# manhtuando97/two-stage-gnn

Hardware: AMD Instinct MI355X
Metric: graphs/sec fwd+bwd, DD batch=32 SAGE-3L h=128 (higher is better)
Workload: dtype f32

## Files before the change

include/tsgnn.h:

```cpp
#ifndef TSGNN_H
#define TSGNN_H
#include <stdint.h>

typedef struct ihipStream_t* tsgnn_stream_t;

#ifdef __cplusplus
extern "C" {
#endif

#define TSGNN_ABI_VERSION 2
int tsgnn_abi_version(void);
const char* tsgnn_strerror(int code);
const char* tsgnn_last_kernel(void);


int tsgnn_scan_workspace_ints(int64_t n, int64_t* ws_ints);
int tsgnn_exclusive_scan_i32(const int* in, int64_t n, int* out, int* ws, tsgnn_stream_t stream);

int tsgnn_row_maps(const int* graph_ptr, int B, int64_t n_rows, int* row_graph, int* row_slot,
                   tsgnn_stream_t stream);

int tsgnn_dense_adj_count(const float* adj, int B, int nmax, const int* graph_ptr, const int* row_graph,
                          int64_t n_rows, int* row_cnt, tsgnn_stream_t stream);
int tsgnn_dense_adj_fill(const float* adj, int B, int nmax, const int* graph_ptr, const int* row_graph,
// ... 44 lines not shown
                              void* after_event, int64_t* ticket);
int tsgnn_collate_pool_submit_ack(tsgnn_collate_pool* pool, const int64_t* ds_graph_ptr, const int64_t* ds_rowptr, const int64_t* ds_col,
                                  const int64_t* ds_node_label, const int64_t* ds_graph_label, const int64_t* ids, int B, int nmax,
                                  int64_t row_cap, int64_t edge_cap, int ell_w, int64_t tail_cap, int32_t* staging, int64_t* out,
                                  const int64_t* host_ack, int64_t ack_target, int seq, int64_t* ticket);
int tsgnn_collate_pool_wait(tsgnn_collate_pool* pool, int64_t ticket);
int tsgnn_collate_pool_destroy(tsgnn_collate_pool* pool);

int tsgnn_csr_transpose(const int* rowptr, const int* col, const float* val, int64_t n_rows, int64_t n_cols,
                        int64_t nnz, int* rowptr_t, int* col_t, float* val_t, int* src_e, int* cnt_ws,
                        int* scan_ws, tsgnn_stream_t stream);


int tsgnn_csr_spmm_f32(const int* rowptr, const int* col, const float* val, const float* self_w,
                       const float* x, int64_t ldx, float* y, int64_t ldy, int64_t n_rows, int feat,
                       float self_scalar, int relu_in, int accumulate, tsgnn_stream_t stream);

int tsgnn_csr_to_ell(const int* rowptr, const int* col, int64_t n_rows, int W, int* ell, int* tail_cnt, tsgnn_stream_t stream);
int tsgnn_csr_tail_fill(const int* rowptr, const int* col, const int* tail_ptr, int64_t n_rows, int W, int* tail_col,
                        tsgnn_stream_t stream);
int tsgnn_ell_spmm_f32(const int* ell, int W, const float* x, int64_t ldx, float* y, int64_t ldy, int64_t n_rows, int feat,
                       float self_scalar, tsgnn_stream_t stream);

int tsgnn_gcn_norm_f32(const int* rowptr, const int* col, const float* val, int64_t n_rows, float self_fill,
                       float* dinv, float* val_out, float* self_w, tsgnn_stream_t stream);

int tsgnn_sddmm_rows_f32(const int* rowptr, const int* col, const float* dy, int64_t lddy, const float* x, int64_t ldx,
                         int64_t n_rows, int feat, float* dval, float* dself, tsgnn_stream_t stream);


int tsgnn_gemm_f32(const float* A, int64_t sam, int64_t sak, const float* B, int64_t sbk, int64_t sbn, float* C,
                   int64_t scm, int64_t scn, int M, int N, int K, int batch, int64_t stride_a, int64_t stride_b,
                   int64_t stride_c, const int* seg_ptr, int ragged, int max_seg, float alpha, int accumulate,
                   tsgnn_stream_t stream);
int tsgnn_gemm_splitk_plan(int M, int N, int K, int* ksplit, int64_t* ws_floats);
int tsgnn_gemm_splitk_f32(const float* A, int64_t sam, int64_t sak, const float* B, int64_t sbk, int64_t sbn,
                          float* C, int M, int N, int K, int ksplit, float* ws, int accumulate,
                          tsgnn_stream_t stream);
int tsgnn_linear_wgrad_plan(int64_t rows, int K_in, int N, int64_t ldz, int64_t lddu, int* nslab, int64_t* rows_per_slab,
                            int64_t* ws_floats);
int tsgnn_linear_wgrad_f32(const float* z, int64_t ldz, const float* du, int64_t lddu, int64_t rows, int K_in, int N, int nslab,
                           int64_t rows_per_slab, int64_t bias_only_rows, float* ws, float* dw, float* db, tsgnn_stream_t stream);
int tsgnn_wgrad_reduce_sets_blocks(const int64_t* desc);
int tsgnn_wgrad_reduce_sets_f32(const int64_t* desc, float* normparts, float* step_state, tsgnn_stream_t stream);
int tsgnn_wgrad_reduce_multi_f32(const float* ws0, int nslab0, int K0, int N0, float* dw0, float* db0, const float* ws1, int nslab1,
                                 int K1, int N1, float* dw1, float* db1, const float* ws2, int nslab2, int K2, int N2, float* dw2,
                                 float* db2, const float* ws3, int nslab3, int K3, int N3, float* dw3, float* db3,
                                 float* normparts, float* step_state, tsgnn_stream_t stream);
int tsgnn_wgrad_blocks_plan(int64_t rows, int K_in, int N, int64_t ldz, int64_t lddu, int* nslab, int64_t* rows_per_slab,
                            int64_t* ws_floats);
int tsgnn_wgrad_blocks_f32(const float* z, int64_t ldz, const float* du, int64_t lddu, int64_t rows, int K_in, int N, int nslab,
                           int64_t rows_per_slab, float* ws, float* dw, int64_t lddw, tsgnn_stream_t stream);
int tsgnn_wgrad_blocks_oi_f32(const float* z, int64_t ldz, const float* du, int64_t lddu, int64_t rows, int K_in, int N, int nslab,
                              int64_t rows_per_slab, float* ws, float* dw_oi, int64_t lddw, float* db, tsgnn_stream_t stream);
int tsgnn_ragged_tn_f32(const float* s_mat, int64_t lds_, const float* x, int64_t ldx, int K, int N, const int* slab_row_ptr,
                        int nslab, const int* seg_slab_ptr, int nseg, float* ws, float* out, tsgnn_stream_t stream);
int tsgnn_ragged_tn_direct_supported(int K, int64_t max_rows);
int tsgnn_ragged_tn_direct_f32(const float* s_mat, int64_t lds_, int K, const int* graph_ptr, int B, const float* x0, int64_t ldx0,
                               int N0, float* out0, const float* x1, int64_t ldx1, int N1, float* out1, tsgnn_stream_t stream);
int tsgnn_ragged_tn_direct_ro_f32(const float* s_mat, int64_t lds_, int K, const int* graph_ptr, int B, const float* x0, int64_t ldx0,
                                  int N0, float* out0, const float* x1, int64_t ldx1, int N1, float* out1, float* ro_out,
                                  int64_t ro_ldo, int* ro_arg, int nmax, int64_t n_real, int ghost_zero, tsgnn_stream_t stream);
int tsgnn_wgrad_narrow_plan(int64_t rows, int K_in, int N, int64_t* ws_floats);
int tsgnn_wgrad_narrow_f32(const float* z, int64_t ldz, const float* du, int64_t lddu, int64_t rows, int K_in, int N, float* ws,
                           float* dwb, tsgnn_stream_t stream);
int tsgnn_colsum_f32(const float* x, int64_t ld, int64_t rows, int F, float* out, float* ws, int accumulate,
                     tsgnn_stream_t stream);

int tsgnn_linear_l2norm_f32(const float* z, int64_t ldz, const float* w, int64_t ldw, const float* bias, float* v,
                            int64_t ldv, float* rinv, int64_t rows, int K, int N, int normalize,
                            tsgnn_stream_t stream);
int tsgnn_rowgemm_supported(const float* a, int64_t lda, const float* b, int64_t ldb, const float* c, int64_t ldc, int K, int N,
                            int trans_b);
int tsgnn_rowgemm_f32(const float* a, int64_t lda, const float* b, int64_t ldb, int trans_b, const float* bias, float* c,
                      int64_t ldc, float* rinv, int64_t rows, int K, int N, int normalize, int64_t fill_rows,
                      tsgnn_stream_t stream);
int tsgnn_panel_blocks(int64_t rows, int panel_units);
int tsgnn_gather_rowgemm_f32(const int* ell, int ell_w, const int* tail_ptr, const int* tail_col, const float* x, int64_t ldx, const float* b, int64_t ldb, int trans_b,
                             const float* bias, float* c, int64_t ldc, float* rinv, float* zout, int64_t ldz, int64_t rows, int K,
                             int N, int normalize, int64_t fill_rows, tsgnn_stream_t stream);
int tsgnn_gather_rowgemm_st_f32(const int* ell, int ell_w, const int* tail_ptr, const int* tail_col, const float* x, int64_t ldx, const float* b, int64_t ldb, const float* bias,
                                float* c, int64_t ldc, float* rinv, float* zout, int64_t ldz, int64_t rows, int K, int N,
                                int64_t fill_rows, const int* row_slot, unsigned long long* sums, float* ghost, int panel_units,
                                tsgnn_stream_t stream);
int tsgnn_sage_layer_fwd_bn_f32(const int* ell, int ell_w, const int* tail_ptr, const int* tail_col, const float* x, int64_t ldx, const float* w, int64_t ldw, const float* bias,
                                float* v, int64_t ldv, float* rinv, float* zout, int64_t ldz, int64_t rows, int K, int64_t fill_rows,
                                const int* graph_ptr, const int* slot_count, int B, int nslots, int n_ghost, unsigned long long* packed,
                                unsigned long long* packed_out, const int* row_graph, const unsigned long long* sums_in,
                                const float* ghost_in, float* mean_out, float* rstd_out, const int* row_slot,
                                unsigned long long* sums_out, float* ghost_out, const int* ro_map, int ro_map_ch, int panel_units,
                                tsgnn_stream_t stream);
int tsgnn_sage_layer_fwd_bn_plan(int64_t rows, int64_t fill_rows, int B, int nslots, int panel_units, int* ro_ch, int* n_gemm,
                                 int* n_full);
int tsgnn_sage_layer_fwd_f32(const int* ell, int ell_w, const int* tail_ptr, const int* tail_col, const float* x, int64_t ldx, const float* w, int64_t ldw, const float* bias,
                             float* v, int64_t ldv, float* rinv, float* zout, int64_t ldz, int64_t rows, int K, int64_t fill_rows,
                             const int* graph_ptr, int B, int nslots, int n_ghost, unsigned long long* packed, tsgnn_stream_t stream);
int tsgnn_sage_layer_fwd_ro_f32(const int* ell, int ell_w, const int* tail_ptr, const int* tail_col, const float* x, int64_t ldx, const float* w, int64_t ldw, const float* bias,
                                float* v, int64_t ldv, float* rinv, float* zout, int64_t ldz, int64_t rows, int K, int64_t fill_rows,
                                const int* graph_ptr, int B, int nslots, int n_ghost, unsigned long long* packed,
                                unsigned long long* packed_out, const int* row_graph, tsgnn_stream_t stream);
int tsgnn_sage_layer_bwd_f32(const int* ell, int ell_w, const int* tail_ptr, const int* tail_col, const float* du, int64_t lddu, const float* w, int64_t ldw, float* dxs,
                             int64_t lddxs, const float* z, int64_t ldz, int64_t rows, int nslab, int64_t rows_per_slab,
                             int64_t bias_only_rows, float* ws, int panel_units, tsgnn_stream_t stream);
int tsgnn_l2norm_bwd_f32(const float* v, int64_t ldv, const float* dv, int64_t lddv, const float* rinv, float* du,
                         int64_t lddu, int64_t rows, int F, tsgnn_stream_t stream);


int tsgnn_bn_slots_fwd_f32(const int* graph_ptr, const int* slot_count, const int* row_slot, int B, int nmax,
                           int64_t n_real, int n_ghost, const float* v, int64_t ldv, int F, int relu, int bn,
                           float* mean, float* rstd, float* y, int64_t ldy, tsgnn_stream_t stream);
int tsgnn_bn_slots_bwd_f32(const int* graph_ptr, const int* slot_count, const int* row_slot, int B, int nmax,
                           int64_t n_real, int n_ghost, const float* v, int64_t ldv, const float* dy, int64_t lddy, int F,
                           int relu, int bn, const float* mean, const float* rstd, float* m1, float* m2, float* dv,
                           int64_t lddv, tsgnn_stream_t stream);

int tsgnn_row_ln_fwd_f32(const float* v, int64_t ldv, int64_t rows, int F, int relu, float* mean, float* rstd, float* y, int64_t ldy,
                         tsgnn_stream_t stream);
int tsgnn_row_ln_bwd_f32(const float* v, int64_t ldv, const float* dy, int64_t lddy, int64_t rows, int F, int relu, const float* mean,
                         const float* rstd, float* dv, int64_t lddv, tsgnn_stream_t stream);

int tsgnn_row_post_bwd_f32(const int* row_graph, int B, int64_t n_real, int64_t rows, const float* v, int64_t ldv, const float* dxs,
                           int64_t lddxs, const float* dout, int64_t ldo, const int* arg, int F, int relu, int ln, const float* mean,
                           const float* rstd, const float* rinv, float* du, int64_t lddu, tsgnn_stream_t stream);

int tsgnn_row_post_nodes_bwd_f32(int64_t n_real, int64_t rows, const float* v, int64_t ldv, const float* dxs, int64_t lddxs,
                                 const float* dnode, int64_t lddn, int ghost_zero, int F, int relu, int ln, const float* mean,
                                 const float* rstd, const float* rinv, float* du, int64_t lddu, tsgnn_stream_t stream);

int tsgnn_readout_max_ws_words(int B, int nmax, int F);
int tsgnn_readout_max_fwd_f32(const int* graph_ptr, const int* slot_count, int B, int nmax, int64_t n_real, int n_ghost,
                              const float* x, int64_t ldx, int F, int relu, unsigned long long* packed_ws, float* out,
                              int64_t ldo, int* arg, tsgnn_stream_t stream);
int tsgnn_readout_max_bwd_f32(const float* dout, int64_t ldo, const int* arg, int B, int F, const float* x, int64_t ldx_in,
                              int relu, int64_t n_real, float* dx, int64_t ldx, tsgnn_stream_t stream);
int tsgnn_readout_max_bwd_rows_f32(const float* dout, int64_t ldo, const int* arg, const int* row_graph, int F, int64_t rows,
                                   int64_t rows_total, const float* add, int64_t ldadd, float* dx, int64_t ldx, tsgnn_stream_t stream);

int tsgnn_pack_rows_f32(const float* src, int nmax, int F, const int* row_graph, const int* row_slot, int64_t n_real,
                        float* dst, int64_t ld, tsgnn_stream_t stream);
int tsgnn_unpack_rows_f32(const int* graph_ptr, int B, int nmax, int64_t n_real, int n_ghost, const float* src, int64_t ld,
                          int F, float fill, float* dst, tsgnn_stream_t stream);
int tsgnn_unpack_rows_bwd_ghost_f32(const int* graph_ptr, int B, int nmax, int64_t n_real, const float* ddst, int F,
                                    float* dsrc, int64_t ld, tsgnn_stream_t stream);


int tsgnn_softmax_ce_f32(const float* logits, int64_t ld, const int64_t* label, int B, int C, float* loss, float* dlogits,
                         tsgnn_stream_t stream);
int tsgnn_adam_from_partials_f32(float* param, const float* grad, float* m, float* v, int64_t n, float lr, float beta1, float beta2,
                                 float eps, float weight_decay, float max_norm, float* state, const float* parts, int nparts,
                                 const float* poison, tsgnn_stream_t stream);
int tsgnn_clip_adam_step_f32(float* param, const float* grad, float* m, float* v, int64_t n, float lr, float beta1,
                             float beta2, float eps, float weight_decay, float max_norm, float grad_scale, float* state,
                             float* ws, const float* poison, tsgnn_stream_t stream);


int tsgnn_dense_stack_supported(int B, int K, int nstack, int L, int fin0, int hidden, int last0, int last1);
int tsgnn_dense_stack_fwd_f32(const int64_t* desc, tsgnn_stream_t stream);
int tsgnn_dense_stack_bwd_f32(const int64_t* desc, tsgnn_stream_t stream);
int tsgnn_dense_stack_max_resident(void);
int tsgnn_dense_stack_barrier_selftest(unsigned* sync, float* err, int expect, tsgnn_stream_t stream);


int tsgnn_node_scores_f32(const float* x, int64_t ldx, int64_t rows, int H, int Fh, const float* a, int64_t lda, float* s,
                          tsgnn_stream_t stream);
int tsgnn_node_scores2_f32(const float* x, int64_t ldx, int64_t rows, int H, int Fh, const float* a1, int64_t lda1, float* s1,
                           const float* a2, int64_t lda2, float* s2, tsgnn_stream_t stream);
int tsgnn_edge_softmax_fwd_f32(const int* rowptr, const int* col, int64_t rows, int H, const float* s_grp, const float* s_oth,
                               int mod, float slope, float* alpha, tsgnn_stream_t stream);
int tsgnn_edge_softmax_bwd_f32(const int* rowptr, const int* col, int64_t rows, int H, const float* s_grp, const float* s_oth,
                               int mod, float slope, const float* alpha, const float* dalpha, float* dt, float* ds_grp,
                               tsgnn_stream_t stream);
int tsgnn_edge_permute_f32(const float* src, const int* perm, int64_t n, int H, int scatter, float* dst, tsgnn_stream_t stream);
int tsgnn_csr_row_sum_f32(const int* rowptr, const float* val, int64_t rows, int H, float* out, tsgnn_stream_t stream);
int tsgnn_csr_row_sum_perm_f32(const int* rowptr, const float* val, const int* eperm, int64_t rows, int H, float* out,
                               tsgnn_stream_t stream);
int tsgnn_csr_spmm_heads_f32(const int* rowptr, const int* col, const float* alpha, int H, int Fh, const float* x, int64_t ldx,
                             int mod, float* y, int64_t ldy, int64_t rows, tsgnn_stream_t stream);
int tsgnn_csr_spmm_heads_epi_f32(const int* rowptr, const int* col, const float* alpha, int H, int Fh, const float* x, int64_t ldx,
                                 int mod, float* y, int64_t ldy, int64_t rows, const float* w1, const float* a1, int64_t lda1,
                                 const float* w2, const float* a2, int64_t lda2, const float* u, int64_t ldu, const float* uw,
                                 int rows_per_seg, const int* row_seg, float uscale, const int* eperm, tsgnn_stream_t stream);
int tsgnn_csr_sddmm_heads_f32(const int* rowptr, const int* col, int H, int Fh, const float* dy, int64_t lddy, const float* x,
                              int64_t ldx, int mod, float* dalpha, int64_t rows, tsgnn_stream_t stream);
int tsgnn_segment_wsum_f32(const float* x, int64_t ldx, const float* w, int H, int Fh, const int* seg_ptr, int nseg, int64_t rows,
                           int64_t max_seg, float scale, int mean, float* ws, float* out, int64_t ldo, tsgnn_stream_t stream);
int tsgnn_segment_wsum2_f32(const float* x, int64_t ldx, const float* w1, const float* w2, int H, int Fh, const int* seg_ptr, int nseg,
// ... 350 lines not shown
```

two-stage-gnn_amd/csrc/head.hip:

```cpp
#include "common.h"
#include "../../include/tsgnn.h"
#include "readout_body.h"
#include "ingest_rider.h"

namespace {

__device__ __forceinline__ float4 ld4(const float* p) { return *reinterpret_cast<const float4*>(p); }

constexpr int HW = 16;

__device__ __forceinline__ void head2_fwd_tail(const float* xs, float* vs, int b, const float* __restrict__ w1,
                                               const float* __restrict__ b1, const float* __restrict__ w2, const float* __restrict__ b2,
                                               int P, int E, int C, float* __restrict__ vec, float* __restrict__ y) {
  const int tid = threadIdx.x, lane = tid & 63, wid = tid >> 6;
  const int P4 = P >> 2;
  for (int j0 = wid; j0 < E; j0 += 8 * HW) {
    float acc[8];
#pragma unroll
    for (int u = 0; u < 8; ++u) acc[u] = 0.f;
    for (int k4 = lane; k4 < P4; k4 += 64) {
      const float4 x = *reinterpret_cast<const float4*>(xs + 4 * k4);
      float4 w[8];
#pragma unroll
      for (int u = 0; u < 8; ++u) {
        const int j = j0 + HW * u;
        w[u] = ld4(w1 + (int64_t)(j < E ? j : 0) * P + 4 * k4);
      }
#pragma unroll
      for (int u = 0; u < 8; ++u) acc[u] += (w[u].x * x.x + w[u].y * x.y) + (w[u].z * x.z + w[u].w * x.w);
    }
#pragma unroll
    for (int u = 0; u < 8; ++u) {
      const int j = j0 + HW * u;
      const float r = wave_sum(acc[u]);
      if (lane == 0 && j < E) { const float v = r + (b1 ? b1[j] : 0.f); vs[j] = v; vec[(int64_t)b * E + j] = v; }
    }
  }
  __syncthreads();
  for (int c = wid; c < C; c += HW) {
    float acc = 0.f;
    for (int j = lane; j < E; j += 64) acc = fmaf(w2[(int64_t)c * E + j], vs[j], acc);
    acc = wave_sum(acc);
    if (lane == 0) y[(int64_t)b * C + c] = acc + (b2 ? b2[c] : 0.f);
  }
}

struct RoTail {
  const float* z; int64_t ldz; int N, c0, F;
  int* arg;
  float* dz; int64_t lddz;
};

__global__ __launch_bounds__(64 * HW) void head2_fwd_kernel(float* __restrict__ out, int64_t ldo, const float* __restrict__ w1,
                                                        const float* __restrict__ b1, const float* __restrict__ w2,
                                                        const float* __restrict__ b2, int P, int E, int C,
                                                        float* __restrict__ vec, float* __restrict__ y, RoTail rt) {
  extern __shared__ __attribute__((aligned(16))) float smem[];
  float* xs = smem;
  float* vs = smem + ((P + 3) & ~3);
  const int b = blockIdx.x, tid = threadIdx.x;
  const int c0 = rt.z ? rt.c0 : P;
  for (int k = tid; k < P; k += 64 * HW) {
    if (k < c0) { xs[k] = out[(int64_t)b * ldo + k]; continue; }
    const int f = k - c0;
    unsigned long long best = 0ull;
    for (int n0 = 0; n0 < rt.N; n0 += 16) {
      float val[16];
#pragma unroll
      for (int u = 0; u < 16; ++u) val[u] = rt.z[((int64_t)b * rt.N + min(n0 + u, rt.N - 1)) * rt.ldz + f];
#pragma unroll
      for (int u = 0; u < 16; ++u) {
        if (n0 + u < rt.N) {
          const unsigned long long q = ((unsigned long long)f32_ordered(val[u]) << 32) |
                                       (unsigned long long)(0xFFFFFFFFu - (unsigned)(b * rt.N + n0 + u));
          best = q > best ? q : best;
        }
      }
    }
    const float v = best ? ordered_f32((unsigned)(best >> 32)) : 0.f;
    xs[k] = v;
    out[(int64_t)b * ldo + k] = v;
    rt.arg[(int64_t)b * rt.F + f] = best ? (int)(0xFFFFFFFFu - (unsigned)(best & 0xFFFFFFFFull)) : -1;
  }
  __syncthreads();
  head2_fwd_tail(xs, vs, b, w1, b1, w2, b2, P, E, C, vec, y);
}

struct ReadoutHeadArgs {
  const unsigned long long* packed; int B, L, Fh, Fl;
  const float* v_last; int64_t ldv;
// ... 326 lines not shown
  for (int b = only >= 0 ? only + (int)threadIdx.x * B : (int)threadIdx.x; b < B; b += 64 * HW) {
    const float* row = ce.y + (int64_t)b * C;
    float m = -INFINITY;
    for (int c = 0; c < C; ++c) m = fmaxf(m, row[c]);
    float d = 0.f;
    for (int c = 0; c < C; ++c) d += expf(row[c] - m);
    const int yb = (int)ce.label[b];
    const float logz = m + logf(d);
    lb[b] = logz - row[yb];
    for (int c = 0; c < C; ++c) dyl[b * C + c] = (expf(row[c] - logz) - (c == yb ? 1.f : 0.f)) * invB;
  }
}

struct DuArgs {
  const int* graph_ptr; int64_t n_real; int n_ghost_rows; int chunks;
  const float* v; int64_t ldv; const float* rinv; const int* arg; int off; int F;
  float* du; int64_t lddu;
  const int* map;
  int compact;
};
template <int DU_CHUNK>
__device__ __forceinline__ void du_resolve(const DuArgs& a, int d, int B, int& b, int& c, int& pad_k, int& pad_n) {
  pad_k = -1; pad_n = a.chunks;
  if (a.map) { b = a.map[d] >> 8; c = a.map[d] & 255; }
  else if (a.compact) {
    const int lane = threadIdx.x & 63;
    const int g0 = a.graph_ptr[min(lane, B)], g1 = a.graph_ptr[min(lane + 1, B)];
    const int nch = lane < B ? max(1, (g1 - g0 + DU_CHUNK - 1) / DU_CHUNK) : 0;
    int pre = nch;
#pragma unroll
    for (int o = 1; o < 64; o <<= 1) { const int t = __shfl_up(pre, o, 64); if (lane >= o) pre += t; }
    const int total = __shfl(pre, 63, 64);
    if (d >= total) { b = B; c = 0; pad_k = d - total; pad_n = (int)gridDim.x - a.compact - total; return; }
    const unsigned long long m = __ballot(pre > d);
    b = __ffsll((long long)m) - 1;
    c = d - (__shfl(pre, b, 64) - __shfl(nch, b, 64));
  } else { b = d / a.chunks; c = d - b * a.chunks; }
  if (b >= B) { pad_k = c; b = B; }
}

template <int DU_CHUNK>
__device__ __forceinline__ void head2_du_role(const DuArgs& a, float* smem, const float* dy , int b, int c,
                                              int pad_k, int pad_n, const float* __restrict__ dvec, const float* __restrict__ w1,
                                              const float* __restrict__ w2, int B, int P, int E, int C, bool dy_ready_needs_sync) {
  const int tid = threadIdx.x, NTH = 64 * HW;
  const int F4 = a.F >> 2, lig = tid & 31, rg = tid >> 5;
  const float4 z4 = make_float4(0.f, 0.f, 0.f, 0.f);
  if (pad_k >= 0) {
    const int64_t lo = a.graph_ptr[B];
    for (int64_t r = lo + (int64_t)pad_k * 32 + rg; r < a.n_real; r += (int64_t)max(pad_n, 1) * 32)
      if (lig < F4) *reinterpret_cast<float4*>(a.du + r * a.lddu + 4 * lig) = z4;
    return;
  }
  const int g0 = a.graph_ptr[b], sz = a.graph_ptr[b + 1] - g0;
  const int lo = DU_CHUNK * c, hi = min(sz, lo + DU_CHUNK);
  const bool ghost_job = c == 0;
  if (lo >= hi && !ghost_job) return;
  const int P4 = P >> 2;
  const int G = min(16, NTH / P4);
  float* ds = smem;
  float* part = smem + ((E + 3) & ~3);
  float* dseg = part + G * a.F;
  constexpr int DU_ROWS = 8;
  static_assert(RB_ROWS % DU_ROWS == 0, "the row block's batches are walked in pieces");
  const int jg = tid >> 5;
  const bool wact = jg < G && lig < F4;
  const unsigned wcol = (unsigned)a.off + 4u * (unsigned)(wact ? lig : 0);
  float4 w[DU_ROWS];
#pragma unroll
  for (int u = 0; u < DU_ROWS; ++u) {
    const int j = jg + G * u;
    w[u] = ld4(w1 + (size_t)((unsigned)((wact && j < E) ? j : 0) * (unsigned)P + wcol));
  }
  float w2r[4];
  float dv0 = 0.f;
  if (tid < E) {
#pragma unroll
    for (int q = 0; q < 4; ++q) w2r[q] = q < C ? w2[(int64_t)q * E + tid] : 0.f;
    if (dvec) dv0 = dvec[(int64_t)b * E + tid];
  }
  if (dy_ready_needs_sync) __syncthreads();
  for (int j = tid; j < E; j += NTH) {
    float acc = j == tid ? dv0 : (dvec ? dvec[(int64_t)b * E + j] : 0.f);
    for (int q = 0; q < C; ++q) acc = fmaf(dy[(int64_t)b * C + q], (j == tid && q < 4) ? w2r[q] : w2[(int64_t)q * E + j], acc);
    ds[j] = acc;
  }
  __syncthreads();
  float4 acc = z4;
#pragma unroll
  for (int u0 = 0; u0 < RB_ROWS; u0 += DU_ROWS) {
    if (u0 > 0) {
#pragma unroll
      for (int u = 0; u < DU_ROWS; ++u) {
        const int j = jg + G * (u0 + u);
        w[u] = ld4(w1 + (size_t)((unsigned)((wact && j < E) ? j : 0) * (unsigned)P + wcol));
      }
    }
#pragma unroll
    for (int u = 0; u < DU_ROWS; ++u) {
      const int j = jg + G * (u0 + u);
      const float dd = (wact && j < E) ? ds[j] : 0.f;
      acc.x = fmaf(dd, w[u].x, acc.x); acc.y = fmaf(dd, w[u].y, acc.y); acc.z = fmaf(dd, w[u].z, acc.z); acc.w = fmaf(dd, w[u].w, acc.w);
    }
    __builtin_amdgcn_sched_barrier(0);
  }
  const unsigned ldv = (unsigned)a.ldv, lddu = (unsigned)a.lddu, col = 4u * (unsigned)(lig < F4 ? lig : 0);
  float4 vv[DU_CHUNK / 32];
  float ri[DU_CHUNK / 32];
  int rows[DU_CHUNK / 32];
#pragma unroll
  for (int u = 0; u < DU_CHUNK / 32; ++u) {
    const int n = lo + rg + 32 * u;
    rows[u] = n < hi ? g0 + n : -1;
    const unsigned rr = rows[u] >= 0 ? (unsigned)rows[u] : 0u;
    vv[u] = ld4(a.v + (size_t)(rr * ldv + col));
    ri[u] = a.rinv[rr];
  }
  const bool has_ghost = ghost_job && sz < a.n_ghost_rows;
  const int grow = (int)a.n_real + (has_ghost ? sz : 0);
  float4 gv = z4;
  float gri = 0.f;
  if (ghost_job && rg == 0 && a.n_ghost_rows > 0) { gv = ld4(a.v + (size_t)((unsigned)grow * ldv + col)); gri = a.rinv[grow]; }
  const int4 win = *reinterpret_cast<const int4*>(a.arg + (size_t)((unsigned)b * (unsigned)a.F + col));
  if (wact) *reinterpret_cast<float4*>(part + jg * a.F + 4 * lig) = acc;
  __syncthreads();
  for (int k = tid; k < a.F; k += NTH) {
    float t = 0.f;
    for (int q = 0; q < G; ++q) t += part[q * a.F + k];
    dseg[k] = t;
  }
  __syncthreads();
  const float4 gd = lig < F4 ? *reinterpret_cast<const float4*>(dseg + 4 * lig) : z4;
#pragma unroll
  for (int u = 0; u < DU_CHUNK / 32; ++u) {
    const int r32 = rows[u];
    float4 dyv = z4;
    if (rows[u] >= 0 && lig < F4) {
      if (win.x == r32) dyv.x = gd.x;
      if (win.y == r32) dyv.y = gd.y;
      if (win.z == r32) dyv.z = gd.z;
      if (win.w == r32) dyv.w = gd.w;
    } else {
      vv[u] = z4;
    }
    float dot = (vv[u].x * dyv.x + vv[u].y * dyv.y) + (vv[u].z * dyv.z + vv[u].w * dyv.w);
    dot = group_sum<32>(dot);
    if (rows[u] >= 0 && lig < F4) {
      if (ri[u] >= 0.999e12f) dot = 0.f;
      *reinterpret_cast<float4*>(a.du + (size_t)((unsigned)rows[u] * lddu + col)) =
          make_float4(ri[u] * (dyv.x - vv[u].x * dot), ri[u] * (dyv.y - vv[u].y * dot), ri[u] * (dyv.z - vv[u].z * dot),
                      ri[u] * (dyv.w - vv[u].w * dot));
    }
  }
  if (ghost_job && rg == 0) {
    const int r32 = grow;
    float4 dyv = z4;
    if (has_ghost && lig < F4) {
      if (win.x == r32) dyv.x = gd.x;
      if (win.y == r32) dyv.y = gd.y;
      if (win.z == r32) dyv.z = gd.z;
      if (win.w == r32) dyv.w = gd.w;
    } else {
      gv = z4;
    }
    float dot = (gv.x * dyv.x + gv.y * dyv.y) + (gv.z * dyv.z + gv.w * dyv.w);
    dot = group_sum<32>(dot);
    if (gri >= 0.999e12f) dot = 0.f;
    if (lig < F4)
      *reinterpret_cast<float4*>(a.du + (size_t)((unsigned)((int)a.n_real + b) * lddu + col)) =
          make_float4(gri * (dyv.x - gv.x * dot), gri * (dyv.y - gv.y * dot), gri * (dyv.z - gv.z * dot), gri * (dyv.w - gv.w * dot));
  }
}

template <int DU_CHUNK>
__global__ __launch_bounds__(64 * HW) void head2_bwd2_kernel(const float* __restrict__ out, int64_t ldo, const float* __restrict__ vec,
                                                         const float* __restrict__ dy_in, const float* __restrict__ dvec,
                                                         const float* __restrict__ w1, const float* __restrict__ w2, int B, int P, int E,
                                                         int C, float* __restrict__ dout, int64_t lddo, float* __restrict__ dw1,
                                                         float* __restrict__ db1, float* __restrict__ dw2, float* __restrict__ db2,
                                                         float* __restrict__ normparts, CeArgs ce, DuArgs dua, RoTail rt) {
  extern __shared__ __attribute__((aligned(16))) float smem_all[];
  const int tid = threadIdx.x, NTH = 64 * HW;
  const int P4 = P >> 2, PP = P;
  const bool has_ce = ce.label != nullptr;
  float* dyl = smem_all;
  float* lb = smem_all + (has_ce ? ((B * C + 3) & ~3) : 0);
  float* smem = lb + (has_ce ? ((B + 3) & ~3) : 0);
  const float* dy = has_ce ? dyl : dy_in;
  const int nj = (E + 3) / 4;
  if ((int)blockIdx.x >= B + nj + 1) {
    const int d = (int)blockIdx.x - (B + nj + 1);
    int gb, gc, pad_k, pad_n;
    du_resolve<DU_CHUNK>(dua, d, B, gb, gc, pad_k, pad_n);
    if (has_ce && pad_k < 0) ce_rows(ce, B, C, dyl, lb, gb);
    head2_du_role<DU_CHUNK>(dua, smem, dy, gb, gc, pad_k, pad_n, dvec, w1, w2, B, P, E, C, has_ce);
    return;
  }

  if ((int)blockIdx.x < B) {
    const int b = blockIdx.x;
    const int G = min(16, NTH / P4);
    const int jg = tid / P4, k4 = tid - jg * P4;
    const bool active = jg < G;
    float* ds = smem;
    float* part = smem + ((E + 3) & ~3);
    float w2r[4];
    float dv0 = 0.f;
    if (tid < E) {
#pragma unroll
      for (int c = 0; c < 4; ++c) w2r[c] = c < C ? w2[(int64_t)c * E + tid] : 0.f;
      if (dvec) dv0 = dvec[(int64_t)b * E + tid];
    }
    float4 w[RB_ROWS];
#pragma unroll
    for (int u = 0; u < RB_ROWS; ++u) {
      const int j = jg + G * u;
      w[u] = ld4(w1 + (int64_t)((active && j < E) ? j : 0) * P + 4 * (active ? k4 : 0));
    }
    if (has_ce) {
      ce_rows(ce, B, C, dyl, lb, b == 0 ? -1 : b);
      __syncthreads();
      if (b == 0) {
        float* red = lb + ((B + 3) & ~3);
        if (tid < 256) {
          float part = 0.f;
          for (int q = tid; q < B; q += 256) part += lb[q];
          part = wave_sum(part);
          if ((tid & 63) == 0) red[tid >> 6] = part;
        }
        __syncthreads();
        if (tid == 0) ce.loss[0] = ((red[0] + red[1]) + (red[2] + red[3])) / (float)B;
        __syncthreads();
      }
    }
    for (int j = tid; j < E; j += NTH) {
      float acc = j == tid ? dv0 : (dvec ? dvec[(int64_t)b * E + j] : 0.f);
      for (int c = 0; c < C; ++c) acc = fmaf(dy[(int64_t)b * C + c], (j == tid && c < 4) ? w2r[c] : w2[(int64_t)c * E + j], acc);
      ds[j] = acc;
    }
    __syncthreads();
    float4 acc = make_float4(0.f, 0.f, 0.f, 0.f);
    for (int j0 = 0; j0 < E; j0 += G * RB_ROWS) {
      if (j0 > 0) {
#pragma unroll
        for (int u = 0; u < RB_ROWS; ++u) {
          const int j = j0 + jg + G * u;
          w[u] = ld4(w1 + (int64_t)((active && j < E) ? j : 0) * P + 4 * (active ? k4 : 0));
        }
      }
#pragma unroll
      for (int u = 0; u < RB_ROWS; ++u) {
        const int j = j0 + jg + G * u;
        const float d = (active && j < E) ? ds[j] : 0.f;
        acc.x = fmaf(d, w[u].x, acc.x); acc.y = fmaf(d, w[u].y, acc.y); acc.z = fmaf(d, w[u].z, acc.z); acc.w = fmaf(d, w[u].w, acc.w);
      }
    }
    if (active) *reinterpret_cast<float4*>(part + jg * PP + 4 * k4) = acc;
    __syncthreads();
    for (int k = tid; k < P; k += NTH) {
      float a = 0.f;
      for (int q = 0; q < G; ++q) a += part[q * PP + k];
      dout[(int64_t)b * lddo + k] = a;
      if (rt.dz && k >= rt.c0 && k < rt.c0 + rt.F) {
        const int f = k - rt.c0;
        const int win = rt.arg[(int64_t)b * rt.F + f];
        for (int n = 0; n < rt.N; ++n) rt.dz[((int64_t)b * rt.N + n) * rt.lddz + f] = (b * rt.N + n) == win ? a : 0.f;
      }
    }
    return;
  }
  const int jb = (int)blockIdx.x - B;
  float sq = 0.f;
  if (jb < nj) {
    const int j0 = 4 * jb;
    const int G = max(1, min(8, 768 / P4));
    const int bg = tid / P4, k4 = tid - bg * P4;
    const bool active = bg < G;
    float* dvs = smem;
    float* part = smem + 4 * ((B + 3) & ~3);
    float w2r[4];
    float dv0 = 0.f;
    const int sb = tid >> 2, sj = j0 + (tid & 3);
    if (tid < 4 * B && sj < E) {
#pragma unroll
      for (int c = 0; c < 4; ++c) w2r[c] = c < C ? w2[(int64_t)c * E + sj] : 0.f;
      if (dvec) dv0 = dvec[(int64_t)sb * E + sj];
    }
    float4 x[WB_ROWS];
#pragma unroll
    for (int u = 0; u < WB_ROWS; ++u) {
      const int bb = bg + G * u;
      x[u] = ld4(out + (int64_t)((active && bb < B) ? bb : 0) * ldo + 4 * (active ? k4 : 0));
    }
    if (has_ce) { ce_rows(ce, B, C, dyl, lb, -1); __syncthreads(); }
    for (int i = tid; i < 4 * B; i += NTH) {
      const int bb = i >> 2, jj = j0 + (i & 3);
      float a = 0.f;
      if (jj < E) {
        a = i == tid ? dv0 : (dvec ? dvec[(int64_t)bb * E + jj] : 0.f);
        for (int c = 0; c < C; ++c) a = fmaf(dy[(int64_t)bb * C + c], (i == tid && c < 4) ? w2r[c] : w2[(int64_t)c * E + jj], a);
      }
      dvs[i] = a;
    }
    __syncthreads();
    float4 a0 = make_float4(0.f, 0.f, 0.f, 0.f), a1 = a0, a2 = a0, a3 = a0;
    for (int b0 = 0; b0 < B; b0 += G * WB_ROWS) {
      if (b0 > 0) {
#pragma unroll
        for (int u = 0; u < WB_ROWS; ++u) {
          const int bb = b0 + bg + G * u;
          x[u] = ld4(out + (int64_t)((active && bb < B) ? bb : 0) * ldo + 4 * (active ? k4 : 0));
        }
      }
#pragma unroll
      for (int u = 0; u < WB_ROWS; ++u) {
        const int bb = b0 + bg + G * u;
        if (active && bb < B) {
          const float4 d = *reinterpret_cast<const float4*>(dvs + 4 * bb);
          a0.x = fmaf(d.x, x[u].x, a0.x); a0.y = fmaf(d.x, x[u].y, a0.y); a0.z = fmaf(d.x, x[u].z, a0.z); a0.w = fmaf(d.x, x[u].w, a0.w);
          a1.x = fmaf(d.y, x[u].x, a1.x); a1.y = fmaf(d.y, x[u].y, a1.y); a1.z = fmaf(d.y, x[u].z, a1.z); a1.w = fmaf(d.y, x[u].w, a1.w);
          a2.x = fmaf(d.z, x[u].x, a2.x); a2.y = fmaf(d.z, x[u].y, a2.y); a2.z = fmaf(d.z, x[u].z, a2.z); a2.w = fmaf(d.z, x[u].w, a2.w);
          a3.x = fmaf(d.w, x[u].x, a3.x); a3.y = fmaf(d.w, x[u].y, a3.y); a3.z = fmaf(d.w, x[u].z, a3.z); a3.w = fmaf(d.w, x[u].w, a3.w);
        }
      }
    }
    if (active) {
      float* pp = part + (int64_t)bg * 4 * PP + 4 * k4;
      *reinterpret_cast<float4*>(pp) = a0; *reinterpret_cast<float4*>(pp + PP) = a1;
      *reinterpret_cast<float4*>(pp + 2 * PP) = a2; *reinterpret_cast<float4*>(pp + 3 * PP) = a3;
    }
    __syncthreads();
    for (int i = tid; i < 4 * P; i += NTH) {
      const int jj = i / P, k = i - jj * P;
      if (j0 + jj < E) {
        float a = 0.f;
        for (int q = 0; q < G; ++q) a += part[(q * 4 + jj) * PP + k];
        dw1[(int64_t)(j0 + jj) * P + k] = a;
        sq = fmaf(a, a, sq);
      }
    }
    if (db1 && tid < 4 && j0 + tid < E) {
      float a = 0.f;
      for (int bb = 0; bb < B; ++bb) a += dvs[4 * bb + tid];
      db1[j0 + tid] = a;
      sq = fmaf(a, a, sq);
    }
  } else {
    if (has_ce) { ce_rows(ce, B, C, dyl, lb, -1); __syncthreads(); }
    for (int i = tid; i < C * E; i += NTH) {
      const int c = i / E, j = i - c * E;
      float a = 0.f;
      int bb = 0;
      for (; bb + 8 <= B; bb += 8) {
        float v[8];
#pragma unroll
        for (int u = 0; u < 8; ++u) v[u] = vec[(int64_t)(bb + u) * E + j];
#pragma unroll
        for (int u = 0; u < 8; ++u) a = fmaf(dy[(int64_t)(bb + u) * C + c], v[u], a);
      }
      for (; bb < B; ++bb) a = fmaf(dy[(int64_t)bb * C + c], vec[(int64_t)bb * E + j], a);
      dw2[i] = a;
      sq = fmaf(a, a, sq);
    }
    if (db2) for (int c = tid; c < C; c += NTH) {
      float a = 0.f;
      for (int bb = 0; bb < B; ++bb) a += dy[(int64_t)bb * C + c];
      db2[c] = a;
      sq = fmaf(a, a, sq);
    }
  }
  if (normparts) {
    sq = wave_sum(sq);
    __syncthreads();
    if ((tid & 63) == 0) smem[tid >> 6] = sq;
    __syncthreads();
    if (tid == 0) {
      float t = 0.f;
      for (int w = 0; w < HW; ++w) t += smem[w];
      normparts[jb] = t;
    }
  }
}

// ... 217 lines not shown
```

two-stage-gnn_amd/csrc/ingest_rider.h:

```cpp
#pragma once
#include "common.h"

struct PullRider { const int4* host; int4* mirror; long long n4; unsigned blocks; long long lo; int parts_left; int skip; };
extern thread_local PullRider tsgnn_pull_rider_;

static inline PullRider take_pull_rider(int threads = 256) {
  PullRider& a = tsgnn_pull_rider_;
  PullRider r = a;
  if (a.blocks == 0) return r;
  if (a.skip > 0) { --a.skip; r.blocks = 0; return r; }
  const int parts = a.parts_left > 1 ? a.parts_left : 1;
  const long long left = a.n4 - a.lo;
  const long long take = parts > 1 ? ((left / parts + 3) & ~3ll) : left;
  r.n4 = a.lo + (take < left ? take : left);
  long long blocks = (r.n4 - r.lo + 2ll * threads - 1) / (2ll * threads);
  if (blocks > 512) blocks = 512;
  if (blocks < 1) blocks = 1;
  r.blocks = (unsigned)blocks;
  a.lo = r.n4;
  a.parts_left = parts - 1;
  if (a.parts_left <= 0 || a.lo >= a.n4) a.blocks = 0;
  return r;
}
static inline void disarm_pull_rider() { tsgnn_pull_rider_.blocks = 0; }

__device__ __forceinline__ void pull_rider_body(const PullRider& p, unsigned b) {
  const long long gtid = (long long)b * blockDim.x + threadIdx.x, gsize = (long long)p.blocks * blockDim.x;
  int4 v[4];
  long long i = p.lo + gtid;
  for (; i + 3 * gsize < p.n4; i += 4 * gsize) {
#pragma unroll
    for (int u = 0; u < 4; ++u) v[u] = p.host[i + u * gsize];
#pragma unroll
    for (int u = 0; u < 4; ++u) p.mirror[i + u * gsize] = v[u];
  }
  for (; i < p.n4; i += gsize) p.mirror[i] = p.host[i];
}

struct CLayout {
  int64_t header, graph_ptr, slot_count, label, rowptr, node_label, tail_ptr, col, tail_col, total;
};

struct ExpandArgs {
  const int32_t* mirror; CLayout L;
  int B, nmax, ell_w, F, ld4; int64_t row_cap;
  int32_t* row_graph; int32_t* row_slot; int32_t* ell; int32_t* tail_ptr; float* x; int64_t ldx;
  int64_t* host_ack;
  int32_t* ell_slots; int32_t* tail_slots;
};
__device__ __forceinline__ int expand_graph_of(const ExpandArgs& a, int64_t r, const int32_t* gp) {
  int lo = 0, hi = a.B;
  while (hi - lo > 1) { const int mid = (lo + hi) >> 1; if (gp[mid] <= r) lo = mid; else hi = mid; }
  return lo;
}

__device__ __forceinline__ void expand_row_lane(const ExpandArgs& a, int64_t r, int q, const int32_t* gp) {
  const int64_t total_rows = a.row_cap + a.nmax;
  if (a.host_ack && r == 0 && q == 0) {
    __hip_atomic_store(a.host_ack, (int64_t)a.mirror[a.L.header + 4], __ATOMIC_RELEASE, __HIP_MEMORY_SCOPE_SYSTEM);
  }
  if (r >= total_rows) return;
  const int64_t n = a.mirror[a.L.header];
  const int32_t ntail = a.mirror[a.L.header + 2];
  const int EQ = a.ell_w / 4;
  const int l = (r < n) ? a.mirror[a.L.node_label + r] : -1;
  if (q < EQ) {
    int4 v = make_int4(-1, -1, -1, -1);
    if (r < n) {
      const int32_t* rowptr = a.mirror + a.L.rowptr;
      const int e0 = rowptr[r], d = rowptr[r + 1] - e0;
      const int32_t* col = a.mirror + a.L.col + e0;
      const int k = 4 * q;
      if (k < d) v.x = col[k];
      if (k + 1 < d) v.y = col[k + 1];
      if (k + 2 < d) v.z = col[k + 2];
      if (k + 3 < d) v.w = col[k + 3];
    }
    *reinterpret_cast<int4*>(a.ell + r * a.ell_w + 4 * q) = v;
    if (a.ell_slots) {
      int4 w = make_int4(-1, -1, -1, -1);
      if (r < n) {
        const int g0 = gp[expand_graph_of(a, r, gp)];
        if (v.x >= 0) w.x = ((v.x - g0) << 20) | v.x;
        if (v.y >= 0) w.y = ((v.y - g0) << 20) | v.y;
        if (v.z >= 0) w.z = ((v.z - g0) << 20) | v.z;
        if (v.w >= 0) w.w = ((v.w - g0) << 20) | v.w;
      }
      *reinterpret_cast<int4*>(a.ell_slots + r * a.ell_w + 4 * q) = w;
    }
  } else if (q == EQ) {
    int g0 = 0;
    if (r < a.row_cap) {
      int g = a.B, slot = -1;
      if (r < n) {
        g = expand_graph_of(a, r, gp);
        g0 = gp[g];
        slot = (int)(r - g0);
      }
      a.row_graph[r] = g;
      a.row_slot[r] = slot;
    }
    a.tail_ptr[r] = r < n ? a.mirror[a.L.tail_ptr + r] : ntail;
    if (r == total_rows - 1) a.tail_ptr[total_rows] = ntail;
    if (a.tail_slots && r < n) {
      const int e1 = (r + 1 < n) ? a.mirror[a.L.tail_ptr + r + 1] : ntail;
      for (int e = a.mirror[a.L.tail_ptr + r]; e < e1; ++e) {
        const int j = a.mirror[a.L.tail_col + e];
        a.tail_slots[e] = ((j - g0) << 20) | j;
      }
    }
  } else {
    const bool ok = l >= 0 && l < a.F;
    for (int c4 = q - EQ - 1; c4 < a.ld4; c4 += 32 - EQ - 1) {
      const int c = 4 * c4;
      const float4 v = make_float4((ok && l == c) ? 1.f : 0.f, (ok && l == c + 1) ? 1.f : 0.f, (ok && l == c + 2) ? 1.f : 0.f,
                                   (ok && l == c + 3) ? 1.f : 0.f);
      *reinterpret_cast<float4*>(a.x + r * a.ldx + c) = v;
// ... 31 lines not shown
```

two-stage-gnn_amd/csrc/layer_bwd.hip:

```cpp
#include "common.h"
#include "../../include/tsgnn.h"
#include "rowgemm_body.h"
#include "tn_rows_body.h"
#include <cstdlib>

namespace {

template <bool PANELS_FIRST, bool UNITS = false>
__global__ __launch_bounds__(256) void sage_layer_bwd_kernel(RowGemmArgs ga, TnArgs gt, unsigned n_tn, unsigned nslab, unsigned n_pan, int slab_delay) {
  extern __shared__ __attribute__((aligned(16))) float smem[];
  if (PANELS_FIRST) {
    if (blockIdx.x < n_pan) rowgemm_body<4, true, true, 1, false, false, false, UNITS>(ga, smem, blockIdx.x);
    else {
      for (int i = 0; i < slab_delay; ++i) __builtin_amdgcn_s_sleep(16);
      const unsigned b = blockIdx.x - n_pan, by = b / nslab, sp = b % nslab;
      unsigned sl = sp;
      if ((nslab & 7u) == 0) sl = ((blockIdx.x & 7u) * (nslab >> 3)) + (sp >> 3);
      tn_rows_body<4, 4, 2>(gt, smem, sl, by, nslab);
    }
  } else {
    if (blockIdx.x < n_tn) tn_rows_body<4, 4, 2>(gt, smem, blockIdx.x % nslab, blockIdx.x / nslab, nslab);
    else rowgemm_body<4, true, true, 1, false, false, false, UNITS>(ga, smem, blockIdx.x - n_tn);
  }
}

}

extern "C" {

int tsgnn_sage_layer_bwd_f32(const int* ell, int ell_w, const int* tail_ptr, const int* tail_col, const float* du, int64_t lddu, const float* w, int64_t ldw, float* dxs,
                             int64_t lddxs, const float* z, int64_t ldz, int64_t rows, int nslab, int64_t rows_per_slab,
                             int64_t bias_only_rows, float* ws, int panel_units, tsgnn_stream_t stream) {
  if (!ell || !du || !w || !dxs || !z || !ws || rows <= 0 || nslab <= 0 || rows_per_slab <= 0 || bias_only_rows < 0) return TSGNN_EINVAL;
  if (ell_w != 4 && ell_w != 8 && ell_w != 16) return TSGNN_EUNSUPPORTED;
  const uintptr_t al = reinterpret_cast<uintptr_t>(ell) | reinterpret_cast<uintptr_t>(du) | reinterpret_cast<uintptr_t>(w) |
                       reinterpret_cast<uintptr_t>(dxs) | reinterpret_cast<uintptr_t>(z);
  if ((al & 15) || (lddu % 4) || (ldw % 4) || (lddxs % 4) || (ldz % 4) || lddu < 128 || ldw < 128 || lddxs < 128 || ldz < 128)
    return TSGNN_EUNSUPPORTED;
  if ((tail_ptr == nullptr) != (tail_col == nullptr)) return TSGNN_EINVAL;
  RowGemmArgs ga{du, lddu, w, ldw, nullptr, dxs, lddxs, nullptr, rows, 128, 128, 0, 0, ell, ell_w, nullptr, 0, tail_ptr, tail_col};
  TnArgs gt{z, ldz, du, lddu, rows, rows_per_slab, 128, 128, ws, nullptr, bias_only_rows};
  const int ncu = device_cu_count();
  const unsigned n_tn = 2u * (unsigned)nslab, n_pan = panel_split(rows, ncu, panel_units, &ga.n_full, &ga.unit);
  constexpr size_t la = rowgemm_lds_bytes<4, true, true>(), lt = tn_rows_lds_bytes<4, 4>();
  static const int panels_first = [] { const char* e = getenv("TSGNN_BWD_PANELS_FIRST"); return e ? atoi(e) : 1; }();
  static const int slab_delay_env = [] { const char* e = getenv("TSGNN_SLAB_DELAY"); return e ? atoi(e) : -1; }();
  const int slab_delay = slab_delay_env >= 0 ? slab_delay_env : ((int64_t)n_pan <= (int64_t)ncu ? 2 : 0);
  const bool units = ga.unit == 8 || ga.unit == 16;
  TSGNN_KNAME("sage_layer_bwd_kernel<%s,%s>", panels_first ? "true" : "false", units ? "true" : "false");
  if (panels_first && units) sage_layer_bwd_kernel<true, true><<<n_tn + n_pan, 256, la > lt ? la : lt, stream>>>(ga, gt, n_tn, (unsigned)nslab, n_pan, slab_delay);
  else if (panels_first) sage_layer_bwd_kernel<true><<<n_tn + n_pan, 256, la > lt ? la : lt, stream>>>(ga, gt, n_tn, (unsigned)nslab, n_pan, slab_delay);
  else if (units) sage_layer_bwd_kernel<false, true><<<n_tn + n_pan, 256, la > lt ? la : lt, stream>>>(ga, gt, n_tn, (unsigned)nslab, n_pan, slab_delay);
  else sage_layer_bwd_kernel<false><<<n_tn + n_pan, 256, la > lt ? la : lt, stream>>>(ga, gt, n_tn, (unsigned)nslab, n_pan, slab_delay);
  TSGNN_CHECK_LAUNCH();
  return TSGNN_OK;
}

}
```

two-stage-gnn_amd/csrc/layer_fwd.hip:

```cpp
#include "common.h"
#include "../../include/tsgnn.h"
#include "rowgemm_body.h"
#include "readout_body.h"
#include "ingest_rider.h"

namespace {

template <bool RO>
__global__ __launch_bounds__(256) void sage_layer_fwd_kernel(RowGemmArgs ga, SlotArgs sa, unsigned n_gemm, unsigned ro_gx, int F4,
                                                             unsigned long long* __restrict__ packed, unsigned n_main, PullRider pr) {
  extern __shared__ __attribute__((aligned(16))) float smem[];
  if (blockIdx.x < n_gemm) {
    rowgemm_body<4, false, true, 1, RO>(ga, smem, blockIdx.x);
  } else if (blockIdx.x < n_main) {
    const unsigned r = blockIdx.x - n_gemm;
    readout_partial_body<32>(sa, ga.a, ga.lda, F4, packed, r % ro_gx, r / ro_gx, reinterpret_cast<unsigned long long*>(smem));
  } else {
    pull_rider_body(pr, blockIdx.x - n_main);
  }
}

template <bool RO, bool ST, bool UNITS = false>
__global__ __launch_bounds__(256, 2) void sage_layer_fwd_bn_kernel(RowGemmArgs ga, SlotArgs sa, BnReadArgs bn, unsigned n_gemm, unsigned ro_gx,
                                                                int ro_ch, int F4, unsigned long long* __restrict__ packed, unsigned n_main,
                                                                PullRider pr, const int* __restrict__ ro_map) {
  extern __shared__ __attribute__((aligned(16))) float smem[];
  if (blockIdx.x < n_gemm) {
    rowgemm_body<4, false, true, 1, RO, true, ST, UNITS>(ga, smem, blockIdx.x);
  } else if (blockIdx.x < n_main) {
    unsigned r = blockIdx.x - n_gemm;
    if (ro_map) r = (unsigned)ro_map[r];
    readout_partial_bn_body<32>(sa, bn, ga.a, ga.lda, F4, packed, r % ro_gx, r / ro_gx, ro_ch, reinterpret_cast<unsigned long long*>(smem));
  } else {
    pull_rider_body(pr, blockIdx.x - n_main);
  }
}

}

extern "C" {

int tsgnn_sage_layer_fwd_bn_plan(int64_t rows, int64_t fill_rows, int B, int nslots, int panel_units, int* ro_ch, int* n_gemm, int* n_full) {
  if (!ro_ch || !n_gemm || !n_full || rows <= 0 || B <= 0 || nslots <= 0) return TSGNN_EINVAL;
  const int ncu = device_cu_count();
  int unit_ = 16;
  const unsigned ng = panel_split(rows, ncu, panel_units, n_full, &unit_) + (fill_rows > 0 ? 1u : 0u);
  int ch = 64;
  while (ch < 256 && ng + (unsigned)((nslots + ch - 1) / ch) * (unsigned)B > 2u * (unsigned)ncu) ch *= 2;
  *ro_ch = ch; *n_gemm = (int)ng;
  return TSGNN_OK;
}

int tsgnn_sage_layer_fwd_bn_f32(const int* ell, int ell_w, const int* tail_ptr, const int* tail_col, const float* x, int64_t ldx, const float* w, int64_t ldw, const float* bias,
                                float* v, int64_t ldv, float* rinv, float* zout, int64_t ldz, int64_t rows, int K, int64_t fill_rows,
                                const int* graph_ptr, const int* slot_count, int B, int nslots, int n_ghost, unsigned long long* packed,
                                unsigned long long* packed_out, const int* row_graph, const unsigned long long* sums_in,
                                const float* ghost_in, float* mean_out, float* rstd_out, const int* row_slot,
                                unsigned long long* sums_out, float* ghost_out, const int* ro_map, int ro_map_ch, int panel_units,
                                tsgnn_stream_t stream) {
  if (!ell || !x || !w || !v || !rinv || !graph_ptr || !slot_count || !packed || !sums_in || !ghost_in || !mean_out || !rstd_out ||
      rows <= 0 || fill_rows < 0 || K <= 0 || B <= 0 || nslots <= 0 || (n_ghost != 0 && n_ghost != nslots) || (packed_out && !row_graph) ||
      (row_slot && (!sums_out || !ghost_out)))
    return TSGNN_EINVAL;
  if (ell_w != 4 && ell_w != 8 && ell_w != 16) return TSGNN_EUNSUPPORTED;
  const uintptr_t al = reinterpret_cast<uintptr_t>(ell) | reinterpret_cast<uintptr_t>(x) | reinterpret_cast<uintptr_t>(w) |
                       reinterpret_cast<uintptr_t>(v) | reinterpret_cast<uintptr_t>(zout) | reinterpret_cast<uintptr_t>(bias) |
                       reinterpret_cast<uintptr_t>(sums_in) | reinterpret_cast<uintptr_t>(sums_out);
  if ((al & 15) || K != 128 || (ldx % 4) || (ldw % 4) || (ldv % 4) || (zout && (ldz % 4 || ldz < K)) || ldx < K || ldw < 128 || ldv < 128 ||
      nslots > BN_TAB || rows >= (1 << 20) || n_ghost == 0 || (packed_out && row_slot))
    return TSGNN_EUNSUPPORTED;
  if (packed_out && fill_rows <= 0) return TSGNN_EUNSUPPORTED;
  if ((tail_ptr == nullptr) != (tail_col == nullptr)) return TSGNN_EINVAL;
  RowGemmArgs ga{x, ldx, w, ldw, bias, v, ldv, rinv, rows, K, 128, 1, fill_rows, ell, ell_w, zout, ldz, tail_ptr, tail_col,
                 packed_out, graph_ptr, row_graph, B, nslots, n_ghost};
  ga.st_row_slot = row_slot; ga.st_sums = sums_out; ga.st_ghost = ghost_out;
  ga.bn_sums = sums_in; ga.bn_ghost = ghost_in; ga.bn_slot_count = slot_count; ga.bn_B = B; ga.bn_nslots = nslots; ga.bn_F = K;
  SlotArgs sa{graph_ptr, slot_count, B, nslots, rows, n_ghost};
  BnReadArgs bn{sums_in, ghost_in, K, mean_out, rstd_out};
  const int ncu = device_cu_count();
  const unsigned n_gemm = panel_split(rows, ncu, panel_units, &ga.n_full, &ga.unit) + (fill_rows > 0 ? 1u : 0u);
  int ro_ch = 64;
  while (ro_ch < 256 && n_gemm + (unsigned)((nslots + ro_ch - 1) / ro_ch) * (unsigned)B > 2u * (unsigned)ncu) ro_ch *= 2;
  const unsigned ro_gx = (unsigned)((nslots + ro_ch - 1) / ro_ch);
  if (ro_map && ro_map_ch != ro_ch) ro_map = nullptr;
  size_t lds = rowgemm_lds_bytes<4, false, true, 1, true>();
  const size_t lro = 8 * 128 * sizeof(unsigned long long) + 256 * sizeof(float2);
  if (lds < lro) lds = lro;
  const unsigned n_main = n_gemm + ro_gx * (unsigned)B;
  const PullRider pr = take_pull_rider();
  const bool units = ga.unit == 8 || ga.unit == 16;
#define TSGNN_FWD_BN(RO_, ST_)                                                                                                              \
  do {                                                                                                                                      \
    if (units) sage_layer_fwd_bn_kernel<RO_, ST_, true><<<n_main + pr.blocks, 256, lds, stream>>>(ga, sa, bn, n_gemm, ro_gx, ro_ch, K / 4, packed, n_main, pr, ro_map); \
    else sage_layer_fwd_bn_kernel<RO_, ST_><<<n_main + pr.blocks, 256, lds, stream>>>(ga, sa, bn, n_gemm, ro_gx, ro_ch, K / 4, packed, n_main, pr, ro_map);             \
  } while (0)
  if (packed_out) {
    TSGNN_KNAME("sage_layer_fwd_bn_kernel<true,false,%s>", units ? "true" : "false");
    TSGNN_FWD_BN(true, false);
  } else if (row_slot) {
    TSGNN_KNAME("sage_layer_fwd_bn_kernel<false,true,%s>", units ? "true" : "false");
    TSGNN_FWD_BN(false, true);
  } else {
    TSGNN_KNAME("sage_layer_fwd_bn_kernel<false,false,%s>", units ? "true" : "false");
    TSGNN_FWD_BN(false, false);
  }
#undef TSGNN_FWD_BN
  TSGNN_CHECK_LAUNCH();
  return TSGNN_OK;
}

int tsgnn_sage_layer_fwd_ro_f32(const int* ell, int ell_w, const int* tail_ptr, const int* tail_col, const float* x, int64_t ldx, const float* w, int64_t ldw, const float* bias,
                                float* v, int64_t ldv, float* rinv, float* zout, int64_t ldz, int64_t rows, int K, int64_t fill_rows,
                                const int* graph_ptr, int B, int nslots, int n_ghost, unsigned long long* packed,
                                unsigned long long* packed_out, const int* row_graph, tsgnn_stream_t stream) {
  if (!ell || !x || !w || !v || !rinv || !graph_ptr || !packed || rows <= 0 || fill_rows < 0 || K <= 0 || B <= 0 || nslots <= 0 ||
      (n_ghost != 0 && n_ghost != nslots) || (packed_out && !row_graph))
    return TSGNN_EINVAL;
  if (ell_w != 4 && ell_w != 8 && ell_w != 16) return TSGNN_EUNSUPPORTED;
  const uintptr_t al = reinterpret_cast<uintptr_t>(ell) | reinterpret_cast<uintptr_t>(x) | reinterpret_cast<uintptr_t>(w) |
                       reinterpret_cast<uintptr_t>(v) | reinterpret_cast<uintptr_t>(zout) | reinterpret_cast<uintptr_t>(bias);
  if ((al & 15) || K != 128 || (ldx % 4) || (ldw % 4) || (ldv % 4) || (zout && (ldz % 4 || ldz < K)) || ldx < K || ldw < 128 || ldv < 128)
    return TSGNN_EUNSUPPORTED;
  if ((tail_ptr == nullptr) != (tail_col == nullptr)) return TSGNN_EINVAL;
  if (packed_out && n_ghost && fill_rows <= 0) return TSGNN_EUNSUPPORTED;
  RowGemmArgs ga{x, ldx, w, ldw, bias, v, ldv, rinv, rows, K, 128, 1, fill_rows, ell, ell_w, zout, ldz, tail_ptr, tail_col,
                 packed_out, graph_ptr, row_graph, B, nslots, n_ghost};
  SlotArgs sa{graph_ptr, nullptr, B, nslots, rows, n_ghost};
  const unsigned n_gemm = (unsigned)ceil_div64(rows, 32) + (fill_rows > 0 ? 1u : 0u);
  const unsigned ro_gx = (unsigned)((nslots + 63) / 64);
  size_t lds = rowgemm_lds_bytes<4, false, true>();
  if (lds < 8 * 128 * sizeof(unsigned long long)) lds = 8 * 128 * sizeof(unsigned long long);
  const unsigned n_main = n_gemm + ro_gx * (unsigned)B;
  const PullRider pr = take_pull_rider();
  if (packed_out) {
    TSGNN_KNAME("sage_layer_fwd_kernel<true>");
    sage_layer_fwd_kernel<true><<<n_main + pr.blocks, 256, lds, stream>>>(ga, sa, n_gemm, ro_gx, K / 4, packed, n_main, pr);
  } else {
    TSGNN_KNAME("sage_layer_fwd_kernel<false>");
    sage_layer_fwd_kernel<false><<<n_main + pr.blocks, 256, lds, stream>>>(ga, sa, n_gemm, ro_gx, K / 4, packed, n_main, pr);
  }
  TSGNN_CHECK_LAUNCH();
  return TSGNN_OK;
}

int tsgnn_sage_layer_fwd_f32(const int* ell, int ell_w, const int* tail_ptr, const int* tail_col, const float* x, int64_t ldx, const float* w, int64_t ldw, const float* bias,
                             float* v, int64_t ldv, float* rinv, float* zout, int64_t ldz, int64_t rows, int K, int64_t fill_rows,
                             const int* graph_ptr, int B, int nslots, int n_ghost, unsigned long long* packed, tsgnn_stream_t stream) {
  return tsgnn_sage_layer_fwd_ro_f32(ell, ell_w, tail_ptr, tail_col, x, ldx, w, ldw, bias, v, ldv, rinv, zout, ldz, rows, K, fill_rows,
                                     graph_ptr, B, nslots, n_ghost, packed, nullptr, nullptr, stream);
}

}
```

two-stage-gnn_amd/csrc/rowgemm.hip:

```cpp
#include "common.h"
#include "../../include/tsgnn.h"

#include <cstdlib>
#include "rowgemm_body.h"
#include "ingest_rider.h"
#include "rowgemm_big_body.h"

namespace {

inline unsigned ks2_max_blocks() {
  static const unsigned n = [] { const char* e = getenv("TSGNN_KS2_MAX_BLOCKS"); return e ? (unsigned)atoi(e) : (unsigned)device_cu_count(); }();
  return n;
}
inline bool rowgemm_ks2_enabled() {
  static const bool on = [] { const char* e = getenv("TSGNN_ROWGEMM_KS2"); return !(e && e[0] == '0'); }();
  return on;
}

template <int NT, bool TRANS_B, bool GATHER>
__global__ __launch_bounds__(256) void rowgemm_kernel(RowGemmArgs g) {
  extern __shared__ __attribute__((aligned(16))) float smem[];
  rowgemm_body<NT, TRANS_B, GATHER>(g, smem, blockIdx.x);
}

template <int NT, bool TRANS_B>
__global__ __launch_bounds__(512) void rowgemm_gather_ks2_kernel(RowGemmArgs g) {
  extern __shared__ __attribute__((aligned(16))) float smem[];
  rowgemm_body<NT, TRANS_B, true, 2>(g, smem, blockIdx.x);
}

template <bool UNITS>
__global__ __launch_bounds__(256) void rowgemm_gather_st_kernel(RowGemmArgs g, PullRider pr, unsigned nblk) {
  extern __shared__ __attribute__((aligned(16))) float smem[];
  if (blockIdx.x >= nblk) { pull_rider_body(pr, blockIdx.x - nblk); return; }
  rowgemm_body<4, false, true, 1, false, false, true, UNITS>(g, smem, blockIdx.x);
}
__global__ __launch_bounds__(512) void rowgemm_gather_ks2_st_kernel(RowGemmArgs g, PullRider pr, unsigned nblk) {
  extern __shared__ __attribute__((aligned(16))) float smem[];
  if (blockIdx.x >= nblk) { pull_rider_body(pr, blockIdx.x - nblk); return; }
  rowgemm_body<4, false, true, 2, false, false, true>(g, smem, blockIdx.x);
}

template <int NT, bool TRANS_B>
__global__ __launch_bounds__(256) void rowgemm_colsplit_kernel(RowGemmArgs g) {
  extern __shared__ __attribute__((aligned(16))) float smem[];
  const int n0 = (int)blockIdx.y * 32 * NT;
  g.N = min(32 * NT, g.N - n0);
  g.c += n0;
  if (g.bias) g.bias += n0;
  g.b += TRANS_B ? (int64_t)n0 * g.ldb : (int64_t)n0;
  g.rinv = nullptr;
  if (!TRANS_B && g.N <= 32) rowgemm_body<1, TRANS_B, false>(g, smem, blockIdx.x);
  else rowgemm_body<NT, TRANS_B, false>(g, smem, blockIdx.x);
}

inline bool rowgemm_colsplit_enabled() {
  static const bool on = [] { const char* e = getenv("TSGNN_ROWGEMM_COLSPLIT"); return !(e && e[0] == '0'); }();
  return on;
}

inline unsigned colsplit_max_panels() {
  static const unsigned n = [] {
    const char* e = getenv("TSGNN_ROWGEMM_COLSPLIT_PANELS");
    return e ? (unsigned)atoi(e) : 0xFFFFFFFFu;
  }();
  return n;
}

inline int64_t rowgemm_big_min_rows() {
  static const int64_t n = [] {
    const char* e = getenv("TSGNN_ROWGEMM_BIG_ROWS");
    return e ? (int64_t)atoll(e) : (int64_t)49152;
  }();
  return n;
}

inline int64_t rowgemm_big_wide_min_rows() {
  static const int64_t n = [] {
    const char* e = getenv("TSGNN_ROWGEMM_BIG_WIDE_ROWS");
    return e ? (int64_t)atoll(e) : (int64_t)2048;
  }();
  return n;
}

template <int U, bool TRANS_B>
void launch_big(const RowGemmArgs& g, hipStream_t s) {
  constexpr size_t lds = rowgemm_big_lds_bytes<U, TRANS_B>();
  static const int bpc = [] {
    if (lds > 64 * 1024)
      (void)hipFuncSetAttribute(reinterpret_cast<const void*>(rowgemm_big_kernel<U, TRANS_B>), hipFuncAttributeMaxDynamicSharedMemorySize, (int)lds);
    int n = 0;
    if (hipOccupancyMaxActiveBlocksPerMultiprocessor(&n, reinterpret_cast<const void*>(rowgemm_big_kernel<U, TRANS_B>), 256, lds) != hipSuccess || n < 1) n = 1;
    return n;
  }();
  const unsigned npanels = (unsigned)ceil_div64(g.rows, 32);
  const unsigned ny = (unsigned)((g.N + 127) / 128);
  const unsigned heavy = (unsigned)(g.N / 128 + ((g.N % 128) > 32 ? 1 : 0));
  unsigned grid = (unsigned)device_cu_count() * (unsigned)bpc / (heavy ? heavy : 1u);
  if (grid > npanels) grid = npanels;
  if (grid == 0) grid = 1;
  if (ny > 1) {
    const unsigned per = (npanels + grid - 1) / grid;
    grid = (npanels + per - 1) / per;
  }
  TSGNN_KNAME("rowgemm_big_kernel<%d,%s>", U, TRANS_B ? "true" : "false");
  rowgemm_big_kernel<U, TRANS_B><<<dim3(grid, ny), 256, lds, s>>>(g, npanels);
}

template <bool TRANS_B>
bool try_big(const RowGemmArgs& g, hipStream_t s) {
  const bool wide = g.N > 128;
  const int64_t mn = wide ? rowgemm_big_wide_min_rows() : rowgemm_big_min_rows();
  if (mn <= 0 || g.rows < mn || g.N > 384 || g.K > 128 || (TRANS_B && (g.K % 4)) || (g.N % 4)) return false;
  if (g.N > 128 && (g.normalize || g.fill_rows > 0 || g.rinv)) return false;
  if (g.K <= 96) launch_big<12, TRANS_B>(g, s);
  else launch_big<16, TRANS_B>(g, s);
  return true;
}

template <bool TRANS_B>
bool try_colsplit(const RowGemmArgs& g, hipStream_t s) {
  const unsigned nblk = (unsigned)ceil_div64(g.rows, 32);
// ... 11 lines not shown
  const unsigned nblk = (unsigned)(ceil_div64(g.rows, 32) + (g.fill_rows > 0 ? 1 : 0));
  if constexpr (GATHER && NT <= 4) {
    if (g.K > KC && nblk <= ks2_max_blocks() && rowgemm_ks2_enabled()) {
      constexpr size_t lds2 = rowgemm_lds_bytes<NT, TRANS_B, true, 2>();
      static bool attr = false;
      if (!attr && lds2 > 64 * 1024) {
        (void)hipFuncSetAttribute(reinterpret_cast<const void*>(rowgemm_gather_ks2_kernel<NT, TRANS_B>),
                                  hipFuncAttributeMaxDynamicSharedMemorySize, (int)lds2);
        attr = true;
      }
      TSGNN_KNAME("rowgemm_gather_ks2_kernel<%d,%s>", NT, TRANS_B ? "true" : "false");
      rowgemm_gather_ks2_kernel<NT, TRANS_B><<<nblk, 512, lds2, s>>>(g);
      return;
    }
  }
  const size_t lds = rowgemm_lds_bytes<NT, TRANS_B, GATHER>();
  TSGNN_KNAME("rowgemm_kernel<%d,%s,%s>", NT, TRANS_B ? "true" : "false", GATHER ? "true" : "false");
  rowgemm_kernel<NT, TRANS_B, GATHER><<<nblk, 256, lds, s>>>(g);
}

template <bool TRANS_B, bool GATHER>
void dispatch_rowgemm(const RowGemmArgs& g, hipStream_t s) {
  switch ((g.N + 31) / 32) {
    case 1: launch_rowgemm<1, TRANS_B, GATHER>(g, s); break;
    case 2: launch_rowgemm<2, TRANS_B, GATHER>(g, s); break;
    case 3: launch_rowgemm<3, TRANS_B, GATHER>(g, s); break;
    case 4: launch_rowgemm<4, TRANS_B, GATHER>(g, s); break;
    default:
      if constexpr (!GATHER) {
        switch ((g.N + 31) / 32) {
          case 5: launch_rowgemm<5, TRANS_B, false>(g, s); break;
          case 6: launch_rowgemm<6, TRANS_B, false>(g, s); break;
          case 7: launch_rowgemm<7, TRANS_B, false>(g, s); break;
          default: launch_rowgemm<8, TRANS_B, false>(g, s); break;
        }
      }
      break;
  }
}

}

extern "C" {

int tsgnn_rowgemm_supported(const float* a, int64_t lda, const float* b, int64_t ldb, const float* c, int64_t ldc, int K, int N,
                            int trans_b) {
  const bool al = ((reinterpret_cast<uintptr_t>(a) | reinterpret_cast<uintptr_t>(b)) & 15) == 0;
  if (!al || (lda % 4) || (ldb % 4) || N > 384 || N <= 0 || K <= 0) return 0;
  if (lda < ((K + 3) / 4) * 4) return 0;
  if (!trans_b && (N % 4)) return 0;
  if (trans_b && (K % 4)) return 0;
  (void)c; (void)ldc;
  return 1;
}

int tsgnn_rowgemm_f32(const float* a, int64_t lda, const float* b, int64_t ldb, int trans_b, const float* bias, float* c,
                      int64_t ldc, float* rinv, int64_t rows, int K, int N, int normalize, int64_t fill_rows,
                      tsgnn_stream_t stream) {
  if (!a || !b || !c || rows < 0 || fill_rows < 0 || K <= 0 || N <= 0 || lda < K || ldc < N) return TSGNN_EINVAL;
  if (!tsgnn_rowgemm_supported(a, lda, b, ldb, c, ldc, K, N, trans_b)) return TSGNN_EUNSUPPORTED;
  if (fill_rows > 0 && ((N % 4) || (ldc % 4) || (reinterpret_cast<uintptr_t>(c) & 15) ||
                        (bias && (reinterpret_cast<uintptr_t>(bias) & 15))))
    return TSGNN_EUNSUPPORTED;
  if (rows == 0 && fill_rows == 0) return TSGNN_OK;
  RowGemmArgs g{a, lda, b, ldb, bias, c, ldc, rinv, rows, K, N, normalize, fill_rows, nullptr, 0, nullptr, 0};
  if (trans_b) {
    if (!try_big<true>(g, stream) && !try_colsplit<true>(g, stream)) {
      if (N > 256) return TSGNN_EUNSUPPORTED;
      dispatch_rowgemm<true, false>(g, stream);
    }
  } else {
    if (!try_big<false>(g, stream) && !try_colsplit<false>(g, stream)) {
      if (N > 256) return TSGNN_EUNSUPPORTED;
      dispatch_rowgemm<false, false>(g, stream);
    }
  }
  TSGNN_CHECK_LAUNCH();
  return TSGNN_OK;
}

int tsgnn_gather_rowgemm_st_f32(const int* ell, int ell_w, const int* tail_ptr, const int* tail_col, const float* x, int64_t ldx, const float* b, int64_t ldb, const float* bias,
                                float* c, int64_t ldc, float* rinv, float* zout, int64_t ldz, int64_t rows, int K, int N,
                                int64_t fill_rows, const int* row_slot, unsigned long long* sums, float* ghost, int panel_units,
                                tsgnn_stream_t stream) {
  if (!ell || !x || !b || !c || !row_slot || !sums || !ghost || rows <= 0 || fill_rows < 0 || K <= 0 || N <= 0 || ldx < K || ldc < N)
    return TSGNN_EINVAL;
  if (ell_w != 4 && ell_w != 8 && ell_w != 16) return TSGNN_EUNSUPPORTED;
  if (!tsgnn_rowgemm_supported(x, ldx, b, ldb, c, ldc, K, N, 0) || N > 128 || N <= 96 || K > 128 || (reinterpret_cast<uintptr_t>(ell) & 15) ||
      (reinterpret_cast<uintptr_t>(sums) & 15))
    return TSGNN_EUNSUPPORTED;
  if (zout && ((ldz % 4) || ldz < K || (reinterpret_cast<uintptr_t>(zout) & 15))) return TSGNN_EUNSUPPORTED;
  if ((N % 4) || (ldc % 4) || (reinterpret_cast<uintptr_t>(c) & 15) || (bias && (reinterpret_cast<uintptr_t>(bias) & 15))) return TSGNN_EUNSUPPORTED;
  if ((tail_ptr == nullptr) != (tail_col == nullptr)) return TSGNN_EINVAL;
  RowGemmArgs g{x, ldx, b, ldb, bias, c, ldc, rinv, rows, K, N, 1, fill_rows, ell, ell_w, zout, ldz, tail_ptr, tail_col};
  g.st_row_slot = row_slot; g.st_sums = sums; g.st_ghost = ghost;
  unsigned nblk = (unsigned)(ceil_div64(rows, 32) + (fill_rows > 0 ? 1 : 0));
  const bool ks2 = K > KC && nblk <= ks2_max_blocks() && rowgemm_ks2_enabled();
  if (!ks2)
    nblk = panel_split(rows, device_cu_count(), panel_units, &g.n_full, &g.unit) + (fill_rows > 0 ? 1u : 0u);
  if (ks2) {
    constexpr size_t lds2 = rowgemm_lds_bytes<4, false, true, 2>();
    static bool attr = false;
    if (!attr && lds2 > 64 * 1024) {
      (void)hipFuncSetAttribute(reinterpret_cast<const void*>(rowgemm_gather_ks2_st_kernel), hipFuncAttributeMaxDynamicSharedMemorySize, (int)lds2);
      attr = true;
    }
    const PullRider pr = take_pull_rider(512);
    TSGNN_KNAME("rowgemm_gather_ks2_st_kernel");
    rowgemm_gather_ks2_st_kernel<<<nblk + pr.blocks, 512, lds2, stream>>>(g, pr, nblk);
  } else {
    const PullRider pr = take_pull_rider(256);
    TSGNN_KNAME("rowgemm_gather_st_kernel<%s>", (g.unit == 8 || g.unit == 16) ? "true" : "false");
    if (g.unit == 8 || g.unit == 16) rowgemm_gather_st_kernel<true><<<nblk + pr.blocks, 256, rowgemm_lds_bytes<4, false, true>(), stream>>>(g, pr, nblk);
    else rowgemm_gather_st_kernel<false><<<nblk + pr.blocks, 256, rowgemm_lds_bytes<4, false, true>(), stream>>>(g, pr, nblk);
  }
  TSGNN_CHECK_LAUNCH();
  return TSGNN_OK;
}

int tsgnn_panel_blocks(int64_t rows, int panel_units) {
  if (rows <= 0) return 0;
  int nf = 0, un = 16;
  return (int)panel_split(rows, device_cu_count(), panel_units, &nf, &un);
}

int tsgnn_gather_rowgemm_f32(const int* ell, int ell_w, const int* tail_ptr, const int* tail_col, const float* x, int64_t ldx, const float* b, int64_t ldb, int trans_b,
                             const float* bias, float* c, int64_t ldc, float* rinv, float* zout, int64_t ldz, int64_t rows, int K,
                             int N, int normalize, int64_t fill_rows, tsgnn_stream_t stream) {
  if (!ell || !x || !b || !c || rows < 0 || fill_rows < 0 || K <= 0 || N <= 0 || ldx < K || ldc < N) return TSGNN_EINVAL;
  if (ell_w != 4 && ell_w != 8 && ell_w != 16) return TSGNN_EUNSUPPORTED;
  if (!tsgnn_rowgemm_supported(x, ldx, b, ldb, c, ldc, K, N, trans_b) || N > 128 || K > 128 || (reinterpret_cast<uintptr_t>(ell) & 15))
    return TSGNN_EUNSUPPORTED;
  if (zout && ((ldz % 4) || ldz < K || (reinterpret_cast<uintptr_t>(zout) & 15))) return TSGNN_EUNSUPPORTED;
  if (fill_rows > 0 && ((N % 4) || (ldc % 4) || (reinterpret_cast<uintptr_t>(c) & 15) ||
                        (bias && (reinterpret_cast<uintptr_t>(bias) & 15))))
    return TSGNN_EUNSUPPORTED;
  if (rows == 0 && fill_rows == 0) return TSGNN_OK;
  if ((tail_ptr == nullptr) != (tail_col == nullptr)) return TSGNN_EINVAL;
  RowGemmArgs g{x, ldx, b, ldb, bias, c, ldc, rinv, rows, K, N, normalize, fill_rows, ell, ell_w, zout, ldz, tail_ptr, tail_col};
  if (trans_b) dispatch_rowgemm<true, true>(g, stream);
  else dispatch_rowgemm<false, true>(g, stream);
  TSGNN_CHECK_LAUNCH();
  return TSGNN_OK;
}

}
```

two-stage-gnn_amd/csrc/rowgemm_body.h:

```cpp
#pragma once
#include "common.h"
#include <type_traits>
#include <cstdlib>

namespace {


typedef float f32x16 __attribute__((ext_vector_type(16)));
constexpr int KC = 32;
constexpr int LDA_S = KC + 4;
constexpr float NORM_EPS = 1e-12f;

struct RowGemmArgs {
  const float* a; int64_t lda;
  const float* b; int64_t ldb;
  const float* bias;
  float* c; int64_t ldc;
  float* rinv;
  int64_t rows; int K; int N;
  int normalize;
  int64_t fill_rows;
  const int* ell; int ell_w;
  float* zout; int64_t ldz;
  const int* tail_ptr; const int* tail_col;
  unsigned long long* ro_packed;
  const int* ro_graph_ptr; const int* ro_row_graph;
  int ro_B, ro_nslots, ro_nghost;
  const int* st_row_slot; unsigned long long* st_sums; float* st_ghost;
  const unsigned long long* bn_sums; const float* bn_ghost; const int* bn_slot_count; int bn_B, bn_nslots, bn_F;
  int n_full;
  int unit;
};

inline int panel_unit_rows(int64_t rows, int ncu) {
  static const int forced = [] { const char* e = getenv("TSGNN_PANEL_UNIT"); const int v = e ? atoi(e) : 0; return (v == 8 || v == 16) ? v : 0; }();
  if (forced) return forced;
  return ((rows + 31) / 32 - ncu) <= ncu / 16 ? 8 : 16;
}
inline unsigned panel_split(int64_t rows, int ncu, int panel_units, int* n_full, int* unit) {
  const int64_t P = (rows + 31) / 32;
  *n_full = 0; *unit = 32;
  if (!panel_units || ncu < 8) return (unsigned)P;
  if (P <= ncu || P - ncu > ncu / 2) return (unsigned)P;
  const int nf = ncu & ~7;
  *n_full = nf;
  const int u = *unit = panel_unit_rows(rows, ncu);
  return (unsigned)nf + (unsigned)((rows - 32 * (int64_t)nf + u - 1) / u);
}

constexpr int BN_TAB = 1024;
constexpr float BN_FWD_EPS = 1e-5f;
constexpr double BN_FIX = 1099511627776.0;

__device__ __forceinline__ unsigned long long rg_pack_max(float val, unsigned r) {
  return ((unsigned long long)f32_ordered(val) << 32) | (unsigned long long)(0xFFFFFFFFu - r);
}

__device__ __forceinline__ float4 ldg4(const float* p) { return *reinterpret_cast<const float4*>(p); }

constexpr int GN = 8;
constexpr int LDA_F = 128;

template <int NT, bool TRANS_B, bool GATHER, int KS = 1, bool READOUT = false, bool BNIN = false, bool STATS = false, bool UNITS = false>
__device__ __forceinline__ void rowgemm_body(const RowGemmArgs& g, float* smem_all, unsigned bid) {
  static_assert(KS == 1 || (KS == 2 && GATHER && NT <= 4), "the split-K variant is built for the gather kernel, widths <= 128");
  static_assert(!READOUT || (NT <= 4 && KS == 1), "the readout epilogue is built for one column tile per wave");
  static_assert(!BNIN || (GATHER && KS == 1), "batch-norm on the fly lives in the gather prologue of the one-group kernel");
  static_assert(!STATS || NT <= 4, "the statistics epilogue is built for one column tile per wave");
  constexpr int NP = 32 * NT;
  constexpr int TPW = (NT + 3) / 4;
  constexpr int BV = NT;
  constexpr int A_FLOATS = GATHER ? 0 : 32 * LDA_S;
  constexpr int B_FLOATS = TRANS_B ? NP * LDA_S : KC * NP;
  constexpr int STAGE = A_FLOATS + B_FLOATS;
  const int tid_all = threadIdx.x;
  const int grp = KS == 2 ? (tid_all >> 8) : 0;
  const int tid = KS == 2 ? (tid_all & 255) : tid_all, lane = tid & 63, wid = tid >> 6;
  const int i = lane & 31, h = lane >> 5;
  const int Kc = KS == 1 ? g.K : ((g.K + 2 * KC - 1) / (2 * KC)) * KC;
  const int kb = grp * Kc;
  const int Kv = KS == 1 ? g.K : min(g.K - kb, Kc);
  constexpr int GRP = (KS == 2 && 2 * STAGE < 4096 + 256) ? 4096 + 256 : 2 * STAGE;
  float* smem = smem_all + grp * GRP;
  float* Apanel = smem_all + KS * GRP + (KS == 2 ? 0 : 256);
  float* scratch = KS == 2 ? smem_all + GRP + 4096 : smem_all + 2 * STAGE;
  const unsigned npanels = (unsigned)((g.rows + 31) / 32);
  int64_t m0, rows_hi;
  if constexpr (UNITS) {
    const int un = g.unit == 8 ? 8 : 16;
    const unsigned nfull = (unsigned)g.n_full, nhalf = (unsigned)((g.rows - 32 * (int64_t)nfull + un - 1) / un);
    if (bid < nfull) { m0 = (int64_t)xcd_remap(bid, nfull) * 32; rows_hi = m0 + 32; }
    else if (bid < nfull + nhalf) { m0 = 32 * (int64_t)nfull + un * (int64_t)xcd_remap(bid - nfull, nhalf); rows_hi = min(m0 + un, g.rows); }
    else { m0 = (int64_t)npanels * 32; rows_hi = m0; }
  } else {
    m0 = (bid < npanels ? (int64_t)xcd_remap(bid, npanels) : (int64_t)bid) * 32;
    rows_hi = g.rows;
  }
  TR(0);
  if (m0 >= g.rows) {
    if (KS == 2 && grp == 1) return;
    float* fred = smem_all;
    const int N4 = g.N / 4, rpp = 256 / N4;
    const int c4 = tid % N4, rsub = tid / N4;
    float4 bv = make_float4(0.f, 0.f, 0.f, 0.f);
    if (g.bias && rsub < rpp) bv = ldg4(g.bias + 4 * c4);
    float ss = rsub == 0 ? (bv.x * bv.x + bv.y * bv.y) + (bv.z * bv.z + bv.w * bv.w) : 0.f;
    ss = wave_sum(ss);
    if (lane == 0) fred[wid] = ss;
    __syncthreads();
    float sc = 1.f;
    if (g.normalize) sc = fminf(__builtin_amdgcn_rsqf((fred[0] + fred[1]) + (fred[2] + fred[3])), 1.0f / NORM_EPS);
    const float4 out = make_float4(bv.x * sc, bv.y * sc, bv.z * sc, bv.w * sc);
    if constexpr (STATS) {
      if (g.st_ghost && wid == 0) {
        const float a = fmaxf(out.x, 0.f), b = fmaxf(out.y, 0.f), c = fmaxf(out.z, 0.f), d = fmaxf(out.w, 0.f);
        float g1 = rsub == 0 ? (a + b) + (c + d) : 0.f, g2 = rsub == 0 ? (a * a + b * b) + (c * c + d * d) : 0.f;
        g1 = wave_sum(g1); g2 = wave_sum(g2);
        if (lane == 0) { g.st_ghost[0] = g1; g.st_ghost[1] = g2; }
      }
    }
    if (rsub < rpp) {
      for (int64_t r = rsub; r < g.fill_rows; r += rpp) {
        *reinterpret_cast<float4*>(g.c + (g.rows + r) * g.ldc + 4 * c4) = out;
        if (g.rinv && c4 == 0) g.rinv[g.rows + r] = sc;
      }
      if constexpr (READOUT) {
        if (g.ro_packed && g.ro_nghost) {
          for (int b = rsub; b < g.ro_B; b += rpp) {
            const int sz = g.ro_graph_ptr[b + 1] - g.ro_graph_ptr[b];
            if (sz < g.ro_nslots && sz < g.fill_rows) {
              const unsigned row = (unsigned)(g.rows + sz);
              unsigned long long* dst = g.ro_packed + (int64_t)b * g.N + 4 * c4;
              atomicMax(dst + 0, rg_pack_max(out.x, row)); atomicMax(dst + 1, rg_pack_max(out.y, row));
              atomicMax(dst + 2, rg_pack_max(out.z, row)); atomicMax(dst + 3, rg_pack_max(out.w, row));
            }
          }
        }
      }
    }
    return;
  }
  int ro_gf = 0, ro_gl = 0;
  if constexpr (READOUT) {
    if (g.ro_packed) {
      ro_gf = g.ro_row_graph[m0];
      ro_gl = g.ro_row_graph[min(m0 + 31, rows_hi - 1)];
    }
  }

  const int am = tid >> 3, ak4 = tid & 7;
  const bool a_row_ok = (m0 + am) < rows_hi;
  const float* ap = g.a + ((a_row_ok && !GATHER) ? (m0 + am) : 0) * g.lda + 4 * ak4 + (GATHER ? 0 : kb);
  const float* bp[BV];
  int b_k[BV];
  int b_lds[BV];
  bool b_nok[BV];
#pragma unroll
  for (int q = 0; q < BV; ++q) {
    const int idx = q * 256 + tid;
    if (!TRANS_B) {
      const int k = idx / (NP / 4), n4 = idx % (NP / 4);
      b_nok[q] = 4 * n4 < g.N;
      bp[q] = g.b + (int64_t)(k + kb) * g.ldb + (b_nok[q] ? 4 * n4 : 0);
      b_k[q] = k;
      b_lds[q] = k * NP + 4 * n4;
    } else {
      const int n = idx / (KC / 4), k4 = idx % (KC / 4);
      b_nok[q] = n < g.N;
      bp[q] = g.b + (int64_t)(b_nok[q] ? n : 0) * g.ldb + 4 * k4 + kb;
      b_k[q] = 4 * k4;
      b_lds[q] = n * LDA_S + 4 * k4;
    }
  }
  struct Staged {
    float4 ra;
    float4 rb[BV];
    int a_valid;
    unsigned b_valid;
    bool plain;
  };
  const bool panel_full = (m0 + 32) <= rows_hi && g.N == NP;
  auto fetch = [&](Staged& s, int k0) {
    s.plain = panel_full && (k0 + KC) <= Kv;
    s.a_valid = 0;
    s.b_valid = 0;
    if (GATHER) {
#pragma unroll
      for (int q = 0; q < BV; ++q) {
        const bool kok = (k0 + b_k[q]) < Kv;
        if (!TRANS_B) s.rb[q] = ldg4(kok ? bp[q] + (int64_t)k0 * g.ldb : bp[q] - (int64_t)b_k[q] * g.ldb);
        else s.rb[q] = ldg4(kok ? bp[q] + k0 : bp[q] - b_k[q]);
        s.b_valid |= (kok && b_nok[q]) ? (1u << q) : 0u;
      }
      s.plain = false;
      return;
    }
    if (s.plain) {
      s.ra = ldg4(ap + k0);
#pragma unroll
      for (int q = 0; q < BV; ++q) s.rb[q] = ldg4(TRANS_B ? bp[q] + k0 : bp[q] + (int64_t)k0 * g.ldb);
      return;
    }
    const int gk = k0 + 4 * ak4;
    const bool ok = a_row_ok && gk < Kv;
    s.a_valid = ok ? min(4, Kv - gk) : 0;
    s.ra = ldg4(gk < Kv ? ap + k0 : ap - 4 * ak4);
#pragma unroll
    for (int q = 0; q < BV; ++q) {
      const bool kok = (k0 + b_k[q]) < Kv;
      if (!TRANS_B) s.rb[q] = ldg4(kok ? bp[q] + (int64_t)k0 * g.ldb : bp[q] - (int64_t)b_k[q] * g.ldb);
      else s.rb[q] = ldg4(kok ? bp[q] + k0 : bp[q] - b_k[q]);
      s.b_valid |= (kok && b_nok[q]) ? (1u << q) : 0u;
    }
  };
  auto commit = [&](const Staged& s, float* st) {
    if (GATHER) {
#pragma unroll
      for (int q = 0; q < BV; ++q)
        *reinterpret_cast<float4*>(st + A_FLOATS + b_lds[q]) = ((s.b_valid >> q) & 1u) ? s.rb[q] : make_float4(0.f, 0.f, 0.f, 0.f);
      return;
    }
    if (s.plain) {
      *reinterpret_cast<float4*>(st + am * LDA_S + 4 * ak4) = s.ra;
#pragma unroll
      for (int q = 0; q < BV; ++q) *reinterpret_cast<float4*>(st + A_FLOATS + b_lds[q]) = s.rb[q];
      return;
    }
    float4 va = s.ra;
    if (s.a_valid < 4) va.w = 0.f;
    if (s.a_valid < 3) va.z = 0.f;
    if (s.a_valid < 2) va.y = 0.f;
    if (s.a_valid < 1) va.x = 0.f;
    *reinterpret_cast<float4*>(st + am * LDA_S + 4 * ak4) = va;
#pragma unroll
    for (int q = 0; q < BV; ++q)
      *reinterpret_cast<float4*>(st + A_FLOATS + b_lds[q]) = ((s.b_valid >> q) & 1u) ? s.rb[q] : make_float4(0.f, 0.f, 0.f, 0.f);
  };
  auto frags = [&](const float* st, int k0, float (&af)[KC / 2], float (&bf)[TPW][KC / 2]) {
    const float* As = GATHER ? Apanel : st;
    constexpr int lda_s = GATHER ? LDA_F : LDA_S;
    const int kq = GATHER ? (kb + k0) >> 2 : 0;
    const float* Bs = st + A_FLOATS;
#pragma unroll
    for (int u = 0; u < KC / 8; ++u) {
      const float4 v = GATHER ? *reinterpret_cast<const float4*>(As + i * lda_s + 4 * ((kq + 2 * u + h) ^ (i & 7)))
                              : *reinterpret_cast<const float4*>(As + i * lda_s + 8 * u + 4 * h);
      af[4 * u] = v.x; af[4 * u + 1] = v.y; af[4 * u + 2] = v.z; af[4 * u + 3] = v.w;
    }
#pragma unroll
    for (int t = 0; t < TPW; ++t) {
      const int tile = wid + 4 * t;
      if (4 * (t + 1) <= NT || tile < NT) {
#pragma unroll
        for (int u = 0; u < KC / 8; ++u) {
          if (!TRANS_B) {
#pragma unroll
            for (int c = 0; c < 4; ++c) bf[t][4 * u + c] = Bs[(8 * u + 4 * h + c) * NP + tile * 32 + i];
          } else {
            const float4 v = *reinterpret_cast<const float4*>(Bs + (tile * 32 + i) * LDA_S + 8 * u + 4 * h);
            bf[t][4 * u] = v.x; bf[t][4 * u + 1] = v.y; bf[t][4 * u + 2] = v.z; bf[t][4 * u + 3] = v.w;
          }
        }
      } else {
#pragma unroll
        for (int j = 0; j < KC / 2; ++j) bf[t][j] = 0.f;
      }
    }
  };

  f32x16 acc[TPW];
#pragma unroll
  for (int t = 0; t < TPW; ++t)
#pragma unroll
    for (int r = 0; r < 16; ++r) acc[t][r] = 0.f;

  constexpr int NS = (NT <= 4 && !GATHER) ? 4 : 2;
  Staged st[NS];
  constexpr int NPASS = 4 / KS;
  int ids[NPASS][GN];
  if (GATHER) {
    const int rsub = tid_all >> 5;
#pragma unroll
    for (int p = 0; p < NPASS; ++p) {
      const int64_t row = m0 + 8 * KS * p + rsub;
#pragma unroll
      for (int q = 0; q < GN / 4; ++q) {
        int4 v = make_int4(-1, -1, -1, -1);
        if (row < rows_hi && 4 * q < g.ell_w) v = *reinterpret_cast<const int4*>(g.ell + row * g.ell_w + 4 * q);
        ids[p][4 * q] = v.x; ids[p][4 * q + 1] = v.y; ids[p][4 * q + 2] = v.z; ids[p][4 * q + 3] = v.w;
      }
    }
  }
  constexpr int BN_PT = BN_TAB / 256;
  float2* bn_tab = reinterpret_cast<float2*>(Apanel + 32 * LDA_F);
  ulonglong2 bn_s[BNIN ? BN_PT : 1];
  int bn_have[BNIN ? BN_PT : 1];
  float bn_g1 = 0.f, bn_g2 = 0.f;
  if constexpr (BNIN) {
#pragma unroll
    for (int q = 0; q < BN_PT; ++q) {
      const int n = min(tid_all + 256 * q, g.bn_nslots - 1);
      bn_s[q] = *reinterpret_cast<const ulonglong2*>(g.bn_sums + 2 * n);
      bn_have[q] = g.bn_slot_count[n];
    }
    bn_g1 = g.bn_ghost[0]; bn_g2 = g.bn_ghost[1];
  }
  int st_slot = -1;
  if constexpr (STATS) {
    if (g.st_sums && wid == 0 && grp == 0 && lane < 32 && (m0 + lane) < rows_hi) st_slot = g.st_row_slot[m0 + lane];
  }
#pragma unroll
  for (int c = 0; c < NS; ++c)
    if (c == 0 || c * KC < Kc) fetch(st[c], c * KC);
  if (GATHER) {
    const int c4 = tid_all & 31, rsub = tid_all >> 5;
    const bool colok = 4 * c4 < g.K;
    if constexpr (BNIN) {
      const double inv_cnt = 1.0 / ((double)g.bn_B * (double)g.bn_F);
#pragma unroll
      for (int q = 0; q < BN_PT; ++q) {
        const int n = tid_all + 256 * q;
        if (n < g.bn_nslots) {
          const float2 ms = bn_stats_from_sums(bn_s[q].x, bn_s[q].y, bn_have[q], bn_g1, bn_g2, g.bn_B, inv_cnt, BN_FWD_EPS);
          bn_tab[n] = make_float2(ms.y, ms.x * ms.y);
        }
      }
    }
    float4 nbv[NPASS][GN];
#pragma unroll
    for (int p = 0; p < NPASS; ++p)
#pragma unroll
      for (int k = 0; k < GN; ++k) {
        nbv[p][k] = make_float4(0.f, 0.f, 0.f, 0.f);
        if (colok && ids[p][k] >= 0) nbv[p][k] = ldg4(g.a + (int64_t)(BNIN ? (ids[p][k] & 0xFFFFF) : ids[p][k]) * g.lda + 4 * c4);
      }
    if constexpr (BNIN) {
      __syncthreads();
#pragma unroll
      for (int p = 0; p < NPASS; ++p)
#pragma unroll
        for (int k = 0; k < GN; ++k) {
          if (ids[p][k] >= 0) {
            const float2 rm = bn_tab[ids[p][k] >> 20];
            float4& t = nbv[p][k];
            t.x = fmaf(fmaxf(t.x, 0.f), rm.x, -rm.y); t.y = fmaf(fmaxf(t.y, 0.f), rm.x, -rm.y);
            t.z = fmaf(fmaxf(t.z, 0.f), rm.x, -rm.y); t.w = fmaf(fmaxf(t.w, 0.f), rm.x, -rm.y);
          }
        }
    }
#pragma unroll
    for (int p = 0; p < NPASS; ++p) {
      const int64_t row = m0 + 8 * KS * p + rsub;
      float4 va = nbv[p][0];
#pragma unroll
      for (int k = 1; k < GN; ++k) { va.x += nbv[p][k].x; va.y += nbv[p][k].y; va.z += nbv[p][k].z; va.w += nbv[p][k].w; }
      bool table_full = g.ell_w <= GN && ids[p][GN - 1] >= 0;
      if (colok && g.ell_w > GN && ids[p][GN - 1] >= 0) {
        static_assert(GN == 8, "the second half of a 16-wide table");
        const int4 e0 = *reinterpret_cast<const int4*>(g.ell + row * g.ell_w + 8), e1 = *reinterpret_cast<const int4*>(g.ell + row * g.ell_w + 12);
        const int js[8] = {e0.x, e0.y, e0.z, e0.w, e1.x, e1.y, e1.z, e1.w};
        table_full = js[7] >= 0;
        float4 t[8];
#pragma unroll
        for (int k = 0; k < 8; ++k) t[k] = ldg4(g.a + (int64_t)(js[k] >= 0 ? (BNIN ? (js[k] & 0xFFFFF) : js[k]) : 0) * g.lda + 4 * c4);
#pragma unroll
        for (int k = 0; k < 8; ++k) {
          if (js[k] >= 0) {
            if constexpr (BNIN) {
              const float2 rm = bn_tab[js[k] >> 20];
              t[k].x = fmaf(fmaxf(t[k].x, 0.f), rm.x, -rm.y); t[k].y = fmaf(fmaxf(t[k].y, 0.f), rm.x, -rm.y);
              t[k].z = fmaf(fmaxf(t[k].z, 0.f), rm.x, -rm.y); t[k].w = fmaf(fmaxf(t[k].w, 0.f), rm.x, -rm.y);
            }
            va.x += t[k].x; va.y += t[k].y; va.z += t[k].z; va.w += t[k].w;
          }
        }
      }
      if (colok && g.tail_ptr && row < rows_hi && table_full) {
        for (int e = g.tail_ptr[row]; e < g.tail_ptr[row + 1]; ++e) {
          const int j = g.tail_col[e];
          float4 t = ldg4(g.a + (int64_t)(BNIN ? (j & 0xFFFFF) : j) * g.lda + 4 * c4);
          if constexpr (BNIN) {
            const float2 rm = bn_tab[j >> 20];
            t.x = fmaf(fmaxf(t.x, 0.f), rm.x, -rm.y); t.y = fmaf(fmaxf(t.y, 0.f), rm.x, -rm.y);
            t.z = fmaf(fmaxf(t.z, 0.f), rm.x, -rm.y); t.w = fmaf(fmaxf(t.w, 0.f), rm.x, -rm.y);
          }
          va.x += t.x; va.y += t.y; va.z += t.z; va.w += t.w;
        }
      }
      {
        const int pr = 8 * KS * p + rsub;
        *reinterpret_cast<float4*>(Apanel + pr * LDA_F + 4 * (c4 ^ (pr & 7))) = va;
      }
      if (g.zout && colok && row < rows_hi) st_out(reinterpret_cast<float4*>(g.zout + row * g.ldz + 4 * c4), va);
    }
  }
  float bias_v[TPW];
#pragma unroll
  for (int t = 0; t < TPW; ++t) {
    const int cn = (wid + 4 * t) * 32 + i;
    bias_v[t] = (g.bias && (wid + 4 * t) < NT && cn < g.N) ? g.bias[cn] : 0.f;
  }
  TR(1);
  commit(st[0], smem);
  if (KC < Kc) commit(st[1], smem + STAGE);
  __syncthreads();
  TR(2);
  float fa[2][KC / 2], fb[2][TPW][KC / 2];
  frags(smem, 0, fa[0], fb[0]);
  if (NS == 2) {
    if (2 * KC < Kc) fetch(st[0], 2 * KC);
    if (3 * KC < Kc) fetch(st[1], 3 * KC);
  }
  auto body = [&](auto ci_, int c) {
    constexpr int CI = decltype(ci_)::value;
    constexpr int P = CI & 1;
    const int k0 = c * KC;
    if (k0 + KC < Kc) frags(smem + (P ^ 1) * STAGE, k0 + KC, fa[P ^ 1], fb[P ^ 1]);
    if (NS == 4 && c >= 0 && k0 + 4 * KC < Kc) fetch(st[CI % NS], k0 + 4 * KC);
    __builtin_amdgcn_sched_barrier(0);
#pragma unroll
    for (int j = 0; j < 8; ++j) acc[0] = __builtin_amdgcn_mfma_f32_32x32x2f32(fa[P][j], fb[P][0][j], acc[0], 0, 0, 0);
    __builtin_amdgcn_sched_barrier(0);
    if (k0 + 2 * KC < Kc) commit(st[(CI + 2) % NS], smem + P * STAGE);
    if (NS == 2 && k0 + 4 * KC < Kc) fetch(st[CI % NS], k0 + 4 * KC);
    __builtin_amdgcn_sched_barrier(0);
#pragma unroll
    for (int j = 8; j < KC / 2; ++j) acc[0] = __builtin_amdgcn_mfma_f32_32x32x2f32(fa[P][j], fb[P][0][j], acc[0], 0, 0, 0);
#pragma unroll
    for (int t = 1; t < TPW; ++t) {
      if (4 * (t + 1) <= NT || (wid + 4 * t) < NT) {
#pragma unroll
        for (int j = 0; j < KC / 2; ++j) acc[t] = __builtin_amdgcn_mfma_f32_32x32x2f32(fa[P][j], fb[P][t][j], acc[t], 0, 0, 0);
      }
    }
    TR(3 + 2 * min(c, 3));
    if (Kc > 2 * KC) __syncthreads();
    TR(4 + 2 * min(c, 3));
  };
  for (int c = 0; c * KC < Kc; c += 4) {
    body(std::integral_constant<int, 0>{}, c);
    if ((c + 1) * KC < Kc) body(std::integral_constant<int, 1>{}, c + 1);
    if ((c + 2) * KC < Kc) body(std::integral_constant<int, 2>{}, c + 2);
    if ((c + 3) * KC < Kc) body(std::integral_constant<int, 3>{}, c + 3);
  }
  if (KS == 2) {
    float* xch = smem_all + GRP;
    if (grp == 1) {
#pragma unroll
      for (int r = 0; r < 16; ++r) xch[(wid * 16 + r) * 64 + lane] = acc[0][r];
    }
    __syncthreads();
    TR(7);
    if (grp == 1) { TR_END(); return; }
#pragma unroll
    for (int r = 0; r < 16; ++r) acc[0][r] += xch[(wid * 16 + r) * 64 + lane];
    TR(8);
  }

  float scale[16];
#pragma unroll
  for (int r = 0; r < 16; ++r) scale[r] = 1.f;
  if (g.bias || g.normalize) {
    float ss[16];
    float q1[STATS ? 16 : 1], q2[STATS ? 16 : 1];
#pragma unroll
    for (int r = 0; r < 16; ++r) ss[r] = 0.f;
#pragma unroll
    for (int t = 0; t < TPW; ++t) {
      const int tile = wid + 4 * t;
      const int cn = tile * 32 + i;
      const bool okc = tile < NT && cn < g.N;
      const float bv = bias_v[t];
#pragma unroll
      for (int r = 0; r < 16; ++r) {
        const float v = okc ? acc[t][r] + bv : 0.f;
        acc[t][r] = v;
        ss[r] = fmaf(v, v, ss[r]);
        if constexpr (STATS) { const float rl = fmaxf(v, 0.f); q1[r] = rl; q2[r] = rl * rl; }
      }
    }
    if (g.normalize) {
      float* red = scratch;
      float* inv = red + 128 + wid * 32;
      float* redq = smem_all;
      if constexpr (STATS) { if (Kc <= 2 * KC) __syncthreads(); }
      float tot = row16_sum_transpose(ss);
      tot += __shfl_xor(tot, 16, 64);
      float t1 = 0.f, t2 = 0.f;
      if constexpr (STATS) {
        t1 = row16_sum_transpose(q1); t2 = row16_sum_transpose(q2);
        t1 += __shfl_xor(t1, 16, 64); t2 += __shfl_xor(t2, 16, 64);
      }
      TR(11);
      if ((lane & 16) == 0) {
        const int r = lane & 15, row = (r & 3) + 8 * (r >> 2) + 4 * h;
        red[row * 4 + wid] = tot;
        if constexpr (STATS) { redq[row * 4 + wid] = t1; redq[128 + row * 4 + wid] = t2; }
      }
      __syncthreads();
      TR(12);
      if (lane < 32) {
        const float4 p = *reinterpret_cast<const float4*>(red + lane * 4);
        const float rs = fminf(__builtin_amdgcn_rsqf((p.x + p.y) + (p.z + p.w)), 1.0f / NORM_EPS);
        inv[lane] = rs;
        if (g.rinv && wid == 0 && (m0 + lane) < rows_hi) g.rinv[m0 + lane] = rs;
        if constexpr (STATS) {
          if (g.st_sums && wid == 0 && st_slot >= 0) {
            const float4 a = *reinterpret_cast<const float4*>(redq + lane * 4), b = *reinterpret_cast<const float4*>(redq + 128 + lane * 4);
            const float s1 = ((a.x + a.y) + (a.z + a.w)) * rs, s2 = ((b.x + b.y) + (b.z + b.w)) * (rs * rs);
            atomicAdd(g.st_sums + 2 * st_slot, (unsigned long long)__double2ll_rn((double)s1 * BN_FIX));
            atomicAdd(g.st_sums + 2 * st_slot + 1, (unsigned long long)__double2ll_rn((double)s2 * BN_FIX));
          }
        }
      }
      __syncthreads();
#pragma unroll
      for (int q = 0; q < 4; ++q) {
        const float4 v = *reinterpret_cast<const float4*>(inv + 8 * q + 4 * h);
        scale[4 * q] = v.x; scale[4 * q + 1] = v.y; scale[4 * q + 2] = v.z; scale[4 * q + 3] = v.w;
      }
    }
  }
  const bool full = panel_full;
#pragma unroll
  for (int t = 0; t < TPW; ++t) {
    const int tile = wid + 4 * t;
    if (tile < NT) {
      const int cn = tile * 32 + i;
      float* cp = g.c + (m0 + 4 * h) * g.ldc + cn;
      if (full) {
#pragma unroll
        for (int r = 0; r < 16; ++r) st_out(cp + (int64_t)((r & 3) + 8 * (r >> 2)) * g.ldc, acc[t][r] * scale[r]);
      } else {
#pragma unroll
        for (int r = 0; r < 16; ++r) {
          const int64_t gm = m0 + (r & 3) + 8 * (r >> 2) + 4 * h;
          if (gm < rows_hi && cn < g.N) cp[(int64_t)((r & 3) + 8 * (r >> 2)) * g.ldc] = acc[t][r] * scale[r];
        }
      }
    }
  }
  if constexpr (READOUT) {
    if (g.ro_packed) {
      const int cn = wid * 32 + i;
      const int64_t last = min(m0 + 31, rows_hi - 1);
      for (int b = ro_gf; b <= ro_gl; ++b) {
        int64_t lo = m0, hi = last + 1;
        if (ro_gf != ro_gl) { lo = max(lo, (int64_t)g.ro_graph_ptr[b]); hi = min(hi, (int64_t)g.ro_graph_ptr[b + 1]); }
        unsigned long long best = 0ull;
#pragma unroll
        for (int r = 0; r < 16; ++r) {
          const int64_t gm = m0 + (r & 3) + 8 * (r >> 2) + 4 * h;
          if (gm >= lo && gm < hi) {
            const unsigned long long p = rg_pack_max(acc[0][r] * scale[r], (unsigned)gm);
            best = p > best ? p : best;
          }
        }
        const unsigned olo = __shfl_xor((unsigned)(best & 0xFFFFFFFFull), 32, 64), ohi = __shfl_xor((unsigned)(best >> 32), 32, 64);
        const unsigned long long other = ((unsigned long long)ohi << 32) | olo;
        best = other > best ? other : best;
        if (h == 0 && best && cn < g.N) atomicMax(&g.ro_packed[(int64_t)b * g.N + cn], best);
      }
    }
  }
  TR(13);
  TR_END();
}


template <int NT, bool TRANS_B, bool GATHER, int KS = 1, bool BNIN = false>
constexpr size_t rowgemm_lds_bytes() {
  constexpr int NP = 32 * NT;
  constexpr int STAGE2 = 2 * ((GATHER ? 0 : 32 * LDA_S) + (TRANS_B ? NP * LDA_S : KC * NP));
  constexpr int GRP = (KS == 2 && STAGE2 < 4096 + 256) ? 4096 + 256 : STAGE2;
  return sizeof(float) * (KS * GRP + (KS == 2 ? 0 : 128 + 4 * 32) + (GATHER ? 32 * LDA_F : 0) + (BNIN ? 2 * BN_TAB : 0));
}

}
```

two-stage-gnn_amd/csrc/sageconv.hip:

```cpp
#include <algorithm>
#include "common.h"
#include "../../include/tsgnn.h"
#include "sageconv_body.h"
#include "tn_rows_body.h"

namespace {

__global__ __launch_bounds__(512) void sage_conv_kernel(SageConvArgs g) {
  extern __shared__ __attribute__((aligned(16))) float smem[];
  sageconv_body(g, smem, blockIdx.x);
}

template <int MT, int NTt, int NY>
__global__ __launch_bounds__(256) void sage_wgrad_pair_kernel(TnArgs a, TnArgs b) {
  extern __shared__ __attribute__((aligned(16))) float tn_smem[];
  tn_rows_body<MT, NTt, NY>(blockIdx.z ? b : a, tn_smem, blockIdx.x, blockIdx.y, gridDim.x);
}

__global__ __launch_bounds__(256) void sage_relu_readout_bwd_kernel(const float* __restrict__ h, int64_t ldh, const float* __restrict__ dxs,
                                                                    int64_t lddxs, const float* __restrict__ dread, int64_t lddr,
                                                                    const int* __restrict__ arg, const int* __restrict__ row_graph,
                                                                    const int* __restrict__ graph_ptr, int64_t rows, int F, int relu,
                                                                    float* __restrict__ du, int64_t lddu, const float* __restrict__ row_scale,
                                                                    float* __restrict__ dus, int64_t lddus) {
  const int F4 = F >> 2;
  const int64_t idx = (int64_t)blockIdx.x * 256 + threadIdx.x;
  if (idx >= rows * F4) return;
  const int64_t r = idx / F4;
  const int c = 4 * (int)(idx % F4);
  const int b = row_graph[r];
  const float4 hv = *reinterpret_cast<const float4*>(h + r * ldh + c);
  float4 d = dxs ? *reinterpret_cast<const float4*>(dxs + r * lddxs + c) : make_float4(0.f, 0.f, 0.f, 0.f);
  if (dread) {
    const float inv_n = 1.0f / (float)max(graph_ptr[b + 1] - graph_ptr[b], 1);
    const float4 dm = *reinterpret_cast<const float4*>(dread + (int64_t)b * lddr + c);
    const float4 ds = *reinterpret_cast<const float4*>(dread + (int64_t)b * lddr + F + c);
    const int4 a = *reinterpret_cast<const int4*>(arg + (int64_t)b * F + c);
    const int ri = (int)r;
    d.x += (a.x == ri ? dm.x : 0.f) + ds.x * inv_n;
    d.y += (a.y == ri ? dm.y : 0.f) + ds.y * inv_n;
    d.z += (a.z == ri ? dm.z : 0.f) + ds.z * inv_n;
    d.w += (a.w == ri ? dm.w : 0.f) + ds.w * inv_n;
  }
  if (relu) {
    d.x = hv.x > 0.f ? d.x : 0.f; d.y = hv.y > 0.f ? d.y : 0.f; d.z = hv.z > 0.f ? d.z : 0.f; d.w = hv.w > 0.f ? d.w : 0.f;
  }
  st_out(reinterpret_cast<float4*>(du + r * lddu + c), d);
  if (dus) {
    const float sc = row_scale[r];
    st_out(reinterpret_cast<float4*>(dus + r * lddus + c), make_float4(d.x * sc, d.y * sc, d.z * sc, d.w * sc));
  }
}

__global__ __launch_bounds__(128) void sage_readout_decode_kernel(unsigned long long* __restrict__ packed, unsigned long long* __restrict__ sums,
                                                                  const int* __restrict__ graph_ptr, int B, int L, int F,
                                                                  float* __restrict__ read, int64_t ldr, int* __restrict__ arg) {
  const int b = blockIdx.x;
  const float inv_n = 1.0f / (float)max(graph_ptr[b + 1] - graph_ptr[b], 1);
  for (int f = threadIdx.x; f < F; f += 128) {
    float m = 0.f, s = 0.f;
    for (int l = 0; l < L; ++l) {
      const int64_t o = ((int64_t)l * B + b) * F + f;
      const unsigned long long pk = packed[o];
      const long long q = (long long)sums[o];
      packed[o] = 0ull; sums[o] = 0ull;
      m += pk ? ordered_f32((unsigned)(pk >> 32)) : 0.f;
      s += (float)((double)q * (1.0 / SC_RO_FIX)) * inv_n;
      arg[o] = (int)(0xFFFFFFFFu - (unsigned)(pk & 0xFFFFFFFFull));
    }
    read[(int64_t)b * ldr + f] = m;
    read[(int64_t)b * ldr + F + f] = s;
  }
}

struct PackSet {
  const float* w; int64_t ldw; int K, N; int kn;
  float4* out;
};
struct PackArgs { PackSet s[16]; int nsets; };

__global__ __launch_bounds__(256) void sage_conv_pack_kernel(PackArgs a) {
  const PackSet& s = a.s[blockIdx.y];
  const int e = (int)blockIdx.x * 256 + (int)threadIdx.x;
  const int lane = e & 63, u = (e >> 6) & 15, wv = e >> 10;
  const int i = lane & 31, h = lane >> 5;
  const int n = 32 * wv + i, k0 = 8 * u + 4 * h;
  float v[4];
#pragma unroll
  for (int c = 0; c < 4; ++c) {
    const int k = k0 + c;
    const bool ok = n < s.N && k < s.K;
    v[c] = ok ? (s.kn ? s.w[(int64_t)k * s.ldw + n] : s.w[(int64_t)n * s.ldw + k]) : 0.f;
  }
  s.out[e] = make_float4(v[0], v[1], v[2], v[3]);
}

}

extern "C" {

int tsgnn_sage_conv_supported(int K, int N) { return (K >= 1 && K <= 128 && N >= 1 && N <= 128) ? 1 : 0; }

int tsgnn_sage_conv_pack_f32(const int64_t* desc, tsgnn_stream_t stream) {
  if (!desc) return TSGNN_EINVAL;
  const int nsets = (int)desc[0];
  if (nsets <= 0 || nsets > 16) return TSGNN_EINVAL;
  PackArgs a{};
  a.nsets = nsets;
  const int64_t* d = desc + 1;
  for (int t = 0; t < nsets; ++t, d += 6) {
    PackSet& s = a.s[t];
    s.w = reinterpret_cast<const float*>(d[0]); s.ldw = d[1]; s.K = (int)d[2]; s.N = (int)d[3]; s.kn = (int)d[4];
    s.out = reinterpret_cast<float4*>(d[5]);
    if (!s.w || !s.out || !tsgnn_sage_conv_supported(s.K, s.N) || s.ldw < (s.kn ? s.N : s.K)) return TSGNN_EINVAL;
    if (reinterpret_cast<uintptr_t>(s.out) & 15) return TSGNN_EUNSUPPORTED;
  }
  TSGNN_KNAME("sage_conv_pack_kernel");
  sage_conv_pack_kernel<<<dim3(16, (unsigned)nsets), 256, 0, stream>>>(a);
  TSGNN_CHECK_LAUNCH();
  return TSGNN_OK;
}

int tsgnn_sage_conv_f32(const int* ell, int ell_w, const int* tail_ptr, const int* tail_col, const float* xg, int64_t ldxg, const float* xs,
                        int64_t ldxs, const float* dst_scale, const float* wl_pk, const float* wr_pk,
                        const float* bias, float* out, int64_t ldo, float* zout, int64_t ldz, float* rinv,
                        int64_t rows, int K, int N, int relu_out, int normalize, unsigned long long* ro_packed,
                        unsigned long long* ro_sums, const int* ro_row_graph, const int* ro_graph_ptr, const float* post_h, int64_t post_ldh,
                        const float* post_dread, int64_t post_lddr, const int* post_arg, const float* post_row_scale, float* out2,
                        int64_t ldo2, tsgnn_stream_t stream) {
  if (!ell || !xg || !xs || !wl_pk || !wr_pk || !out || rows < 0 || K <= 0 || N <= 0) return TSGNN_EINVAL;
  if ((tail_ptr == nullptr) != (tail_col == nullptr)) return TSGNN_EINVAL;
  if ((ro_packed == nullptr) != (ro_sums == nullptr) || (ro_packed && (!ro_row_graph || !ro_graph_ptr))) return TSGNN_EINVAL;
  if (post_h && (!post_dread || !post_arg || !ro_row_graph || !ro_graph_ptr || post_ldh < N || post_lddr < 2 * N || ro_packed || relu_out ||
                 normalize || (out2 && (!post_row_scale || ldo2 < N))))
    return TSGNN_EINVAL;
  if (!post_h && out2) return TSGNN_EINVAL;
  if (ell_w != 4 && ell_w != 8 && ell_w != 16) return TSGNN_EUNSUPPORTED;
  if (!tsgnn_sage_conv_supported(K, N)) return TSGNN_EUNSUPPORTED;
  const int K4 = (K + 3) / 4 * 4;
  if ((ldxg % 4) || (ldxs % 4) || ldxg < K4 || ldxs < K4 || ldo < N || (zout && ((ldz % 4) || ldz < K4))) return TSGNN_EUNSUPPORTED;
  if ((reinterpret_cast<uintptr_t>(ell) | reinterpret_cast<uintptr_t>(xg) | reinterpret_cast<uintptr_t>(xs) | reinterpret_cast<uintptr_t>(zout) |
       reinterpret_cast<uintptr_t>(wl_pk) | reinterpret_cast<uintptr_t>(wr_pk)) & 15)
    return TSGNN_EUNSUPPORTED;
  if (rows == 0) return TSGNN_OK;
  if (rows >= (int64_t)1 << 31) return TSGNN_EUNSUPPORTED;
  SageConvArgs g{xg, ldxg, xs, ldxs, ell, ell_w, tail_ptr, tail_col, dst_scale, reinterpret_cast<const float4*>(wl_pk),
                 reinterpret_cast<const float4*>(wr_pk), bias, out, ldo, zout, ldz, rinv, rows, K, N, relu_out, normalize, ro_packed, ro_sums,
                 ro_row_graph, ro_graph_ptr, post_h, post_ldh, post_dread, post_lddr, post_arg, post_row_scale, out2, ldo2};
  constexpr size_t lds = sageconv_lds_bytes();
  static bool attr = false;
  if (!attr && lds > 48 * 1024) {
    (void)hipFuncSetAttribute(reinterpret_cast<const void*>(sage_conv_kernel), hipFuncAttributeMaxDynamicSharedMemorySize, (int)lds);
    attr = true;
  }
  TSGNN_KNAME("sage_conv_kernel");
  sage_conv_kernel<<<(unsigned)ceil_div64(rows, 32), 512, lds, stream>>>(g);
  TSGNN_CHECK_LAUNCH();
  return TSGNN_OK;
}

int tsgnn_sage_wgrad_pair_f32(const float* z, int64_t ldz, const float* x, int64_t ldx, const float* du, int64_t lddu, int64_t rows, int K,
                              int N, int nslab, int64_t rows_per_slab, float* ws_l, float* ws_r, tsgnn_stream_t stream) {
  if (!z || !x || !du || !ws_l || !ws_r || rows < 0 || nslab <= 0 || rows_per_slab <= 0 || K <= 0 || N <= 0) return TSGNN_EINVAL;
  if (K > 128 || N > 128 || (ldz % 4) || (ldx % 4) || (lddu % 4) || (N % 4) ||
      ((reinterpret_cast<uintptr_t>(z) | reinterpret_cast<uintptr_t>(x) | reinterpret_cast<uintptr_t>(du)) & 15))
    return TSGNN_EUNSUPPORTED;
  TnArgs a{z, ldz, du, lddu, rows, rows_per_slab, K, N, ws_l, nullptr, 0};
  TnArgs b{x, ldx, du, lddu, rows, rows_per_slab, K, N, ws_r, nullptr, 0};
  const int mt = (K + 31) / 32, nt = (N + 31) / 32;
  const unsigned ny = (mt * nt >= 8 && nslab < 512) ? 2u : 1u;
  const dim3 grid((unsigned)nslab, ny, 2);
  TSGNN_KNAME("sage_wgrad_pair_kernel<%d,%d,%u>", mt, nt, ny);
#define TSGNN_TN(M_, N_) do { \
    constexpr size_t lds_ = tn_rows_lds_bytes<M_, N_>(); \
    static bool attr_ = false; \
    if (ny == 2) { \
      if (!attr_ && lds_ > 48 * 1024) { (void)hipFuncSetAttribute(reinterpret_cast<const void*>(sage_wgrad_pair_kernel<M_, N_, 2>), hipFuncAttributeMaxDynamicSharedMemorySize, (int)lds_); attr_ = true; } \
      sage_wgrad_pair_kernel<M_, N_, 2><<<grid, 256, lds_, stream>>>(a, b); \
    } else { \
      if (!attr_ && lds_ > 48 * 1024) { (void)hipFuncSetAttribute(reinterpret_cast<const void*>(sage_wgrad_pair_kernel<M_, N_, 1>), hipFuncAttributeMaxDynamicSharedMemorySize, (int)lds_); attr_ = true; } \
      sage_wgrad_pair_kernel<M_, N_, 1><<<grid, 256, lds_, stream>>>(a, b); \
    } } while (0)
  switch (mt * 10 + nt) {
    case 11: TSGNN_TN(1, 1); break; case 12: TSGNN_TN(1, 2); break; case 13: TSGNN_TN(1, 3); break; case 14: TSGNN_TN(1, 4); break;
    case 21: TSGNN_TN(2, 1); break; case 22: TSGNN_TN(2, 2); break; case 23: TSGNN_TN(2, 3); break; case 24: TSGNN_TN(2, 4); break;
    case 31: TSGNN_TN(3, 1); break; case 32: TSGNN_TN(3, 2); break; case 33: TSGNN_TN(3, 3); break; case 34: TSGNN_TN(3, 4); break;
    case 41: TSGNN_TN(4, 1); break; case 42: TSGNN_TN(4, 2); break; case 43: TSGNN_TN(4, 3); break; default: TSGNN_TN(4, 4); break;
  }
#undef TSGNN_TN
  TSGNN_CHECK_LAUNCH();
  return TSGNN_OK;
}

int tsgnn_sage_relu_readout_bwd_f32(const float* h, int64_t ldh, const float* dxs, int64_t lddxs, const float* dread, int64_t lddr,
                                    const int* arg, const int* row_graph, const int* graph_ptr, int64_t rows, int F, int relu, float* du,
                                    int64_t lddu, const float* row_scale, float* dus, int64_t lddus, tsgnn_stream_t stream) {
  if (!h || !du || rows < 0 || F <= 0 || (dread && (!arg || !row_graph || !graph_ptr)) || (dus && (!row_scale || (lddus % 4))))
    return TSGNN_EINVAL;
// ... 60 lines not shown
```

two-stage-gnn_amd/sage_stack.py:

```python
import torch

from . import _native as nat
from . import message_passing as mp


def eligible(g, convs, bn, x):
    if not bn or g.B > 128 or len(convs) < 2:
        return False
    hid = convs[0].output_dim
    for i, c in enumerate(convs):
        if c.add_self or not c.normalize_embedding or c.dropout > 0.001:
            return False
        if c.output_dim % 4 or c.output_dim > 128:
            return False
        if i < len(convs) - 1 and c.output_dim != hid:
            return False
    return x.dim() == 2 and x.size(1) % 4 == 0 and x.is_cuda and x.stride(0) % 4 == 0


def _aggregate_raw(g, x, transposed=False, rows=None):
    n = g.total_rows if rows is None else rows
    if g.val is None and mp.ell_ok(x) and g.total_rows <= mp.ELL_MAX_ROWS and (not transposed or g.symmetric):
        return mp.spmm_ell(g, x, rows=n)
    rp, col, val = g.transposed() if transposed else (g.rowptr, g.col, g.val)
    return mp.spmm_raw(rp, col, val, x, n)


import os

FUSED_TAIL = os.environ.get("TSGNN_FUSED_TAIL", "1") != "0"
MERGED_FWD = os.environ.get("TSGNN_MERGED_FWD", "1") != "0"
MERGED_BWD = os.environ.get("TSGNN_MERGED_BWD", "1") != "0"
GATHER_MAX_ROWS = int(os.environ.get("TSGNN_GATHER_MAX_ROWS", 65536))
GATHER_FUSED = os.environ.get("TSGNN_GATHER_FUSED", "1") != "0"
EPILOGUE_READOUT = os.environ.get("TSGNN_EPILOGUE_READOUT", "1") != "0"
LAST_LAYER_ROWS = os.environ.get("TSGNN_LAST_LAYER_ROWS", "1") != "0"
RO_MAP = os.environ.get("TSGNN_RO_MAP", "1") != "0"
FUSED_BN = os.environ.get("TSGNN_FUSED_BN", "1") != "0"
SLOT_WGRAD = os.environ.get("TSGNN_SLOT_WGRAD", "0") != "0"
HEAD_DU = os.environ.get("TSGNN_HEAD_DU", "1") != "0"


DU_MAP = os.environ.get("TSGNN_DU_MAP", "1") != "0"
SLABS_BESIDE = os.environ.get("TSGNN_SLABS_BESIDE", "1") != "0"
NSLAB_MAX = int(os.environ.get("TSGNN_NSLAB_MAX", "0"))
_ncu = {}


def _cu_count(dev):
    n = _ncu.get(dev)
    if n is None:
        n = _ncu[dev] = torch.cuda.get_device_properties(dev).multi_processor_count
    return n


def _slabs_beside_panels(nslab, rps, need, rows, K, N, dev, panel_units):
    if not SLABS_BESIDE or nslab <= 0:
        return nslab, rps, need
    if NSLAB_MAX and nslab > NSLAB_MAX:
        rps = (-(-rows // NSLAB_MAX) + 7) // 8 * 8
        nslab = -(-rows // rps)
        need = nslab * (K + 1) * N
    ncu = _cu_count(dev)
    npan = int(nat.lib().tsgnn_panel_blocks(int(rows), int(panel_units)))
    if npan <= ncu or 2 * nslab + npan <= 2 * ncu:
        return nslab, rps, need
    cap = max(32, (2 * ncu - npan) // 2)
    rps = -(-rows // cap)
    rps = (rps + 7) // 8 * 8
    nslab = -(-rows // rps)
    return nslab, rps, nslab * (K + 1) * N


def _gather_ok(g, x):
    if not GATHER_FUSED or g.val is not None or not mp.ell_ok(x) or g.total_rows > GATHER_MAX_ROWS:
        return False
    return True


def _flush_readout(g, B, sn, sg, pending):
    if pending is not None:
        y, pk = pending
        nat.call("readout_partial_f32", g.graph_ptr, B, sn, g.n_rows, sg, y, y.stride(0), y.size(1), pk)


_PER_GRAPH = [False]


class per_graph_stats:
    def __init__(self, on=True):
        self.on = bool(on)

    def __enter__(self):
        self.prev = _PER_GRAPH[0]
        _PER_GRAPH[0] = self.on

    def __exit__(self, *exc):
        _PER_GRAPH[0] = self.prev
        return False


class _SageStack(torch.autograd.Function):

    @staticmethod
    def forward(ctx, x0, g, has_bias, n_head, nodes, *params):
        head = params[len(params) - n_head:] if n_head else None
        params = params[:len(params) - n_head] if n_head else params
        L = len(params) // 2
        Ws = [params[2 * l].contiguous() for l in range(L)]
        bs = [params[2 * l + 1] if has_bias else None for l in range(L)]
        dev = x0.device
        R, B = g.total_rows, g.B
        Fh, Fl = Ws[0].size(1), Ws[-1].size(1)
        total = B * ((L - 1) * Fh + Fl)
        packed = torch.empty(total + Fl, dtype=torch.int64, device=dev) if not nodes else None
        cat = torch.empty(R, (L - 1) * Fh + Fl, dtype=torch.float32, device=dev) if nodes else None
        x = mp._check(x0, R)
        gs = g.n_ghost
        if g.n_ghost > 0 and x.stride(0) % 4 == 0 and all(
                Ws[l].size(1) % 4 == 0 and Ws[l].data_ptr() % 16 == 0 and (bs[l] is None or bs[l].data_ptr() % 16 == 0)
                for l in range(L)):
            fixed = getattr(g, "ghost_slots_fixed", None)
            gs = min(g.nmax, (int(fixed) if fixed is not None else int(g.sizes.max()) + 1))
        if nodes == 1:
            gs = g.n_ghost
        sn, sg = (gs, gs) if g.n_ghost else (g.nmax, 0)
        saved = []
        off = 0
        pending_ro = None
        keep = []
        last_ro_done = False
        bnf = None
        per_graph = ctx.per_graph = bool(_PER_GRAPH[0])
        if per_graph and head is not None:
            raise NotImplementedError("per-graph statistics: the readout and the node-feature form of the stack only")
        if (FUSED_BN and not per_graph and head is not None and not nodes and L >= 2 and g.n_ghost == g.nmax and sn == sg and sn <= 1024
                and Fh == 128 and Fl == 128 and Ws[0].size(0) <= 128 and x.size(1) % 4 == 0 and MERGED_FWD and EPILOGUE_READOUT
                and _gather_ok(g, x) and all(Ws[l].size(0) == 128 and Ws[l].stride(0) % 4 == 0 for l in range(1, L))
                and all(Ws[l].data_ptr() % 16 == 0 and (bs[l] is None or bs[l].data_ptr() % 16 == 0) for l in range(L))
                and mp.rowgemm_ok(x, x.stride(0), Ws[0], Ws[0].stride(0), Ws[0].size(0), Fh, False)
                and head[0].size(0) <= 128 and (L - 1) * Fh + Fl <= 2048 and g.row_graph is not None):
            ell_s = g.ell_slots()
            if ell_s is not None:
                bnf = g.bn_workspace(B, L, Fh, Fl, sn)
                if bnf["dirty"]:
                    bnf["sums"].zero_(); bnf["ghost"].zero_(); bnf["packed"].zero_()
                bnf["dirty"] = True
                packed = bnf["packed"]
        if bnf is not None:
            ell, ell_w, tail = g.ell()
            tp, tc = tail if tail is not None else (None, None)
            ell_s, tc_s = ell_s
            sums, ghost = bnf["sums"], bnf["ghost"]
            ro_map, ro_ch = g.readout_map(sn, gs) if RO_MAP else (None, 0)
            for l in range(L):
                K, N = Ws[l].size(0), Ws[l].size(1)
                v = torch.empty(R, N, dtype=torch.float32, device=dev)
                rinv = torch.empty(R, dtype=torch.float32, device=dev)
                z = torch.empty(R, x.size(1) if l == 0 else Fh, dtype=torch.float32, device=dev)
                s_out = sums[l * 2 * sn:(l + 1) * 2 * sn] if l < L - 1 else None
                g_out = ghost[2 * l:2 * l + 2] if l < L - 1 else None
                if l == 0:
                    nat.call("gather_rowgemm_st_f32", ell, ell_w, tp, tc, x, x.stride(0), Ws[0], Ws[0].stride(0), bs[0], v, v.stride(0), rinv, z,
                             z.stride(0), g.n_rows, K, N, gs, g.row_slot, s_out, g_out, int(g.panel_units))
                    mean = rstd = None
                else:
                    pm, pr_ = saved[l - 1][3], saved[l - 1][4]
                    last = l == L - 1
                    nat.call("sage_layer_fwd_bn_f32", ell_s, ell_w, tp, tc_s, saved[l - 1][1], saved[l - 1][1].stride(0), Ws[l], Ws[l].stride(0), bs[l],
                             v, v.stride(0), rinv, z, z.stride(0), g.n_rows, K, gs, g.graph_ptr, g.slot_count, B, sn, sg,
                             packed[(l - 1) * B * Fh:(l - 1) * B * Fh + B * Fh],
                             packed[l * B * Fh:l * B * Fh + (B + 1) * N] if last else None, g.row_graph,
                             sums[(l - 1) * 2 * sn:l * 2 * sn], ghost[2 * (l - 1):2 * l], pm, pr_,
                             None if last else g.row_slot, s_out, g_out, ro_map, ro_ch, int(g.panel_units))
                if l < L - 1:
                    mean = torch.empty(g.nmax, dtype=torch.float32, device=dev)
                    rstd = torch.empty(g.nmax, dtype=torch.float32, device=dev)
                else:
                    mean = rstd = None
                saved.append((z, v, rinv, mean, rstd, True))
            last_ro_done = True
        for l in (range(L) if bnf is None else ()):
            K, N = Ws[l].size(0), Ws[l].size(1)
            if nodes and l == L - 1:
                v = cat[:, (L - 1) * Fh:]
            else:
                v = torch.empty(R, N, dtype=torch.float32, device=dev)
            rinv = torch.empty(R, dtype=torch.float32, device=dev)
            lean = (g.n_ghost > 0 and x.stride(0) % 4 == 0 and N % 4 == 0 and Ws[l].data_ptr() % 16 == 0
                    and (bs[l] is None or bs[l].data_ptr() % 16 == 0))
            fused = lean and N <= 128 and _gather_ok(g, x) and mp.rowgemm_ok(x, x.stride(0), Ws[l], Ws[l].stride(0), K, N, False)
            if (fused and MERGED_FWD and pending_ro is not None and K == 128 and N == 128 and x.size(1) == 128
                    and Ws[l].stride(0) % 4 == 0):
                ell, ell_w, tail = g.ell()
                tp, tc = tail if tail is not None else (None, None)
                z = torch.empty(R, x.size(1), dtype=torch.float32, device=dev)
                if EPILOGUE_READOUT and l == L - 1 and not nodes and l > 0 and (not g.n_ghost or gs > 0):
                    nat.call("sage_layer_fwd_ro_f32", ell, ell_w, tp, tc, x, x.stride(0), Ws[l], Ws[l].stride(0), bs[l], v, v.stride(0),
                             rinv, z, z.stride(0), g.n_rows, K, gs, g.graph_ptr, B, sn, sg, pending_ro[1],
                             packed[off:off + (B + 1) * N], g.row_graph)
                    last_ro_done = True
                else:
                    nat.call("sage_layer_fwd_f32", ell, ell_w, tp, tc, x, x.stride(0), Ws[l], Ws[l].stride(0), bs[l], v, v.stride(0), rinv,
                             z, z.stride(0), g.n_rows, K, gs, g.graph_ptr, B, sn, sg, pending_ro[1])
                pending_ro = None
            elif fused:
                _flush_readout(g, B, sn, sg, pending_ro)
                pending_ro = None
                ell, ell_w, tail = g.ell()
                tp, tc = tail if tail is not None else (None, None)
                z = torch.empty(R, x.size(1), dtype=torch.float32, device=dev)
                nat.call("gather_rowgemm_f32", ell, ell_w, tp, tc, x, x.stride(0), Ws[l], Ws[l].stride(0), 0, bs[l], v, v.stride(0), rinv,
                         z, z.stride(0), g.n_rows, K, N, 1, gs)
            else:
                _flush_readout(g, B, sn, sg, pending_ro)
                pending_ro = None
                z = _aggregate_raw(g, x, rows=g.n_rows if lean else None)
                if lean and mp.rowgemm_ok(z, z.stride(0), Ws[l], Ws[l].stride(0), K, N, False):
                    nat.call("rowgemm_f32", z, z.stride(0), Ws[l], Ws[l].stride(0), 0, bs[l], v, v.stride(0), rinv, g.n_rows, K, N, 1,
                             gs)
                elif mp.rowgemm_ok(z, z.stride(0), Ws[l], Ws[l].stride(0), K, N, False):
                    if lean:
                        z[g.n_rows:].zero_()
                        lean = False
                    nat.call("rowgemm_f32", z, z.stride(0), Ws[l], Ws[l].stride(0), 0, bs[l], v, v.stride(0), rinv, R, K, N, 1, 0)
                else:
                    if lean:
                        z[g.n_rows:].zero_()
                        lean = False
                    nat.call("linear_l2norm_f32", z, z.stride(0), Ws[l], Ws[l].stride(0), bs[l], v, v.stride(0), rinv, R, K, N, 1)
            pk = packed[off:off + B * N] if not nodes else None
            if l < L - 1 and per_graph:
                mean = torch.empty(R, dtype=torch.float32, device=dev)
                rstd = torch.empty(R, dtype=torch.float32, device=dev)
                y = torch.empty_like(v) if not nodes else cat[:, l * Fh:(l + 1) * Fh]
                if l == 0 and not nodes:
                    packed[:total].zero_()
                nat.call("row_ln_fwd_f32", v, v.stride(0), g.n_rows + sg, N, 1, mean, rstd, y, y.stride(0))
                if not nodes:
                    pending_ro = (y, pk)
                keep.append(y)
                x = y
            elif l < L - 1:
                mean = torch.empty(g.nmax, dtype=torch.float32, device=dev)
                rstd = torch.empty(g.nmax, dtype=torch.float32, device=dev)
                y = torch.empty_like(v) if not nodes else cat[:, l * Fh:(l + 1) * Fh]
                nat.call("slot_bn_fwd_f32", g.graph_ptr, g.slot_count, B, sn, g.n_rows, sg, v, v.stride(0), N, 1,
                         mean, rstd, y, y.stride(0), packed if (l == 0 and not nodes) else None, total)
                if not nodes:
                    pending_ro = (y, pk)
                keep.append(y)
                x = y
            else:
                mean = rstd = None
                if head is None and not nodes and not last_ro_done:
                    nat.call("readout_partial_f32", g.graph_ptr, B, sn, g.n_rows, sg, v, v.stride(0), N, pk)
            saved.append((z, v, rinv, mean, rstd, lean))
            off += B * N
        ctx.nodes = nodes
        if nodes:
            if nodes == 2 and g.n_ghost:
                nat.defer_zero(cat[g.n_rows:])
            ctx.g, ctx.L, ctx.has_bias, ctx.dims = g, L, has_bias, (Fh, Fl)
            ctx.slots = (sn, sg)
            ctx.Ws, ctx.saved, ctx.arg = Ws, saved, None
            ctx.params = params
            ctx.head = None
            return cat
        out = torch.empty(B, (L - 1) * Fh + Fl, dtype=torch.float32, device=dev)
        arg = torch.empty(total, dtype=torch.int32, device=dev)
        ctx.g, ctx.L, ctx.has_bias, ctx.dims = g, L, has_bias, (Fh, Fl)
        ctx.slots = (sn, sg)
        ctx.Ws, ctx.saved, ctx.arg = Ws, saved, arg
        ctx.params = params
        ctx.x0_ld = x.size(1) if L == 0 else x0.size(1)
        ctx.head = None
        if head is None:
            nat.call("readout_decode_layers_f32", packed, B, L, Fh, Fl, out, out.stride(0), arg)
            return out
        w1, b1, w2, b2 = head
        w1c, w2c = w1.contiguous(), w2.contiguous()
        E, C = w1c.size(0), w2c.size(0)
        vec = torch.empty(B, E, dtype=torch.float32, device=dev)
        y = torch.empty(B, C, dtype=torch.float32, device=dev)
        v_last = saved[-1][1]
        if bnf is not None:
            nat.call("packed_head_fwd_z_f32", packed, B, L, Fh, Fl, out, out.stride(0), arg, w1c, b1, w2c, b2, E, C, vec, y,
                     bnf["sums"], (L - 1) * 2 * sn)
            bnf["dirty"] = False
        elif last_ro_done and E <= 128 and out.size(1) <= 2048:
            nat.call("packed_head_fwd_f32", packed, B, L, Fh, Fl, out, out.stride(0), arg, w1c, b1, w2c, b2, E, C, vec, y)
        else:
            nat.call("readout_head_fwd_f32", packed, B, L, Fh, Fl, v_last, v_last.stride(0), g.graph_ptr, g.n_rows, sn, sg, out,
                     out.stride(0), arg, w1c, b1, w2c, b2, E, C, vec, y)
        ctx.head = (out, vec, w1c, w2c, head)
        ctx.set_materialize_grads(False)
        return vec, y

    @staticmethod
    def backward(ctx, *gouts):
        g, L = ctx.g, ctx.L
        Fh, Fl = ctx.dims
        R, B = g.total_rows, g.B
        head_grads = ()
        du_last = None
        if ctx.head is None:
            dout = gouts[0].contiguous()
            dev = dout.device
        else:
            out, vec, w1c, w2c, (pw1, pb1, pw2, pb2) = ctx.head
            dvec, dy = gouts
            dev = out.device
            P, E, C = out.size(1), w1c.size(0), w2c.size(0)
            if dy is None and dvec is None:
                return (None,) * (5 + 2 * L + 4)
            ce = mp.take_deferred_ce(dy) if dy is not None else None
            if ce is None:
                dy = dy.contiguous() if dy is not None else torch.zeros(B, C, device=dev)
            dvec = dvec.contiguous() if dvec is not None else None
            dout = torch.empty(B, P, dtype=torch.float32, device=dev)
            dw1, s1 = mp._sink_or_new(pw1, (E, P), dev)
            dw2, s2 = mp._sink_or_new(pw2, (C, E), dev)
            db1, s3 = mp._sink_or_new(pb1, (E,), dev) if pb1 is not None else (None, False)
            db2, s4 = mp._sink_or_new(pb2, (C,), dev) if pb2 is not None else (None, False)
            parts = mp.head_norm_slots((s1, s2, s3, s4), (pb1 is not None, pb2 is not None), (pw1, pb1, pw2, pb2), E)
            sn_, sg_ = ctx.slots
            v_l, rinv_l, lean_l = ctx.saved[L - 1][1], ctx.saved[L - 1][2], ctx.saved[L - 1][5]
            if (HEAD_DU and LAST_LAYER_ROWS and not ctx.nodes and L > 1 and lean_l and Fl % 4 == 0 and Fl <= 128 and g.n_ghost == g.nmax
                    and sn_ == sg_ and g.n_ghost >= B and ctx.needs_input_grad[5 + 2 * (L - 1)] and v_l.stride(0) % 4 == 0):
                du_l = torch.empty(R, Fl, dtype=torch.float32, device=dev)
                argl = ctx.arg[(L - 1) * B * Fh:(L - 1) * B * Fh + B * Fl]
                dmap, ndmap, dchunk = g.du_map(B + (E + 3) // 4 + 1) if DU_MAP else (None, 0, 64)
                if nat.try_call("head2_bwd_du_map_f32", out, out.stride(0), vec, ce[0] if ce is not None else None,
                                ce[1] if ce is not None else None, ce[2] if ce is not None else None, None if ce is not None else dy, dvec,
                                w1c, w2c, B, P, E, C, dout, dout.stride(0), dw1, db1, dw2, db2, parts, g.graph_ptr, g.n_rows, sg_,
                                sn_, v_l, v_l.stride(0), rinv_l, argl, (L - 1) * Fh, Fl, du_l, du_l.stride(0), dmap, ndmap, dchunk):
                    du_last = du_l
            if du_last is not None:
                pass
            elif ce is not None:
                nat.call("head2_bwd_ce_f32", out, out.stride(0), vec, ce[0], ce[1], ce[2], dvec, w1c, w2c, B, P, E, C, dout,
                         dout.stride(0), dw1, db1, dw2, db2, parts)
            else:
                nat.call("head2_bwd_f32", out, out.stride(0), vec, dy, dvec, w1c, w2c, B, P, E, C, dout, dout.stride(0), dw1, db1, dw2,
                         db2, parts)
            head_grads = (None if s1 else dw1, None if s3 else db1, None if s2 else dw2, None if s4 else db2)
            if mp.GRAD_SINK is not None and s1 and s2 and (s3 or pb1 is None) and (s4 or pb2 is None):
                mp.GRAD_SINK.ready((pw1, pb1, pw2, pb2))
        sn, sg = ctx.slots
        grads = [None] * (2 * L)
        dxs = None
        dx0 = None
        keep = []
        red = mp.WgradSets(mp.wgrad_reduce_multi, max_sets_with_shares=4)
        for l in range(L - 1, -1, -1):
            z, v, rinv, mean, rstd, lean = ctx.saved[l]
            W = ctx.Ws[l]
            K, N = W.size(0), W.size(1)
            last = l == L - 1
            du = du_last if (last and du_last is not None) else torch.empty(R, N, dtype=torch.float32, device=dev)
            bo = sg
            if ctx.nodes:
                dsl = argl = None
                dnode = dout[:, l * Fh:l * Fh + N]
            else:
                dsl = dout[:, l * Fh:l * Fh + N]
                argl = ctx.arg[l * B * Fh:l * B * Fh + B * N]
                dnode = None
            if last and du_last is not None:
                bo = B
            elif (LAST_LAYER_ROWS and last and not ctx.nodes and dxs is None and N % 4 == 0 and N <= 128 and g.n_ghost == g.nmax
                    and sn == sg and dout.stride(0) % 4 == 0 and dsl.data_ptr() % 16 == 0 and g.row_graph is not None):
                nat.call("readout_l2_bwd_f32", g.graph_ptr, g.row_graph, B, g.n_rows, sg, v, v.stride(0), dsl, dout.stride(0), argl, N, rinv,
                         du, du.stride(0))
            elif (SLOT_WGRAD and l == 0 and L > 1 and not ctx.nodes and not ctx.needs_input_grad[0] and lean and B <= 32 and N == 128
                  and K <= 128 and sn == sg and g.n_ghost == g.nmax and ctx.needs_input_grad[5] and z.stride(0) % 4 == 0
                  and z.data_ptr() % 16 == 0 and v.data_ptr() % 16 == 0 and (not ctx.has_bias or ctx.needs_input_grad[6])):
                per = int(os.environ.get("TSGNN_SLOT_WGRAD_PER", "2"))
                nblk = max(1, -(-sn // per))
                ws0 = torch.empty(nblk * (K + 1) * N, dtype=torch.float32, device=dev)
                nat.call("slot_post_wgrad_f32", g.graph_ptr, g.slot_count, B, sn, g.n_rows, sg, v, v.stride(0), dxs,
                         dxs.stride(0) if dxs is not None else 0, dsl, dout.stride(0) if dsl is not None else 0, argl, N, 1, 1, mean, rstd,
                         rinv, z, z.stride(0), K, ws0, nblk)
                dw = red.grad(ctx.params[0], (K, N))
                db = red.grad(ctx.params[1] if ctx.has_bias else None, (N,))
                red.add((ws0, nblk, K, N, dw, db))
                grads[0], grads[1] = red.autograd_grad(dw), red.autograd_grad(db)
                continue
            elif ctx.per_graph and ctx.nodes:
                nat.call("row_post_nodes_bwd_f32", g.n_rows, g.n_rows + sg, v, v.stride(0), dxs, dxs.stride(0) if dxs is not None else 0,
                         dnode, dnode.stride(0), 1 if ctx.nodes == 2 else 0, N, 0 if last else 1, 0 if last else 1, mean, rstd, rinv, du,
                         du.stride(0))
            elif ctx.per_graph:
                nat.call("row_post_bwd_f32", g.row_graph, B, g.n_rows, g.n_rows + sg, v, v.stride(0), dxs,
                         dxs.stride(0) if dxs is not None else 0, dsl, dout.stride(0), argl, N, 0 if last else 1, 0 if last else 1, mean,
                         rstd, rinv, du, du.stride(0))
            else:
                nat.call("slot_post_bwd_f32", g.graph_ptr, g.slot_count, B, sn, g.n_rows, sg, v, v.stride(0), dxs,
                         dxs.stride(0) if dxs is not None else 0, dnode, dnode.stride(0) if dnode is not None else 0, dsl,
                         dout.stride(0) if dsl is not None else 0, argl, N, 0 if last else 1, 0 if last else 1, mean, rstd, rinv, du,
                         du.stride(0))
            want_w = ctx.needs_input_grad[5 + 2 * l]
            want_b = ctx.has_bias and ctx.needs_input_grad[6 + 2 * l]
            merged = False
            if (MERGED_BWD and want_w and lean and l > 0 and K == 128 and N == 128 and g.symmetric and z.size(1) == K
                    and _gather_ok(g, du) and z.data_ptr() % 16 == 0 and du.data_ptr() % 16 == 0 and W.data_ptr() % 16 == 0
                    and W.stride(0) % 4 == 0):
                nslab, rps, need = mp.wgrad_plan(g.n_rows, K, N, z.stride(0), du.stride(0))
                nslab, rps, need = _slabs_beside_panels(nslab, rps, need, g.n_rows, K, N, dev, g.panel_units)
                if 0 < nslab < 512:
                    ell, ell_w, tail = g.ell()
                    tp, tc = tail if tail is not None else (None, None)
                    ws = torch.empty(need, dtype=torch.float32, device=dev)
                    dxs = torch.empty(R, K, dtype=torch.float32, device=dev)
                    nat.call("sage_layer_bwd_f32", ell, ell_w, tp, tc, du, du.stride(0), W, W.stride(0), dxs, dxs.stride(0), z, z.stride(0),
                             g.n_rows, nslab, rps, bo, ws, int(g.panel_units))
                    dw = red.grad(ctx.params[2 * l], (K, N))
                    db = red.grad(ctx.params[2 * l + 1] if want_b else None, (N,))
                    red.add((ws, nslab, K, N, dw, db))
                    grads[2 * l], grads[2 * l + 1] = red.autograd_grad(dw), red.autograd_grad(db)
                    keep.append(du)
                    merged = True
            if merged:
                continue
            if want_w:
                if not lean and sg < g.n_ghost:
                    du[g.n_rows + sg:].zero_()
                sl = mp.linear_wgrad_slabs(z, K, du[:g.n_rows + bo] if lean else du, bias_only_rows=bo if lean else 0)
                if sl is not None:
                    dw = red.grad(ctx.params[2 * l], (K, N))
                    db = red.grad(ctx.params[2 * l + 1] if want_b else None, (N,))
                    red.add((sl[0], sl[1], K, N, dw, db))
                    dw, db = red.autograd_grad(dw), red.autograd_grad(db)
                else:
                    if lean:
                        z[g.n_rows:].zero_()
                        du[g.n_rows + sg:].zero_()
                    dw, db = mp.linear_wgrad(z, K, du, want_b)
                grads[2 * l], grads[2 * l + 1] = dw, db
            elif want_b:
                if sg < g.n_ghost:
                    du[g.n_rows + sg:].zero_()
                grads[2 * l + 1] = mp.colsum(du)
            keep.append(du)
            need_dx = l > 0 or ctx.needs_input_grad[0]
            if need_dx:
                ldz = z.size(1)
                if (l > 0 and g.n_ghost > 0 and g.symmetric and ldz == K and K <= 128 and _gather_ok(g, du)
                        and mp.rowgemm_ok(du, du.stride(0), W, W.stride(0), N, K, True)):
                    ell, ell_w, tail = g.ell()
                    tp, tc = tail if tail is not None else (None, None)
                    dxs = torch.empty(R, ldz, dtype=torch.float32, device=dev)
                    nat.call("gather_rowgemm_f32", ell, ell_w, tp, tc, du, du.stride(0), W, W.stride(0), 1, None, dxs, dxs.stride(0), None,
                             None, 0, g.n_rows, N, K, 0, 0)
                else:
                    dz = torch.zeros(R, ldz, dtype=torch.float32, device=dev) if ldz > K else torch.empty(R, ldz, dtype=torch.float32, device=dev)
                    if mp.rowgemm_ok(du, du.stride(0), W, W.stride(0), N, K, True):
                        nat.call("rowgemm_f32", du, du.stride(0), W, W.stride(0), 1, None, dz, dz.stride(0), None, g.n_rows, N, K, 0, 0)
                    else:
                        mp.gemm(du, du.stride(0), 1, W, 1, W.stride(0), dz, dz.stride(0), 1, R, K, N)
                    dxs = _aggregate_raw(g, dz, transposed=True, rows=g.n_rows if (l > 0 and g.n_ghost) else None)
                if l == 0:
                    dx0 = dxs
        red.close()
        del keep
        return (dx0, None, None, None, None) + tuple(grads) + head_grads


def sage_stack_readouts(x, g, convs):
    has_bias = convs[0].bias is not None
    params = []
    for c in convs:
        params.append(c.weight)
        params.append(c.bias if has_bias else c.weight.new_zeros(1))
    return _SageStack.apply(x, g, has_bias, 0, 0, *params)


def sage_stack_nodes(x, g, convs, mask_ghost):
    has_bias = convs[0].bias is not None
    params = []
    for c in convs:
        params.append(c.weight)
        params.append(c.bias if has_bias else c.weight.new_zeros(1))
    return _SageStack.apply(x, g, has_bias, 0, 2 if (mask_ghost and g.n_ghost) else 1, *params)


PAIR_LAUNCHES = os.environ.get("TSGNN_STACK_PAIRS", "1") != "0"
ZERO_RIDER = os.environ.get("TSGNN_ZERO_RIDER", "1") != "0"


def _multi(tn, gs, zero=None):
    import numpy as np
    words = [len(tn), len(gs)]
    for a in tn:
        words += [nat._arg(v) or 0 for v in a[:11]]
    for a in gs:
        words += [(nat._arg(v) or 0) if not isinstance(v, bool) else int(v) for v in a[:20]]
    d = np.asarray(words, dtype=np.int64)
    if zero is not None:
# ... 152 lines not shown
```

Before: 249,400.

## Pre-pack layer weights into MFMA fragment images and load B directly from them

The first-layer gather GEMM now also packs the weights of the later layers, both forward and transposed, into a fragment-ordered float4 image using a pack descriptor. The forward BN layer kernels and the merged backward kernels then read B operands directly into registers from this image, skipping the LDS staging and commit of W. This is meant to cut LDS traffic and synchronisation inside the rowgemm loop and to shrink LDS use. The cost is extra packing work and scratch memory per forward pass, plus more template variants. There are also minor rewrites of the rider copy loop and of register indexing in the head kernel.

Measured after the change: 257,800 (median of 6 runs). +3.4%, better.

```diff
diff --git a/include/tsgnn.h b/include/tsgnn.h
--- a/include/tsgnn.h
+++ b/include/tsgnn.h
@@ -150,14 +150,14 @@
 int tsgnn_gather_rowgemm_st_f32(const int* ell, int ell_w, const int* tail_ptr, const int* tail_col, const float* x, int64_t ldx, const float* b, int64_t ldb, const float* bias,
                                 float* c, int64_t ldc, float* rinv, float* zout, int64_t ldz, int64_t rows, int K, int N,
                                 int64_t fill_rows, const int* row_slot, unsigned long long* sums, float* ghost, int panel_units,
-                                tsgnn_stream_t stream);
+                                const int64_t* pack_desc, tsgnn_stream_t stream);
 int tsgnn_sage_layer_fwd_bn_f32(const int* ell, int ell_w, const int* tail_ptr, const int* tail_col, const float* x, int64_t ldx, const float* w, int64_t ldw, const float* bias,
                                 float* v, int64_t ldv, float* rinv, float* zout, int64_t ldz, int64_t rows, int K, int64_t fill_rows,
                                 const int* graph_ptr, const int* slot_count, int B, int nslots, int n_ghost, unsigned long long* packed,
                                 unsigned long long* packed_out, const int* row_graph, const unsigned long long* sums_in,
                                 const float* ghost_in, float* mean_out, float* rstd_out, const int* row_slot,
                                 unsigned long long* sums_out, float* ghost_out, const int* ro_map, int ro_map_ch, int panel_units,
-                                tsgnn_stream_t stream);
+                                const float* w_img, tsgnn_stream_t stream);
 int tsgnn_sage_layer_fwd_bn_plan(int64_t rows, int64_t fill_rows, int B, int nslots, int panel_units, int* ro_ch, int* n_gemm,
                                  int* n_full);
 int tsgnn_sage_layer_fwd_f32(const int* ell, int ell_w, const int* tail_ptr, const int* tail_col, const float* x, int64_t ldx, const float* w, int64_t ldw, const float* bias,
@@ -169,7 +169,7 @@
                                 unsigned long long* packed_out, const int* row_graph, tsgnn_stream_t stream);
 int tsgnn_sage_layer_bwd_f32(const int* ell, int ell_w, const int* tail_ptr, const int* tail_col, const float* du, int64_t lddu, const float* w, int64_t ldw, float* dxs,
                              int64_t lddxs, const float* z, int64_t ldz, int64_t rows, int nslab, int64_t rows_per_slab,
-                             int64_t bias_only_rows, float* ws, int panel_units, tsgnn_stream_t stream);
+                             int64_t bias_only_rows, float* ws, int panel_units, const float* w_img, tsgnn_stream_t stream);
 int tsgnn_l2norm_bwd_f32(const float* v, int64_t ldv, const float* dv, int64_t lddv, const float* rinv, float* du,
                          int64_t lddu, int64_t rows, int F, tsgnn_stream_t stream);
 
diff --git a/two-stage-gnn_amd/csrc/head.hip b/two-stage-gnn_amd/csrc/head.hip
--- a/two-stage-gnn_amd/csrc/head.hip
+++ b/two-stage-gnn_amd/csrc/head.hip
@@ -6,6 +6,7 @@
 namespace {
 
 __device__ __forceinline__ float4 ld4(const float* p) { return *reinterpret_cast<const float4*>(p); }
+__device__ __forceinline__ float pick4(const float (&r)[4], int q) { return q == 0 ? r[0] : q == 1 ? r[1] : q == 2 ? r[2] : r[3]; }
 
 constexpr int HW = 16;
 
@@ -498,7 +499,7 @@
   if (dy_ready_needs_sync) __syncthreads();
   for (int j = tid; j < E; j += NTH) {
     float acc = j == tid ? dv0 : (dvec ? dvec[(int64_t)b * E + j] : 0.f);
-    for (int q = 0; q < C; ++q) acc = fmaf(dy[(int64_t)b * C + q], (j == tid && q < 4) ? w2r[q] : w2[(int64_t)q * E + j], acc);
+    for (int q = 0; q < C; ++q) acc = fmaf(dy[(int64_t)b * C + q], (j == tid && q < 4) ? pick4(w2r, q) : w2[(int64_t)q * E + j], acc);
     ds[j] = acc;
   }
   __syncthreads();
@@ -651,7 +652,7 @@
     }
     for (int j = tid; j < E; j += NTH) {
       float acc = j == tid ? dv0 : (dvec ? dvec[(int64_t)b * E + j] : 0.f);
-      for (int c = 0; c < C; ++c) acc = fmaf(dy[(int64_t)b * C + c], (j == tid && c < 4) ? w2r[c] : w2[(int64_t)c * E + j], acc);
+      for (int c = 0; c < C; ++c) acc = fmaf(dy[(int64_t)b * C + c], (j == tid && c < 4) ? pick4(w2r, c) : w2[(int64_t)c * E + j], acc);
       ds[j] = acc;
     }
     __syncthreads();
@@ -714,7 +715,7 @@
       float a = 0.f;
       if (jj < E) {
         a = i == tid ? dv0 : (dvec ? dvec[(int64_t)bb * E + jj] : 0.f);
-        for (int c = 0; c < C; ++c) a = fmaf(dy[(int64_t)bb * C + c], (i == tid && c < 4) ? w2r[c] : w2[(int64_t)c * E + jj], a);
+        for (int c = 0; c < C; ++c) a = fmaf(dy[(int64_t)bb * C + c], (i == tid && c < 4) ? pick4(w2r, c) : w2[(int64_t)c * E + jj], a);
       }
       dvs[i] = a;
     }
diff --git a/two-stage-gnn_amd/csrc/ingest_rider.h b/two-stage-gnn_amd/csrc/ingest_rider.h
--- a/two-stage-gnn_amd/csrc/ingest_rider.h
+++ b/two-stage-gnn_amd/csrc/ingest_rider.h
@@ -26,13 +26,10 @@
 
 __device__ __forceinline__ void pull_rider_body(const PullRider& p, unsigned b) {
   const long long gtid = (long long)b * blockDim.x + threadIdx.x, gsize = (long long)p.blocks * blockDim.x;
-  int4 v[4];
   long long i = p.lo + gtid;
   for (; i + 3 * gsize < p.n4; i += 4 * gsize) {
-#pragma unroll
-    for (int u = 0; u < 4; ++u) v[u] = p.host[i + u * gsize];
-#pragma unroll
-    for (int u = 0; u < 4; ++u) p.mirror[i + u * gsize] = v[u];
+    const int4 v0 = p.host[i], v1 = p.host[i + gsize], v2 = p.host[i + 2 * gsize], v3 = p.host[i + 3 * gsize];
+    p.mirror[i] = v0; p.mirror[i + gsize] = v1; p.mirror[i + 2 * gsize] = v2; p.mirror[i + 3 * gsize] = v3;
   }
   for (; i < p.n4; i += gsize) p.mirror[i] = p.host[i];
 }
diff --git a/two-stage-gnn_amd/csrc/layer_bwd.hip b/two-stage-gnn_amd/csrc/layer_bwd.hip
--- a/two-stage-gnn_amd/csrc/layer_bwd.hip
+++ b/two-stage-gnn_amd/csrc/layer_bwd.hip
@@ -6,11 +6,11 @@
 
 namespace {
 
-template <bool PANELS_FIRST, bool UNITS = false>
+template <bool PANELS_FIRST, bool UNITS = false, bool BIMG = false>
 __global__ __launch_bounds__(256) void sage_layer_bwd_kernel(RowGemmArgs ga, TnArgs gt, unsigned n_tn, unsigned nslab, unsigned n_pan, int slab_delay) {
   extern __shared__ __attribute__((aligned(16))) float smem[];
   if (PANELS_FIRST) {
-    if (blockIdx.x < n_pan) rowgemm_body<4, true, true, 1, false, false, false, UNITS>(ga, smem, blockIdx.x);
+    if (blockIdx.x < n_pan) rowgemm_body<4, true, true, 1, false, false, false, UNITS, BIMG>(ga, smem, blockIdx.x);
     else {
       for (int i = 0; i < slab_delay; ++i) __builtin_amdgcn_s_sleep(16);
       const unsigned b = blockIdx.x - n_pan, by = b / nslab, sp = b % nslab;
@@ -20,7 +20,7 @@
     }
   } else {
     if (blockIdx.x < n_tn) tn_rows_body<4, 4, 2>(gt, smem, blockIdx.x % nslab, blockIdx.x / nslab, nslab);
-    else rowgemm_body<4, true, true, 1, false, false, false, UNITS>(ga, smem, blockIdx.x - n_tn);
+    else rowgemm_body<4, true, true, 1, false, false, false, UNITS, BIMG>(ga, smem, blockIdx.x - n_tn);
   }
 }
 
@@ -30,28 +30,37 @@
 
 int tsgnn_sage_layer_bwd_f32(const int* ell, int ell_w, const int* tail_ptr, const int* tail_col, const float* du, int64_t lddu, const float* w, int64_t ldw, float* dxs,
                              int64_t lddxs, const float* z, int64_t ldz, int64_t rows, int nslab, int64_t rows_per_slab,
-                             int64_t bias_only_rows, float* ws, int panel_units, tsgnn_stream_t stream) {
+                             int64_t bias_only_rows, float* ws, int panel_units, const float* w_img, tsgnn_stream_t stream) {
   if (!ell || !du || !w || !dxs || !z || !ws || rows <= 0 || nslab <= 0 || rows_per_slab <= 0 || bias_only_rows < 0) return TSGNN_EINVAL;
   if (ell_w != 4 && ell_w != 8 && ell_w != 16) return TSGNN_EUNSUPPORTED;
   const uintptr_t al = reinterpret_cast<uintptr_t>(ell) | reinterpret_cast<uintptr_t>(du) | reinterpret_cast<uintptr_t>(w) |
-                       reinterpret_cast<uintptr_t>(dxs) | reinterpret_cast<uintptr_t>(z);
+                       reinterpret_cast<uintptr_t>(dxs) | reinterpret_cast<uintptr_t>(z) | reinterpret_cast<uintptr_t>(w_img);
   if ((al & 15) || (lddu % 4) || (ldw % 4) || (lddxs % 4) || (ldz % 4) || lddu < 128 || ldw < 128 || lddxs < 128 || ldz < 128)
     return TSGNN_EUNSUPPORTED;
   if ((tail_ptr == nullptr) != (tail_col == nullptr)) return TSGNN_EINVAL;
   RowGemmArgs ga{du, lddu, w, ldw, nullptr, dxs, lddxs, nullptr, rows, 128, 128, 0, 0, ell, ell_w, nullptr, 0, tail_ptr, tail_col};
+  ga.b_img = reinterpret_cast<const float4*>(w_img);
   TnArgs gt{z, ldz, du, lddu, rows, rows_per_slab, 128, 128, ws, nullptr, bias_only_rows};
   const int ncu = device_cu_count();
   const unsigned n_tn = 2u * (unsigned)nslab, n_pan = panel_split(rows, ncu, panel_units, &ga.n_full, &ga.unit);
-  constexpr size_t la = rowgemm_lds_bytes<4, true, true>(), lt = tn_rows_lds_bytes<4, 4>();
+  constexpr size_t lt = tn_rows_lds_bytes<4, 4>();
+  const size_t la = w_img ? rowgemm_lds_bytes<4, true, true, 1, false, true>() : rowgemm_lds_bytes<4, true, true>();
+  const size_t lds = la > lt ? la : lt;
   static const int panels_first = [] { const char* e = getenv("TSGNN_BWD_PANELS_FIRST"); return e ? atoi(e) : 1; }();
   static const int slab_delay_env = [] { const char* e = getenv("TSGNN_SLAB_DELAY"); return e ? atoi(e) : -1; }();
   const int slab_delay = slab_delay_env >= 0 ? slab_delay_env : ((int64_t)n_pan <= (int64_t)ncu ? 2 : 0);
   const bool units = ga.unit == 8 || ga.unit == 16;
   TSGNN_KNAME("sage_layer_bwd_kernel<%s,%s>", panels_first ? "true" : "false", units ? "true" : "false");
-  if (panels_first && units) sage_layer_bwd_kernel<true, true><<<n_tn + n_pan, 256, la > lt ? la : lt, stream>>>(ga, gt, n_tn, (unsigned)nslab, n_pan, slab_delay);
-  else if (panels_first) sage_layer_bwd_kernel<true><<<n_tn + n_pan, 256, la > lt ? la : lt, stream>>>(ga, gt, n_tn, (unsigned)nslab, n_pan, slab_delay);
-  else if (units) sage_layer_bwd_kernel<false, true><<<n_tn + n_pan, 256, la > lt ? la : lt, stream>>>(ga, gt, n_tn, (unsigned)nslab, n_pan, slab_delay);
-  else sage_layer_bwd_kernel<false><<<n_tn + n_pan, 256, la > lt ? la : lt, stream>>>(ga, gt, n_tn, (unsigned)nslab, n_pan, slab_delay);
+#define TSGNN_BWD_(PF_, UN_) \
+  do {                       \
+    if (w_img) sage_layer_bwd_kernel<PF_, UN_, true><<<n_tn + n_pan, 256, lds, stream>>>(ga, gt, n_tn, (unsigned)nslab, n_pan, slab_delay); \
+    else sage_layer_bwd_kernel<PF_, UN_><<<n_tn + n_pan, 256, lds, stream>>>(ga, gt, n_tn, (unsigned)nslab, n_pan, slab_delay);            \
+  } while (0)
+  if (panels_first && units) TSGNN_BWD_(true, true);
+  else if (panels_first) TSGNN_BWD_(true, false);
+  else if (units) TSGNN_BWD_(false, true);
+  else TSGNN_BWD_(false, false);
+#undef TSGNN_BWD_
   TSGNN_CHECK_LAUNCH();
   return TSGNN_OK;
 }
diff --git a/two-stage-gnn_amd/csrc/layer_fwd.hip b/two-stage-gnn_amd/csrc/layer_fwd.hip
--- a/two-stage-gnn_amd/csrc/layer_fwd.hip
+++ b/two-stage-gnn_amd/csrc/layer_fwd.hip
@@ -20,13 +20,13 @@
   }
 }
 
-template <bool RO, bool ST, bool UNITS = false>
+template <bool RO, bool ST, bool UNITS = false, bool BIMG = false>
 __global__ __launch_bounds__(256, 2) void sage_layer_fwd_bn_kernel(RowGemmArgs ga, SlotArgs sa, BnReadArgs bn, unsigned n_gemm, unsigned ro_gx,
                                                                 int ro_ch, int F4, unsigned long long* __restrict__ packed, unsigned n_main,
                                                                 PullRider pr, const int* __restrict__ ro_map) {
   extern __shared__ __attribute__((aligned(16))) float smem[];
   if (blockIdx.x < n_gemm) {
-    rowgemm_body<4, false, true, 1, RO, true, ST, UNITS>(ga, smem, blockIdx.x);
+    rowgemm_body<4, false, true, 1, RO, true, ST, UNITS, BIMG>(ga, smem, blockIdx.x);
   } else if (blockIdx.x < n_main) {
     unsigned r = blockIdx.x - n_gemm;
     if (ro_map) r = (unsigned)ro_map[r];
@@ -57,7 +57,7 @@
                                 unsigned long long* packed_out, const int* row_graph, const unsigned long long* sums_in,
                                 const float* ghost_in, float* mean_out, float* rstd_out, const int* row_slot,
                                 unsigned long long* sums_out, float* ghost_out, const int* ro_map, int ro_map_ch, int panel_units,
-                                tsgnn_stream_t stream) {
+                                const float* w_img, tsgnn_stream_t stream) {
   if (!ell || !x || !w || !v || !rinv || !graph_ptr || !slot_count || !packed || !sums_in || !ghost_in || !mean_out || !rstd_out ||
       rows <= 0 || fill_rows < 0 || K <= 0 || B <= 0 || nslots <= 0 || (n_ghost != 0 && n_ghost != nslots) || (packed_out && !row_graph) ||
       (row_slot && (!sums_out || !ghost_out)))
@@ -65,7 +65,7 @@
   if (ell_w != 4 && ell_w != 8 && ell_w != 16) return TSGNN_EUNSUPPORTED;
   const uintptr_t al = reinterpret_cast<uintptr_t>(ell) | reinterpret_cast<uintptr_t>(x) | reinterpret_cast<uintptr_t>(w) |
                        reinterpret_cast<uintptr_t>(v) | reinterpret_cast<uintptr_t>(zout) | reinterpret_cast<uintptr_t>(bias) |
-                       reinterpret_cast<uintptr_t>(sums_in) | reinterpret_cast<uintptr_t>(sums_out);
+                       reinterpret_cast<uintptr_t>(sums_in) | reinterpret_cast<uintptr_t>(sums_out) | reinterpret_cast<uintptr_t>(w_img);
   if ((al & 15) || K != 128 || (ldx % 4) || (ldw % 4) || (ldv % 4) || (zout && (ldz % 4 || ldz < K)) || ldx < K || ldw < 128 || ldv < 128 ||
       nslots > BN_TAB || rows >= (1 << 20) || n_ghost == 0 || (packed_out && row_slot))
     return TSGNN_EUNSUPPORTED;
@@ -74,6 +74,7 @@
   RowGemmArgs ga{x, ldx, w, ldw, bias, v, ldv, rinv, rows, K, 128, 1, fill_rows, ell, ell_w, zout, ldz, tail_ptr, tail_col,
                  packed_out, graph_ptr, row_graph, B, nslots, n_ghost};
   ga.st_row_slot = row_slot; ga.st_sums = sums_out; ga.st_ghost = ghost_out;
+  ga.b_img = reinterpret_cast<const float4*>(w_img);
   ga.bn_sums = sums_in; ga.bn_ghost = ghost_in; ga.bn_slot_count = slot_count; ga.bn_B = B; ga.bn_nslots = nslots; ga.bn_F = K;
   SlotArgs sa{graph_ptr, slot_count, B, nslots, rows, n_ghost};
   BnReadArgs bn{sums_in, ghost_in, K, mean_out, rstd_out};
@@ -83,16 +84,18 @@
   while (ro_ch < 256 && n_gemm + (unsigned)((nslots + ro_ch - 1) / ro_ch) * (unsigned)B > 2u * (unsigned)ncu) ro_ch *= 2;
   const unsigned ro_gx = (unsigned)((nslots + ro_ch - 1) / ro_ch);
   if (ro_map && ro_map_ch != ro_ch) ro_map = nullptr;
-  size_t lds = rowgemm_lds_bytes<4, false, true, 1, true>();
+  size_t lds = w_img ? rowgemm_lds_bytes<4, false, true, 1, true, true>() : rowgemm_lds_bytes<4, false, true, 1, true>();
   const size_t lro = 8 * 128 * sizeof(unsigned long long) + 256 * sizeof(float2);
   if (lds < lro) lds = lro;
   const unsigned n_main = n_gemm + ro_gx * (unsigned)B;
   const PullRider pr = take_pull_rider();
   const bool units = ga.unit == 8 || ga.unit == 16;
-#define TSGNN_FWD_BN(RO_, ST_)                                                                                                              \
-  do {                                                                                                                                      \
-    if (units) sage_layer_fwd_bn_kernel<RO_, ST_, true><<<n_main + pr.blocks, 256, lds, stream>>>(ga, sa, bn, n_gemm, ro_gx, ro_ch, K / 4, packed, n_main, pr, ro_map); \
-    else sage_layer_fwd_bn_kernel<RO_, ST_><<<n_main + pr.blocks, 256, lds, stream>>>(ga, sa, bn, n_gemm, ro_gx, ro_ch, K / 4, packed, n_main, pr, ro_map);             \
+#define TSGNN_FWD_BN_(RO_, ST_, UN_, IM_) \
+  sage_layer_fwd_bn_kernel<RO_, ST_, UN_, IM_><<<n_main + pr.blocks, 256, lds, stream>>>(ga, sa, bn, n_gemm, ro_gx, ro_ch, K / 4, packed, n_main, pr, ro_map)
+#define TSGNN_FWD_BN(RO_, ST_)                                                                  \
+  do {                                                                                          \
+    if (units) { if (w_img) TSGNN_FWD_BN_(RO_, ST_, true, true); else TSGNN_FWD_BN_(RO_, ST_, true, false); }   \
+    else { if (w_img) TSGNN_FWD_BN_(RO_, ST_, false, true); else TSGNN_FWD_BN_(RO_, ST_, false, false); }       \
   } while (0)
   if (packed_out) {
     TSGNN_KNAME("sage_layer_fwd_bn_kernel<true,false,%s>", units ? "true" : "false");
@@ -105,6 +108,7 @@
     TSGNN_FWD_BN(false, false);
   }
 #undef TSGNN_FWD_BN
+#undef TSGNN_FWD_BN_
   TSGNN_CHECK_LAUNCH();
   return TSGNN_OK;
 }
diff --git a/two-stage-gnn_amd/csrc/pack_body.h b/two-stage-gnn_amd/csrc/pack_body.h
--- /dev/null
+++ b/two-stage-gnn_amd/csrc/pack_body.h
@@ -0,0 +1,37 @@
+#pragma once
+#include "common.h"
+
+struct PackSet {
+  const float* w; int64_t ldw; int K, N; int kn;
+  float4* out;
+};
+constexpr int PACK_SET_ENTRIES = 4096;
+
+__device__ __forceinline__ void sage_conv_pack_body(const PackSet& s, int e) {
+  const int lane = e & 63, u = (e >> 6) & 15, wv = e >> 10;
+  const int i = lane & 31, h = lane >> 5;
+  const int n = 32 * wv + i, k0 = 8 * u + 4 * h;
+  float v[4];
+#pragma unroll
+  for (int c = 0; c < 4; ++c) {
+    const int k = k0 + c;
+    const bool ok = n < s.N && k < s.K;
+    v[c] = ok ? (s.kn ? s.w[(int64_t)k * s.ldw + n] : s.w[(int64_t)n * s.ldw + k]) : 0.f;
+  }
+  s.out[e] = make_float4(v[0], v[1], v[2], v[3]);
+}
+
+static inline int pack_set_from_desc(const int64_t* d, PackSet& s) {
+  s.w = reinterpret_cast<const float*>(d[0]); s.ldw = d[1]; s.K = (int)d[2]; s.N = (int)d[3]; s.kn = (int)d[4];
+  s.out = reinterpret_cast<float4*>(d[5]);
+  if (!s.w || !s.out || s.K < 1 || s.K > 128 || s.N < 1 || s.N > 128 || s.ldw < (s.kn ? s.N : s.K)) return TSGNN_EINVAL;
+  if (reinterpret_cast<uintptr_t>(s.out) & 15) return TSGNN_EUNSUPPORTED;
+  return TSGNN_OK;
+}
+
+constexpr int PACK_RIDER_SETS = 8;
+struct PackRider { PackSet s[PACK_RIDER_SETS]; unsigned blocks; };
+__device__ __forceinline__ void pack_rider_body(const PackRider& p, unsigned b) {
+  const unsigned e = b * blockDim.x + threadIdx.x;
+  sage_conv_pack_body(p.s[e / PACK_SET_ENTRIES], (int)(e % PACK_SET_ENTRIES));
+}
diff --git a/two-stage-gnn_amd/csrc/rowgemm.hip b/two-stage-gnn_amd/csrc/rowgemm.hip
--- a/two-stage-gnn_amd/csrc/rowgemm.hip
+++ b/two-stage-gnn_amd/csrc/rowgemm.hip
@@ -4,6 +4,7 @@
 #include <cstdlib>
 #include "rowgemm_body.h"
 #include "ingest_rider.h"
+#include "pack_body.h"
 #include "rowgemm_big_body.h"
 
 namespace {
@@ -29,15 +30,19 @@
   rowgemm_body<NT, TRANS_B, true, 2>(g, smem, blockIdx.x);
 }
 
+__device__ __forceinline__ void st_passengers(const PackRider& pk, const PullRider& pr, unsigned b) {
+  if (b < pk.blocks) pack_rider_body(pk, b);
+  else pull_rider_body(pr, b - pk.blocks);
+}
 template <bool UNITS>
-__global__ __launch_bounds__(256) void rowgemm_gather_st_kernel(RowGemmArgs g, PullRider pr, unsigned nblk) {
-  extern __shared__ __attribute__((aligned(16))) float smem[];
-  if (blockIdx.x >= nblk) { pull_rider_body(pr, blockIdx.x - nblk); return; }
+__global__ __launch_bounds__(256) void rowgemm_gather_st_kernel(RowGemmArgs g, PullRider pr, unsigned nblk, PackRider pk) {
+  extern __shared__ __attribute__((aligned(16))) float smem[];
+  if (blockIdx.x >= nblk) { st_passengers(pk, pr, blockIdx.x - nblk); return; }
   rowgemm_body<4, false, true, 1, false, false, true, UNITS>(g, smem, blockIdx.x);
 }
-__global__ __launch_bounds__(512) void rowgemm_gather_ks2_st_kernel(RowGemmArgs g, PullRider pr, unsigned nblk) {
-  extern __shared__ __attribute__((aligned(16))) float smem[];
-  if (blockIdx.x >= nblk) { pull_rider_body(pr, blockIdx.x - nblk); return; }
+__global__ __launch_bounds__(512) void rowgemm_gather_ks2_st_kernel(RowGemmArgs g, PullRider pr, unsigned nblk, PackRider pk) {
+  extern __shared__ __attribute__((aligned(16))) float smem[];
+  if (blockIdx.x >= nblk) { st_passengers(pk, pr, blockIdx.x - nblk); return; }
   rowgemm_body<4, false, true, 2, false, false, true>(g, smem, blockIdx.x);
 }
 
@@ -215,7 +220,7 @@
 int tsgnn_gather_rowgemm_st_f32(const int* ell, int ell_w, const int* tail_ptr, const int* tail_col, const float* x, int64_t ldx, const float* b, int64_t ldb, const float* bias,
                                 float* c, int64_t ldc, float* rinv, float* zout, int64_t ldz, int64_t rows, int K, int N,
                                 int64_t fill_rows, const int* row_slot, unsigned long long* sums, float* ghost, int panel_units,
-                                tsgnn_stream_t stream) {
+                                const int64_t* pack_desc, tsgnn_stream_t stream) {
   if (!ell || !x || !b || !c || !row_slot || !sums || !ghost || rows <= 0 || fill_rows < 0 || K <= 0 || N <= 0 || ldx < K || ldc < N)
     return TSGNN_EINVAL;
   if (ell_w != 4 && ell_w != 8 && ell_w != 16) return TSGNN_EUNSUPPORTED;
@@ -224,6 +229,17 @@
     return TSGNN_EUNSUPPORTED;
   if (zout && ((ldz % 4) || ldz < K || (reinterpret_cast<uintptr_t>(zout) & 15))) return TSGNN_EUNSUPPORTED;
   if ((N % 4) || (ldc % 4) || (reinterpret_cast<uintptr_t>(c) & 15) || (bias && (reinterpret_cast<uintptr_t>(bias) & 15))) return TSGNN_EUNSUPPORTED;
+  PackRider pk{};
+  if (pack_desc) {
+    if (reinterpret_cast<uintptr_t>(pack_desc) & 7) return TSGNN_EINVAL;
+    const int nsets = (int)pack_desc[0];
+    if (nsets <= 0 || nsets > PACK_RIDER_SETS) return TSGNN_EINVAL;
+    for (int t = 0; t < nsets; ++t) {
+      const int rc = pack_set_from_desc(pack_desc + 1 + 6 * t, pk.s[t]);
+      if (rc != TSGNN_OK) return rc;
+    }
+    pk.blocks = (unsigned)nsets;
+  }
   if ((tail_ptr == nullptr) != (tail_col == nullptr)) return TSGNN_EINVAL;
   RowGemmArgs g{x, ldx, b, ldb, bias, c, ldc, rinv, rows, K, N, 1, fill_rows, ell, ell_w, zout, ldz, tail_ptr, tail_col};
   g.st_row_slot = row_slot; g.st_sums = sums; g.st_ghost = ghost;
@@ -239,13 +255,15 @@
       attr = true;
     }
     const PullRider pr = take_pull_rider(512);
+    pk.blocks *= PACK_SET_ENTRIES / 512;
     TSGNN_KNAME("rowgemm_gather_ks2_st_kernel");
-    rowgemm_gather_ks2_st_kernel<<<nblk + pr.blocks, 512, lds2, stream>>>(g, pr, nblk);
+    rowgemm_gather_ks2_st_kernel<<<nblk + pk.blocks + pr.blocks, 512, lds2, stream>>>(g, pr, nblk, pk);
   } else {
     const PullRider pr = take_pull_rider(256);
+    pk.blocks *= PACK_SET_ENTRIES / 256;
     TSGNN_KNAME("rowgemm_gather_st_kernel<%s>", (g.unit == 8 || g.unit == 16) ? "true" : "false");
-    if (g.unit == 8 || g.unit == 16) rowgemm_gather_st_kernel<true><<<nblk + pr.blocks, 256, rowgemm_lds_bytes<4, false, true>(), stream>>>(g, pr, nblk);
-    else rowgemm_gather_st_kernel<false><<<nblk + pr.blocks, 256, rowgemm_lds_bytes<4, false, true>(), stream>>>(g, pr, nblk);
+    if (g.unit == 8 || g.unit == 16) rowgemm_gather_st_kernel<true><<<nblk + pk.blocks + pr.blocks, 256, rowgemm_lds_bytes<4, false, true>(), stream>>>(g, pr, nblk, pk);
+    else rowgemm_gather_st_kernel<false><<<nblk + pk.blocks + pr.blocks, 256, rowgemm_lds_bytes<4, false, true>(), stream>>>(g, pr, nblk, pk);
   }
   TSGNN_CHECK_LAUNCH();
   return TSGNN_OK;
diff --git a/two-stage-gnn_amd/csrc/rowgemm_body.h b/two-stage-gnn_amd/csrc/rowgemm_body.h
--- a/two-stage-gnn_amd/csrc/rowgemm_body.h
+++ b/two-stage-gnn_amd/csrc/rowgemm_body.h
@@ -30,6 +30,7 @@
   const unsigned long long* bn_sums; const float* bn_ghost; const int* bn_slot_count; int bn_B, bn_nslots, bn_F;
   int n_full;
   int unit;
+  const float4* b_img;
 };
 
 inline int panel_unit_rows(int64_t rows, int ncu) {
@@ -61,12 +62,14 @@
 constexpr int GN = 8;
 constexpr int LDA_F = 128;
 
-template <int NT, bool TRANS_B, bool GATHER, int KS = 1, bool READOUT = false, bool BNIN = false, bool STATS = false, bool UNITS = false>
+template <int NT, bool TRANS_B, bool GATHER, int KS = 1, bool READOUT = false, bool BNIN = false, bool STATS = false, bool UNITS = false,
+          bool BIMG = false>
 __device__ __forceinline__ void rowgemm_body(const RowGemmArgs& g, float* smem_all, unsigned bid) {
   static_assert(KS == 1 || (KS == 2 && GATHER && NT <= 4), "the split-K variant is built for the gather kernel, widths <= 128");
   static_assert(!READOUT || (NT <= 4 && KS == 1), "the readout epilogue is built for one column tile per wave");
   static_assert(!BNIN || (GATHER && KS == 1), "batch-norm on the fly lives in the gather prologue of the one-group kernel");
   static_assert(!STATS || NT <= 4, "the statistics epilogue is built for one column tile per wave");
+  static_assert(!BIMG || (GATHER && KS == 1 && NT == 4), "the image variant is built for the one-group gather kernel at K = N = 128");
   constexpr int NP = 32 * NT;
   constexpr int TPW = (NT + 3) / 4;
   constexpr int BV = NT;
@@ -80,10 +83,10 @@
   const int Kc = KS == 1 ? g.K : ((g.K + 2 * KC - 1) / (2 * KC)) * KC;
   const int kb = grp * Kc;
   const int Kv = KS == 1 ? g.K : min(g.K - kb, Kc);
-  constexpr int GRP = (KS == 2 && 2 * STAGE < 4096 + 256) ? 4096 + 256 : 2 * STAGE;
+  constexpr int GRP = BIMG ? 256 : (KS == 2 && 2 * STAGE < 4096 + 256) ? 4096 + 256 : 2 * STAGE;
   float* smem = smem_all + grp * GRP;
   float* Apanel = smem_all + KS * GRP + (KS == 2 ? 0 : 256);
-  float* scratch = KS == 2 ? smem_all + GRP + 4096 : smem_all + 2 * STAGE;
+  float* scratch = KS == 2 ? smem_all + GRP + 4096 : smem_all + GRP;
   const unsigned npanels = (unsigned)((g.rows + 31) / 32);
   int64_t m0, rows_hi;
   if constexpr (UNITS) {
@@ -247,6 +250,7 @@
                               : *reinterpret_cast<const float4*>(As + i * lda_s + 8 * u + 4 * h);
       af[4 * u] = v.x; af[4 * u + 1] = v.y; af[4 * u + 2] = v.z; af[4 * u + 3] = v.w;
     }
+    if constexpr (BIMG) return;
 #pragma unroll
     for (int t = 0; t < TPW; ++t) {
       const int tile = wid + 4 * t;
@@ -309,9 +313,20 @@
   if constexpr (STATS) {
     if (g.st_sums && wid == 0 && grp == 0 && lane < 32 && (m0 + lane) < rows_hi) st_slot = g.st_row_slot[m0 + lane];
   }
-#pragma unroll
-  for (int c = 0; c < NS; ++c)
-    if (c == 0 || c * KC < Kc) fetch(st[c], c * KC);
+  if constexpr (!BIMG) {
+#pragma unroll
+    for (int c = 0; c < NS; ++c)
+      if (c == 0 || c * KC < Kc) fetch(st[c], c * KC);
+  }
+  float bq[BIMG ? 4 * KC / 2 : 1];
+  auto img_fetch = [&](int u0) {
+    const float4* img = g.b_img + (wid * 16 + u0) * 64 + lane;
+#pragma unroll
+    for (int u = 0; u < 8; ++u) {
+      const float4 v = img[u * 64];
+      bq[4 * (u0 + u)] = v.x; bq[4 * (u0 + u) + 1] = v.y; bq[4 * (u0 + u) + 2] = v.z; bq[4 * (u0 + u) + 3] = v.w;
+    }
+  };
   if (GATHER) {
     const int c4 = tid_all & 31, rsub = tid_all >> 5;
     const bool colok = 4 * c4 < g.K;
@@ -334,6 +349,11 @@
         nbv[p][k] = make_float4(0.f, 0.f, 0.f, 0.f);
         if (colok && ids[p][k] >= 0) nbv[p][k] = ldg4(g.a + (int64_t)(BNIN ? (ids[p][k] & 0xFFFFF) : ids[p][k]) * g.lda + 4 * c4);
       }
+    if constexpr (BIMG) {
+      __builtin_amdgcn_sched_barrier(0);
+      img_fetch(0);
+      __builtin_amdgcn_sched_barrier(0);
+    }
     if constexpr (BNIN) {
       __syncthreads();
 #pragma unroll
@@ -393,6 +413,11 @@
       }
       if (g.zout && colok && row < rows_hi) st_out(reinterpret_cast<float4*>(g.zout + row * g.ldz + 4 * c4), va);
     }
+    if constexpr (BIMG) {
+      __builtin_amdgcn_sched_barrier(0);
+      img_fetch(8);
+      __builtin_amdgcn_sched_barrier(0);
+    }
   }
   float bias_v[TPW];
 #pragma unroll
@@ -401,13 +426,27 @@
     bias_v[t] = (g.bias && (wid + 4 * t) < NT && cn < g.N) ? g.bias[cn] : 0.f;
   }
   TR(1);
-  commit(st[0], smem);
-  if (KC < Kc) commit(st[1], smem + STAGE);
+  if constexpr (!BIMG) {
+    commit(st[0], smem);
+    if (KC < Kc) commit(st[1], smem + STAGE);
+  }
   __syncthreads();
   TR(2);
   float fa[2][KC / 2], fb[2][TPW][KC / 2];
   frags(smem, 0, fa[0], fb[0]);
-  if (NS == 2) {
+  if constexpr (BIMG) {
+#pragma unroll
+    for (int c = 0; c < 4; ++c) {
+      if (c < 3) frags(smem, (c + 1) * KC, fa[(c + 1) & 1], fb[0]);
+      __builtin_amdgcn_sched_barrier(0);
+#pragma unroll
+      for (int j = 0; j < KC / 2; ++j) acc[0] = __builtin_amdgcn_mfma_f32_32x32x2f32(fa[c & 1][j], bq[16 * c + j], acc[0], 0, 0, 0);
+      __builtin_amdgcn_sched_barrier(0);
+      TR(3 + 2 * c);
+      TR(4 + 2 * c);
+    }
+  }
+  if (NS == 2 && !BIMG) {
     if (2 * KC < Kc) fetch(st[0], 2 * KC);
     if (3 * KC < Kc) fetch(st[1], 3 * KC);
   }
@@ -437,7 +476,7 @@
     if (Kc > 2 * KC) __syncthreads();
     TR(4 + 2 * min(c, 3));
   };
-  for (int c = 0; c * KC < Kc; c += 4) {
+  for (int c = 0; !BIMG && c * KC < Kc; c += 4) {
     body(std::integral_constant<int, 0>{}, c);
     if ((c + 1) * KC < Kc) body(std::integral_constant<int, 1>{}, c + 1);
     if ((c + 2) * KC < Kc) body(std::integral_constant<int, 2>{}, c + 2);
@@ -568,10 +607,10 @@
 }
 
 
-template <int NT, bool TRANS_B, bool GATHER, int KS = 1, bool BNIN = false>
+template <int NT, bool TRANS_B, bool GATHER, int KS = 1, bool BNIN = false, bool BIMG = false>
 constexpr size_t rowgemm_lds_bytes() {
   constexpr int NP = 32 * NT;
-  constexpr int STAGE2 = 2 * ((GATHER ? 0 : 32 * LDA_S) + (TRANS_B ? NP * LDA_S : KC * NP));
+  constexpr int STAGE2 = BIMG ? 256 : 2 * ((GATHER ? 0 : 32 * LDA_S) + (TRANS_B ? NP * LDA_S : KC * NP));
   constexpr int GRP = (KS == 2 && STAGE2 < 4096 + 256) ? 4096 + 256 : STAGE2;
   return sizeof(float) * (KS * GRP + (KS == 2 ? 0 : 128 + 4 * 32) + (GATHER ? 32 * LDA_F : 0) + (BNIN ? 2 * BN_TAB : 0));
 }
diff --git a/two-stage-gnn_amd/csrc/sageconv.hip b/two-stage-gnn_amd/csrc/sageconv.hip
--- a/two-stage-gnn_amd/csrc/sageconv.hip
+++ b/two-stage-gnn_amd/csrc/sageconv.hip
@@ -2,6 +2,7 @@
 #include "common.h"
 #include "../../include/tsgnn.h"
 #include "sageconv_body.h"
+#include "pack_body.h"
 #include "tn_rows_body.h"
 
 namespace {
@@ -73,26 +74,10 @@
   }
 }
 
-struct PackSet {
-  const float* w; int64_t ldw; int K, N; int kn;
-  float4* out;
-};
 struct PackArgs { PackSet s[16]; int nsets; };
 
 __global__ __launch_bounds__(256) void sage_conv_pack_kernel(PackArgs a) {
-  const PackSet& s = a.s[blockIdx.y];
-  const int e = (int)blockIdx.x * 256 + (int)threadIdx.x;
-  const int lane = e & 63, u = (e >> 6) & 15, wv = e >> 10;
-  const int i = lane & 31, h = lane >> 5;
-  const int n = 32 * wv + i, k0 = 8 * u + 4 * h;
-  float v[4];
-#pragma unroll
-  for (int c = 0; c < 4; ++c) {
-    const int k = k0 + c;
-    const bool ok = n < s.N && k < s.K;
-    v[c] = ok ? (s.kn ? s.w[(int64_t)k * s.ldw + n] : s.w[(int64_t)n * s.ldw + k]) : 0.f;
-  }
-  s.out[e] = make_float4(v[0], v[1], v[2], v[3]);
+  sage_conv_pack_body(a.s[blockIdx.y], (int)blockIdx.x * 256 + (int)threadIdx.x);
 }
 
 }
@@ -109,11 +94,8 @@
   a.nsets = nsets;
   const int64_t* d = desc + 1;
   for (int t = 0; t < nsets; ++t, d += 6) {
-    PackSet& s = a.s[t];
-    s.w = reinterpret_cast<const float*>(d[0]); s.ldw = d[1]; s.K = (int)d[2]; s.N = (int)d[3]; s.kn = (int)d[4];
-    s.out = reinterpret_cast<float4*>(d[5]);
-    if (!s.w || !s.out || !tsgnn_sage_conv_supported(s.K, s.N) || s.ldw < (s.kn ? s.N : s.K)) return TSGNN_EINVAL;
-    if (reinterpret_cast<uintptr_t>(s.out) & 15) return TSGNN_EUNSUPPORTED;
+    const int rc = pack_set_from_desc(d, a.s[t]);
+    if (rc != TSGNN_OK) return rc;
   }
   TSGNN_KNAME("sage_conv_pack_kernel");
   sage_conv_pack_kernel<<<dim3(16, (unsigned)nsets), 256, 0, stream>>>(a);
diff --git a/two-stage-gnn_amd/sage_stack.py b/two-stage-gnn_amd/sage_stack.py
--- a/two-stage-gnn_amd/sage_stack.py
+++ b/two-stage-gnn_amd/sage_stack.py
@@ -1,3 +1,4 @@
+import numpy as np
 import torch
 
 from . import _native as nat
@@ -85,6 +86,9 @@
 
 
 _PER_GRAPH = [False]
+
+_IMG_FLOATS = 16384
+_IMG_LAYERS = 4
 
 
 class per_graph_stats:
@@ -147,12 +151,24 @@
                     bnf["sums"].zero_(); bnf["ghost"].zero_(); bnf["packed"].zero_()
                 bnf["dirty"] = True
                 packed = bnf["packed"]
+        ctx.w_img = ctx.pack_desc = None
         if bnf is not None:
             ell, ell_w, tail = g.ell()
             tp, tc = tail if tail is not None else (None, None)
             ell_s, tc_s = ell_s
             sums, ghost = bnf["sums"], bnf["ghost"]
             ro_map, ro_ch = g.readout_map(sn, gs) if RO_MAP else (None, 0)
+            w_img = pack_desc = None
+            if 1 <= L - 1 <= _IMG_LAYERS:
+                w_img = torch.empty(2 * (L - 1), _IMG_FLOATS, dtype=torch.float32, device=dev)
+                pack_desc = np.empty(1 + 12 * (L - 1), dtype=np.int64)
+                pack_desc[0] = 2 * (L - 1)
+                for l in range(1, L):
+                    for kn in (1, 0):
+                        t = 2 * (l - 1) + (1 - kn)
+                        pack_desc[1 + 6 * t:7 + 6 * t] = (Ws[l].data_ptr(), Ws[l].stride(0), 128, 128, kn, w_img[t].data_ptr())
+                bnf["pack_desc"] = pack_desc
+            ctx.w_img, ctx.pack_desc = w_img, pack_desc
             for l in range(L):
                 K, N = Ws[l].size(0), Ws[l].size(1)
                 v = torch.empty(R, N, dtype=torch.float32, device=dev)
@@ -162,7 +178,8 @@
                 g_out = ghost[2 * l:2 * l + 2] if l < L - 1 else None
                 if l == 0:
                     nat.call("gather_rowgemm_st_f32", ell, ell_w, tp, tc, x, x.stride(0), Ws[0], Ws[0].stride(0), bs[0], v, v.stride(0), rinv, z,
-                             z.stride(0), g.n_rows, K, N, gs, g.row_slot, s_out, g_out, int(g.panel_units))
+                             z.stride(0), g.n_rows, K, N, gs, g.row_slot, s_out, g_out, int(g.panel_units),
+                             pack_desc.ctypes.data if pack_desc is not None else None)
                     mean = rstd = None
                 else:
                     pm, pr_ = saved[l - 1][3], saved[l - 1][4]
@@ -172,7 +189,8 @@
                              packed[(l - 1) * B * Fh:(l - 1) * B * Fh + B * Fh],
                              packed[l * B * Fh:l * B * Fh + (B + 1) * N] if last else None, g.row_graph,
                              sums[(l - 1) * 2 * sn:l * 2 * sn], ghost[2 * (l - 1):2 * l], pm, pr_,
-                             None if last else g.row_slot, s_out, g_out, ro_map, ro_ch, int(g.panel_units))
+                             None if last else g.row_slot, s_out, g_out, ro_map, ro_ch, int(g.panel_units),
+                             w_img[2 * (l - 1)] if w_img is not None else None)
                 if l < L - 1:
                     mean = torch.empty(g.nmax, dtype=torch.float32, device=dev)
                     rstd = torch.empty(g.nmax, dtype=torch.float32, device=dev)
@@ -302,6 +320,7 @@
         g, L = ctx.g, ctx.L
         Fh, Fl = ctx.dims
         R, B = g.total_rows, g.B
+        w_img = ctx.w_img
         head_grads = ()
         du_last = None
         if ctx.head is None:
@@ -414,7 +433,8 @@
                     ws = torch.empty(need, dtype=torch.float32, device=dev)
                     dxs = torch.empty(R, K, dtype=torch.float32, device=dev)
                     nat.call("sage_layer_bwd_f32", ell, ell_w, tp, tc, du, du.stride(0), W, W.stride(0), dxs, dxs.stride(0), z, z.stride(0),
-                             g.n_rows, nslab, rps, bo, ws, int(g.panel_units))
+                             g.n_rows, nslab, rps, bo, ws, int(g.panel_units),
+                             w_img[2 * (l - 1) + 1] if w_img is not None else None)
                     dw = red.grad(ctx.params[2 * l], (K, N))
                     db = red.grad(ctx.params[2 * l + 1] if want_b else None, (N,))
                     red.add((ws, nslab, K, N, dw, db))
```
